# PacificBiosciences/pb-StarPhase

Measured on AMD Instinct MI355X. Metric: HiFi reads/sec diplotyped (HLA+CYP2D6), higher is better.
Workload: dtype int32; 1 GPU; BASELINE configs[1] + configs[2] as ONE sample per step: HLA-A/-B 10000 HiFi reads vs IMGT/HLA v0.14.1 (11,199 DNA alleles) + CYP2D6 2000 targeted reads (39 templates), the six configs[2] scenarios in turn; a new sample uploaded every step; reads -> diplotypes; hla_reads=10000, cyp2d6_reads=2000, cyp2d6_lanes=6, hla_lanes=2, cyp2d6_consensus=launch pairs

## Files before the change

pb-starphase_amd/csrc/sp_affine.hip:

```cpp
#include "sp_internal.h"
#include "sp_wfa.hip.h"
#include <mutex>
#include <set>
#include <string>

namespace {

constexpr int AF_NEG = -(1 << 28);
constexpr uint32_t AF_BIAS = 1u << 22;

struct AfState { int s; uint32_t m0, m1; };
struct AfKey { uint32_t k, m0, m1; };

__device__ __forceinline__ AfState af_none() { AfState x; x.s = AF_NEG; x.m0 = 0; x.m1 = 0; return x; }
template <int CTRL, int ROW_MASK>
__device__ __forceinline__ AfKey af_dpp(const AfKey& v) {
    AfKey r;
    r.k = (uint32_t)__builtin_amdgcn_update_dpp(0, (int)v.k, CTRL, ROW_MASK, 0xf, false);
    r.m0 = (uint32_t)__builtin_amdgcn_update_dpp(0, (int)v.m0, CTRL, ROW_MASK, 0xf, false);
    r.m1 = (uint32_t)__builtin_amdgcn_update_dpp(0, (int)v.m1, CTRL, ROW_MASK, 0xf, false);
    return r;
}
__device__ __forceinline__ AfKey af_max(const AfKey& a, const AfKey& b) { return b.k > a.k ? b : a; }
__device__ __forceinline__ AfKey af_scan(AfKey v) {
// ... 307 lines not shown
        }
        spw::wave_lds_sync();
        if (lane == 0) {
            while (true) {
                const int r = ci - i_lo - r0;
                if (r < 0) break;
                if ((unsigned)cidx >= (unsigned)BAND) { done = 2; break; }
                const uint32_t d = tile[r * BAND + cidx];
                if (st == 0) {
                    const uint32_t h = d & 7u;
                    if (h == AF_D_DIAG || h == AF_D_START) { emit((d & AF_D_X) ? 8u : 7u); --ci; if (h == AF_D_START) { done = 1; break; } continue; }
                    if (h >= AF_D_NONE) { done = 2; break; }
                    st = (int)h;
                }
                if (st == (int)AF_D_E1 || st == (int)AF_D_E2) {
                    emit(2u); const bool cont = d & (st == (int)AF_D_E1 ? AF_D_E1C : AF_D_E2C); --ci; ++cidx; if (!cont) st = 0;
                } else {
                    emit(1u); const bool cont = d & (st == (int)AF_D_F1 ? AF_D_F1C : AF_D_F2C); --cidx; if (!cont) st = 0;
                }
            }
        }
        ci = __shfl(ci, 0); done = __shfl(done, 0);
        if (ci < i_lo && !done) done = 2;
    }
    if (lane == 0) {
        emit(0xE);
        res.score = bs; res.nm = (int32_t)bm1; res.b_start = (int32_t)(bm0 >> 16); res.b_end = bi + 1; res.a_start = (int32_t)(bm0 & 0xFFFFu); res.a_end = bj + 1;
        const bool lost = done != 1 || n_ops > ops_cap;
        out[p] = res; n_cigar[p] = lost ? AF_TB_LOST : n_ops;
        const uint32_t n_out = lost ? 0u : (n_ops < stride ? n_ops : stride);
        for (uint32_t k = 0; k < n_out; ++k) cigar[(size_t)p * stride + k] = ops[n_ops - 1 - k];
    }
}

inline int64_t af_tb_rows(int tlen, int qlen, int diag, int band) {
    const int64_t klo = -(int64_t)diag - band / 2;
    int64_t i_lo = -(klo + band - 1); if (i_lo < 0) i_lo = 0;
    int64_t i_hi = (int64_t)qlen - 1 - klo; if (i_hi > (int64_t)tlen - 1) i_hi = (int64_t)tlen - 1;
    if (tlen <= 0 || qlen <= 0 || i_lo > i_hi) return 0;
    return i_hi - i_lo + 1;
}

}

int sp_launch_affine(sp_ctx* ctx, const sp_seqset* A, const sp_seqset* B, const void* d_pairs, uint64_t n_pairs, const sp_affine_opts& o, int band, sp_affine_aln* d_out,
                     const char* prof_name, const uint32_t* d_n_live, const void* d_wins, const void* d_mids) {
    if (n_pairs == 0) return SP_OK;
    if (band != 64 && band != 256) return sp_fail(ctx, SP_ERR_INVALID_ARG, "affine: band must be 64 or 256");
    if (B->max_len > 65535 || A->max_len > 65535) return sp_fail(ctx, SP_ERR_TOO_LONG, "affine: sequences of up to 65,535 bases");
    const int t_words_max = (B->max_len >> 4) + 4;
    const size_t lds_bytes = sizeof(uint32_t) * (size_t)(4 * t_words_max + 2 * (2 * band / 16 + 8));
    ProfScope ps(ctx, prof_name, n_pairs);
    const bool hasn = A->has_n || B->has_n;
#define SP_AF_LAUNCH(D, N) do { \
        (void)hipFuncSetAttribute((const void*)affine_kernel<D, N>, hipFuncAttributeMaxDynamicSharedMemorySize, (int)lds_bytes); \
        hipLaunchKernelGGL((affine_kernel<D, N>), dim3((uint32_t)n_pairs), dim3(64), lds_bytes, ctx->stream, A->view(), B->view(), (const AfPair*)d_pairs, (uint32_t)n_pairs, d_n_live, o, d_out, t_words_max, (const AfWin*)d_wins, (const AfMid*)d_mids); } while (0)
    if (band == 64) { if (hasn) SP_AF_LAUNCH(1, true); else SP_AF_LAUNCH(1, false); }
    else { if (hasn) SP_AF_LAUNCH(4, true); else SP_AF_LAUNCH(4, false); }
#undef SP_AF_LAUNCH
    if (hipGetLastError() != hipSuccess) return sp_fail(ctx, SP_ERR_HIP, "affine launch failed");
    return SP_OK;
}

constexpr int AF_ISOLATED = 16;
constexpr int AF_MARGIN = 24;
struct AfAudit { int32_t route, diag; };
__device__ __forceinline__ int af_gap_cost(const sp_affine_opts& o, int l) { const int c1 = o.q + l * o.e, c2 = o.q2 + l * o.e2; return c1 < c2 ? c1 : c2; }
struct AfPathCost {
    int pen = 0, type = -1, pos = 0, run = 0;
    __device__ __forceinline__ void step(const sp_affine_opts& o, int t, int p) {
        if (t == (int)SP_EV_X) { pen += o.b; run = 0; }
        else {
            const bool more = run > 0 && t == type && p == (t == (int)SP_EV_D ? pos + 1 : pos);
            run = more ? run + 1 : 1;
            pen += af_gap_cost(o, run) - (run > 1 ? af_gap_cost(o, run - 1) : 0);
        }
        type = t; pos = p;
    }
};

template <bool ENDS>
__global__ void af_classify_kernel(const CellDesc* __restrict__ cells, const sp_aln* __restrict__ ref, const sp_aln* __restrict__ tr, const uint32_t* __restrict__ ev,
                                   uint32_t stride, uint32_t n, int target_is_a, int has_n, sp_affine_opts o, sp_affine_aln* __restrict__ out,
                                   AfPair* __restrict__ todo, uint32_t* __restrict__ todo_at, uint32_t* __restrict__ n_todo, AfWin* __restrict__ wins, AfMid* __restrict__ mids, int band, int windows, int ends_only, AfAudit* __restrict__ audit) {
    const uint32_t x = blockIdx.x * blockDim.x + threadIdx.x;
    if (x >= n) return;
    sp_affine_aln res; res.score = 0; res.nm = 0; res.a_start = res.a_end = res.b_start = res.b_end = 0;
    const CellDesc c = cells[x];
    if (c.max_ed < 0) { out[x] = res; if (audit) { audit[x].route = 3; audit[x].diag = target_is_a ? -c.diag : c.diag; } return; }
    const sp_aln r = ref[x], t = tr[x];
    const int d_mid = ((r.b_start - r.a_start) + (r.b_end - r.a_end)) / 2;
    const int d_dp = r.ok ? (target_is_a ? -d_mid : d_mid) : (target_is_a ? -c.diag : c.diag);
    bool simple = !has_n && r.ok && t.ok && t.nm == r.nm && t.a_start == r.a_start && t.a_end == r.a_end && t.b_start == r.b_start && t.b_end == r.b_end && (uint32_t)r.nm <= stride;
    const bool traced = simple;
    int nx = 0, ngap = 0, gap_cost = -1;
    if (simple) {
        const uint32_t* e = ev + (size_t)x * stride;
        int prev = -(1 << 29);
        for (int k = 0; k < r.nm && simple; ++k) {
            const uint32_t w = e[k]; const int pos = (int)(w & 0x3FFFFFFFu), type = (int)(w >> 30);
            const int gap = pos > prev ? pos - prev : prev - pos;
            if (k > 0 && gap < AF_ISOLATED) simple = false;
            if (pos - r.b_start < AF_ISOLATED || r.b_end - pos < AF_ISOLATED) simple = false;
            if (type == (int)SP_EV_X) ++nx; else ++ngap;
            prev = pos;
        }
    }
    int kh = -1, kt = r.nm;
    if (ENDS && ends_only > 0 && traced && !simple && r.nm > 0) {
        const uint32_t* e = ev + (size_t)x * stride;
        const int clear = o.a * AF_ISOLATED - af_gap_cost(o, 1);
        AfPathCost pc; int nxd = 0, total = 0, drift = 0;
        bool in_band = true;
        nx = 0; ngap = 0;
        for (int pass = 0; pass < 2; ++pass) {
            pc = AfPathCost(); nxd = 0;
            for (int k = 0; k < r.nm; ++k) {
                const uint32_t w = e[k]; const int pos = (int)(w & 0x3FFFFFFFu), type = (int)(w >> 30);
                const int before = o.a * (pos - r.b_start - nxd) - pc.pen;
                pc.step(o, type, pos);
                if (type != (int)SP_EV_I) ++nxd;
                if (pass == 0) {
                    if (type == (int)SP_EV_X) ++nx; else ++ngap;
                    drift += type == (int)SP_EV_D ? 1 : type == (int)SP_EV_I ? -1 : 0;
                    const int off = (r.b_start - r.a_start) + drift - d_mid;
                    if (off <= -(band / 2 - 2) || off >= band / 2 - 2) in_band = false;
                    const int prev = k > 0 ? (int)(e[k - 1] & 0x3FFFFFFFu) : -(1 << 29), next = k + 1 < r.nm ? (int)(e[k + 1] & 0x3FFFFFFFu) : (1 << 29);
                    const bool lone = pos - prev >= AF_ISOLATED && next - pos >= AF_ISOLATED && pos - r.b_start >= AF_ISOLATED && r.b_end - pos >= AF_ISOLATED;
                    if (o.a * (pos - r.b_start - (nxd - (type != (int)SP_EV_I ? 1 : 0))) - pc.pen < clear || (!lone && pos - r.b_start < ends_only)) kh = k;
                    if (!lone && r.b_end - pos < ends_only && k < kt) kt = k;
                } else if (total - before < clear && k < kt) kt = k;
            }
            if (pass == 0) total = o.a * (r.b_end - r.b_start - nxd) - pc.pen;
        }
        if (!in_band) { kh = r.nm - 1; kt = 0; }
        if (kh < 0 && kt == r.nm) { simple = true; gap_cost = pc.pen - o.b * nx; }
    }
    if (simple) {
        const int a_span = r.a_end - r.a_start, b_span = r.b_end - r.b_start;
        const int m2 = a_span + b_span - 2 * nx - ngap;
        const int M = m2 / 2;
        res.score = o.a * M - o.b * nx - (gap_cost >= 0 ? gap_cost : (o.q + o.e) * ngap); res.nm = r.nm;
        if (target_is_a) { res.b_start = r.a_start; res.b_end = r.a_end; res.a_start = r.b_start; res.a_end = r.b_end; }
        else { res.a_start = r.a_start; res.a_end = r.a_end; res.b_start = r.b_start; res.b_end = r.b_end; }
        out[x] = res;
        if (audit) { audit[x].route = 0; audit[x].diag = d_dp; }
        return;
    }
    const uint32_t at = atomicAdd(n_todo, 1u);
    AfPair p;
    if (target_is_a) { p.a = c.b; p.b = c.a; } else { p.a = c.a; p.b = c.b; }
    p.diag = d_dp; p.pad = 0;
    todo[at] = p; todo_at[at] = x;
    AfWin w; w.r0 = -1; w.r1 = -1; w.idx_in = w.idx_out = 0; w.s_in = w.nm_in = w.d_score = w.d_nm = w.end_t = w.end_q = w.n_mid = 0; w.start_cell = 0;
    if (traced && windows && r.nm > 0) {
        const uint32_t* e = ev + (size_t)x * stride;
        auto pos_of = [&](int k) { return (int)(e[k] & 0x3FFFFFFFu); };
        int wF[AF_MAXMID + 1], wL[AF_MAXMID + 1], wIn[AF_MAXMID + 1], wOut[AF_MAXMID + 1], nw = 0;
        const bool ends_head = ENDS && kh >= 0, ends_tail = ENDS && kt < r.nm;
        if (ends_head || ends_tail) {
            if (ends_head) { while (kh + 1 < r.nm && pos_of(kh + 1) - pos_of(kh) < AF_MARGIN + AF_ISOLATED) ++kh; }
            if (ends_tail) { while (kt > 0 && pos_of(kt) - pos_of(kt - 1) < AF_MARGIN + AF_ISOLATED) --kt; }
            if (kh < kt) {
                if (ends_head) { wF[nw] = 0; wL[nw] = kh; wIn[nw] = pos_of(0) - AF_MARGIN; wOut[nw] = pos_of(kh) + AF_MARGIN; ++nw; }
                if (ends_tail) { wF[nw] = kt; wL[nw] = r.nm - 1; wIn[nw] = pos_of(kt) - AF_MARGIN; wOut[nw] = pos_of(r.nm - 1) + AF_MARGIN; ++nw; }
            }
        } else
        for (int k = 0; k < r.nm; ++k) {
            const int pos = pos_of(k);
            const bool lone = !(pos - r.b_start < AF_ISOLATED || r.b_end - pos < AF_ISOLATED) && !(k > 0 && pos - pos_of(k - 1) < AF_ISOLATED) && !(k + 1 < r.nm && pos_of(k + 1) - pos < AF_ISOLATED);
            if (lone) continue;
            int kF = k, kL = k;
            const int floor_k = nw ? wL[nw - 1] + 1 : 0;
            int entry = pos_of(kF) - AF_MARGIN;
            while (kF > floor_k && pos_of(kF - 1) > entry - AF_ISOLATED) { --kF; entry = pos_of(kF) - AF_MARGIN; }
            int leave = pos_of(kL) + AF_MARGIN;
            while (kL + 1 < r.nm && pos_of(kL + 1) < leave + AF_ISOLATED) { ++kL; leave = pos_of(kL) + AF_MARGIN; }
            if (nw && (entry - wOut[nw - 1] < AF_ISOLATED || nw == AF_MAXMID + 1)) { wL[nw - 1] = kL; wOut[nw - 1] = leave; }
            else { wF[nw] = kF; wL[nw] = kL; wIn[nw] = entry; wOut[nw] = leave; ++nw; }
            k = kL;
        }
        if (nw > 0) {
            const int klo = -p.diag - band / 2;
            int i = r.a_start, j = r.b_start, cx = 0, cd = 0, ci = 0, k = 0; AfPathCost pc;
            auto piece_cost = [&]() { return ENDS ? pc.pen : o.b * cx + (o.q + o.e) * (cd + ci); };
            auto step_to = [&](int k2) { const int pos = pos_of(k2), type = (int)(e[k2] >> 30); if (ENDS) pc.step(o, type, pos); i += pos - j; j = pos; if (type == (int)SP_EV_X) { ++i; ++j; ++cx; } else if (type == (int)SP_EV_D) { ++j; ++cd; } else { ++i; ++ci; } };
            AfMid* mid = mids + (size_t)at * AF_MAXMID;
            int out_t = 0, out_idx = 0, out_b = 0; bool have_out = false;
            for (int v = 0; v < nw; ++v) {
                for (; k < wF[v]; ++k) step_to(k);
                {
                    const int ia = i + (wIn[v] - j), jb = wIn[v];
                    const int t_in = target_is_a ? ia : jb, q_in = target_is_a ? jb : ia;
                    const int idx = (q_in - t_in) - klo;
                    const bool fits = idx >= 0 && idx < band && t_in >= 1 && q_in >= 1;
                    if (v == 0) {
                        if (wIn[0] - r.b_start >= AF_ISOLATED && fits) {
                            w.r0 = t_in; w.idx_in = idx;
                            w.s_in = o.a * ((wIn[0] - r.b_start) - cx - cd) - piece_cost(); w.nm_in = cx + cd + ci;
                            const int ts = target_is_a ? r.a_start : r.b_start, qs = target_is_a ? r.b_start : r.a_start;
                            w.start_cell = ((uint32_t)ts << 16) | (uint32_t)(qs & 0xFFFF);
                        }
                    } else if (have_out && fits && t_in > out_t + 1) {
                        AfMid m; m.r_exit = out_t; m.idx_out = out_idx; m.r_entry = t_in; m.idx_in = idx;
                        m.d_score = o.a * ((wIn[v] - out_b - 1) - cx - cd) - piece_cost(); m.d_nm = cx + cd + ci;
                        mid[w.n_mid++] = m;
                    }
                }
                for (; k <= wL[v]; ++k) step_to(k);
                cx = cd = ci = 0; pc.pen = 0;
                {
                    const int ia = i + (wOut[v] - j), jb = wOut[v];
                    const int t_out = target_is_a ? ia : jb, q_out = target_is_a ? jb : ia;
                    const int idx = (q_out - t_out) - klo;
                    have_out = idx >= 0 && idx < band && wOut[v] >= j;
                    out_t = t_out; out_idx = idx; out_b = wOut[v];
                }
            }
            if (have_out && r.b_end - out_b >= AF_ISOLATED) {
                for (; k < r.nm; ++k) step_to(k);
                w.r1 = out_t; w.idx_out = out_idx;
                w.d_score = o.a * ((r.b_end - out_b - 1) - cx - cd) - piece_cost(); w.d_nm = cx + cd + ci;
                w.end_t = target_is_a ? r.a_end : r.b_end; w.end_q = target_is_a ? r.b_end : r.a_end;
            }
        }
    }
    wins[at] = w;
    if (audit) { audit[x].route = (w.r0 >= 0 || w.r1 >= 0 || w.n_mid > 0) ? 1 : 2; audit[x].diag = d_dp; }
}
__global__ void af_scatter_kernel(const sp_affine_aln* __restrict__ part, const uint32_t* __restrict__ todo_at, const uint32_t* __restrict__ n_todo, sp_affine_aln* __restrict__ out) {
    const uint32_t k = blockIdx.x * blockDim.x + threadIdx.x;
    if (k < *n_todo) out[todo_at[k]] = part[k];
}

int sp_rescore_mappings(sp_ctx* ctx, const sp_seqset* Aw, const sp_seqset* Bw, const CellDesc* d_cells, const sp_aln* d_ref, uint64_t n, bool target_is_a,
                        const sp_affine_opts& o, int band, sp_affine_aln* d_out, const char* prefix, uint32_t stride, int trace_retry_wide, const sp_aln* d_tr_in, const uint32_t* d_ev_in, int ends_only, int windows, void* d_audit) {
    if (n == 0) return SP_OK;
    const std::string pre(prefix);
    static std::mutex names_lock; static std::set<std::string> names;
    auto stable = [&](const std::string& n2) { std::lock_guard<std::mutex> g(names_lock); return names.insert(n2).first->c_str(); };
    const sp_aln* d_tr = d_tr_in ? d_tr_in : (const sp_aln*)sp_pool(ctx, (pre + "_tr").c_str(), n * sizeof(sp_aln));
    const uint32_t* d_ev = d_ev_in ? d_ev_in : (const uint32_t*)sp_pool(ctx, (pre + "_ev").c_str(), n * (size_t)stride * 4);
    AfPair* d_todo = (AfPair*)sp_pool(ctx, (pre + "_todo").c_str(), n * sizeof(AfPair));
    uint32_t* d_at = (uint32_t*)sp_pool(ctx, (pre + "_at").c_str(), n * 4 + 64);
    sp_affine_aln* d_part = (sp_affine_aln*)sp_pool(ctx, (pre + "_part").c_str(), n * sizeof(sp_affine_aln));
    AfWin* d_win = (AfWin*)sp_pool(ctx, (pre + "_win").c_str(), n * sizeof(AfWin));
    AfMid* d_mid = (AfMid*)sp_pool(ctx, (pre + "_mid").c_str(), n * sizeof(AfMid) * AF_MAXMID);
    if (!d_tr || !d_ev || !d_todo || !d_at || !d_part || !d_win || !d_mid) return sp_fail(ctx, SP_ERR_OUT_OF_MEMORY, "rescore buffers");
    uint32_t* d_n = d_at + n;
    (void)hipMemsetAsync(d_n, 0, 4, ctx->stream);
    int rc = SP_OK;
    if (!d_tr_in) rc = sp_launch_cells(ctx, Aw, Bw, d_cells, n, const_cast<sp_aln*>(d_tr), const_cast<uint32_t*>(d_ev), stride, stable(pre + "_trace"), trace_retry_wide);
    if (rc != SP_OK) return rc;
    auto* classify = ends_only > 0 ? af_classify_kernel<true> : af_classify_kernel<false>;
    hipLaunchKernelGGL(classify, dim3((unsigned)((n + 255) / 256)), dim3(256), 0, ctx->stream, d_cells, d_ref, d_tr, d_ev, stride, (uint32_t)n, target_is_a ? 1 : 0,
                       (Aw->has_n || Bw->has_n) ? 1 : 0, o, d_out, d_todo, d_at, d_n, d_win, d_mid, band, windows < 0 ? (ctx->mm2_rescore == 2 ? 0 : 1) : windows, ends_only, (AfAudit*)d_audit);
    rc = sp_launch_affine(ctx, target_is_a ? Bw : Aw, target_is_a ? Aw : Bw, d_todo, n, o, band, d_part, stable(pre + "_dp"), d_n, d_win, d_mid);
    if (rc != SP_OK) return rc;
    hipLaunchKernelGGL(af_scatter_kernel, dim3((unsigned)((n + 255) / 256)), dim3(256), 0, ctx->stream, d_part, d_at, d_n, d_out);
    if (ctx->profile_rescore_counts && ctx->profiling) {
        uint32_t n_dp = 0;
        SP_HIP_CHECK(ctx, hipMemcpyAsync(&n_dp, d_n, 4, hipMemcpyDeviceToHost, ctx->stream));
        SP_HIP_CHECK(ctx, hipStreamSynchronize(ctx->stream));
        auto& e = ctx->prof[pre + "_dp_pairs"]; e.cells += n_dp; e.launches += 1;
    }
    return SP_OK;
}

extern "C" int32_t sp_affine_rescore_batch(sp_ctx* ctx, const sp_seqset* A, const sp_seqset* B, const sp_pair* pairs, uint64_t n_pairs, const sp_affine_opts* opts,
                                           int32_t band, sp_affine_aln* out) {
    if (!ctx || !A || !B || !opts || (n_pairs && (!pairs || !out))) return SP_ERR_INVALID_ARG;
    if (n_pairs == 0) return SP_OK;
    if (n_pairs > 0xFFFFFFFFull) return sp_fail(ctx, SP_ERR_INVALID_ARG, "affine: too many pairs");
    (void)hipSetDevice(ctx->device);
    for (uint64_t i = 0; i < n_pairs; ++i) if (pairs[i].a >= A->n || pairs[i].b >= B->n) return sp_fail(ctx, SP_ERR_INVALID_ARG, "affine: index out of range");
    static_assert(sizeof(sp_pair) == sizeof(AfPair), "pair layout");
    void* d_pairs = sp_pool(ctx, "affine_pairs", n_pairs * sizeof(sp_pair));
    sp_affine_aln* d_out = (sp_affine_aln*)sp_pool(ctx, "affine_out", n_pairs * sizeof(sp_affine_aln));
    if (!d_pairs || !d_out) return sp_fail(ctx, SP_ERR_OUT_OF_MEMORY, "affine buffers");
    SP_HIP_CHECK(ctx, hipMemcpyAsync(d_pairs, pairs, n_pairs * sizeof(sp_pair), hipMemcpyHostToDevice, ctx->stream));
    const int rc = sp_launch_affine(ctx, A, B, d_pairs, n_pairs, *opts, band, d_out, "affine_rescore", nullptr, nullptr, nullptr);
    if (rc != SP_OK) return rc;
    SP_HIP_CHECK(ctx, hipMemcpyAsync(out, d_out, n_pairs * sizeof(sp_affine_aln), hipMemcpyDeviceToHost, ctx->stream));
    SP_HIP_CHECK(ctx, hipStreamSynchronize(ctx->stream));
    return SP_OK;
}

extern "C" int32_t sp_affine_rescore_mappings_audit(sp_ctx* ctx, const sp_seqset* A, const sp_seqset* B, const sp_pair* pairs, uint64_t n_pairs, const sp_affine_opts* opts,
                                                    int32_t band, int32_t target_is_a, uint32_t events_stride, int32_t windows, int32_t ends_only, sp_affine_aln* out,
                                                    int32_t* route, int32_t* diag) {
    if (!ctx || !A || !B || !opts || (n_pairs && (!pairs || !out || !route || !diag))) return SP_ERR_INVALID_ARG;
    if (n_pairs == 0) return SP_OK;
    if (n_pairs > 0xFFFFFFFFull) return sp_fail(ctx, SP_ERR_INVALID_ARG, "rescore audit: too many pairs");
    if (events_stride == 0 || events_stride > SP_MAX_ED + 1) return sp_fail(ctx, SP_ERR_INVALID_ARG, "rescore audit: events_stride must be 1..SP_MAX_ED + 1");
    if (ends_only < 0) return sp_fail(ctx, SP_ERR_INVALID_ARG, "rescore audit: ends_only must be >= 0");
    (void)hipSetDevice(ctx->device);
    std::vector<CellDesc> cells(n_pairs);
    for (uint64_t i = 0; i < n_pairs; ++i) {
        if (pairs[i].a >= A->n || pairs[i].b >= B->n) return sp_fail(ctx, SP_ERR_INVALID_ARG, "rescore audit: index out of range");
        if (pairs[i].max_ed > SP_MAX_ED) return sp_fail(ctx, SP_ERR_INVALID_ARG, "rescore audit: max_ed must be <= SP_MAX_ED (< 0: no mapping)");
        cells[i] = CellDesc{pairs[i].a, pairs[i].b, pairs[i].diag, pairs[i].max_ed, 0, -1};
    }
    CellDesc* d_cells = (CellDesc*)sp_pool(ctx, "af_audit_cells", n_pairs * sizeof(CellDesc));
    sp_aln* d_ref = (sp_aln*)sp_pool(ctx, "af_audit_ref", n_pairs * sizeof(sp_aln));
    sp_affine_aln* d_out = (sp_affine_aln*)sp_pool(ctx, "af_audit_out", n_pairs * sizeof(sp_affine_aln));
    AfAudit* d_audit = (AfAudit*)sp_pool(ctx, "af_audit_route", n_pairs * sizeof(AfAudit));
    if (!d_cells || !d_ref || !d_out || !d_audit) return sp_fail(ctx, SP_ERR_OUT_OF_MEMORY, "rescore audit buffers");
    SP_HIP_CHECK(ctx, hipMemcpyAsync(d_cells, cells.data(), n_pairs * sizeof(CellDesc), hipMemcpyHostToDevice, ctx->stream));
    SP_HIP_CHECK(ctx, hipMemsetAsync(d_ref, 0, n_pairs * sizeof(sp_aln), ctx->stream));
    int rc = sp_launch_cells(ctx, A, B, d_cells, n_pairs, d_ref, nullptr, 0, "af_audit_cells", 2);
    if (rc != SP_OK) return rc;
    rc = sp_rescore_mappings(ctx, A, B, d_cells, d_ref, n_pairs, target_is_a != 0, *opts, band, d_out, "af_audit", events_stride, 2, nullptr, nullptr, ends_only, windows ? 1 : 0, d_audit);
    if (rc != SP_OK) return rc;
    std::vector<AfAudit> au(n_pairs);
    SP_HIP_CHECK(ctx, hipMemcpyAsync(out, d_out, n_pairs * sizeof(sp_affine_aln), hipMemcpyDeviceToHost, ctx->stream));
    SP_HIP_CHECK(ctx, hipMemcpyAsync(au.data(), d_audit, n_pairs * sizeof(AfAudit), hipMemcpyDeviceToHost, ctx->stream));
    SP_HIP_CHECK(ctx, hipStreamSynchronize(ctx->stream));
    for (uint64_t i = 0; i < n_pairs; ++i) { route[i] = au[i].route; diag[i] = au[i].diag; }
    return SP_OK;
}

constexpr size_t AF_TB_BUDGET = 512ull << 20;

extern "C" int32_t sp_affine_align_batch(sp_ctx* ctx, const sp_seqset* A, const sp_seqset* B, const sp_pair* pairs, uint64_t n_pairs, const sp_affine_opts* opts,
                                         int32_t band, sp_affine_aln* out, uint32_t* cigar, uint32_t cigar_stride, uint32_t* n_cigar) {
    if (!ctx || !A || !B || !opts || (n_pairs && (!pairs || !out || !n_cigar || (cigar_stride && !cigar)))) return SP_ERR_INVALID_ARG;
    if (n_pairs == 0) return SP_OK;
    if (n_pairs > 0xFFFFFFFFull) return sp_fail(ctx, SP_ERR_INVALID_ARG, "affine: too many pairs");
    if (band != 64 && band != 256) return sp_fail(ctx, SP_ERR_INVALID_ARG, "affine: band must be 64 or 256");
    if (B->max_len > 65535 || A->max_len > 65535) return sp_fail(ctx, SP_ERR_TOO_LONG, "affine: sequences of up to 65,535 bases");
    (void)hipSetDevice(ctx->device);
    for (uint64_t i = 0; i < n_pairs; ++i) if (pairs[i].a >= A->n || pairs[i].b >= B->n) return sp_fail(ctx, SP_ERR_INVALID_ARG, "affine: index out of range");
    std::vector<uint64_t> off(n_pairs); std::vector<uint64_t> chunk_end;
    size_t used = 0, largest = 0;
    for (uint64_t i = 0; i < n_pairs; ++i) {
        const int64_t rows = pairs[i].max_ed < 0 ? 0 : af_tb_rows(B->h_len[pairs[i].b], A->h_len[pairs[i].a], pairs[i].diag, band);
        const size_t bytes = rows ? (((size_t)rows * band + ((size_t)2 * rows + 2) * 4 + 15) & ~(size_t)15) : 0;
        if (used && used + bytes > AF_TB_BUDGET) { chunk_end.push_back(i); used = 0; }
        off[i] = used; used += bytes; largest = std::max(largest, used);
// ... 273 lines not shown
```

pb-starphase_amd/csrc/sp_api.hip:

```cpp
#include "sp_internal.h"
#include <algorithm>
#include <thread>
#include <atomic>
#include <cstring>
#include <new>
#include <unistd.h>

extern "C" {

int32_t sp_abi_version(void) { return SP_ABI_VERSION; }

int32_t sp_device_count(int32_t* count) {
    int n = 0;
    hipError_t e = hipGetDeviceCount(&n);
    if (count) *count = (e == hipSuccess) ? n : 0;
    return e == hipSuccess ? SP_OK : SP_ERR_NO_DEVICE;
}

int32_t sp_ctx_create(int32_t device, void* stream, sp_ctx** out) {
    if (!out) return SP_ERR_INVALID_ARG;
    *out = nullptr;
    static std::atomic<int> effective{-1};
    bool by_library = false;
    if (effective.load() < 0) {
// ... 2 lines not shown
        for (int fd = 0; fd < 1024 && !hip_up; ++fd) {
            char path[64]; std::snprintf(path, sizeof path, "/proc/self/fd/%d", fd);
            const ssize_t k = readlink(path, link, sizeof link - 1);
            if (k > 0) { link[k] = 0; hip_up = std::strcmp(link, "/dev/kfd") == 0; }
        }
        const char* had = std::getenv("GPU_MAX_HW_QUEUES");
        if (!had && !hip_up) { (void)setenv("GPU_MAX_HW_QUEUES", "16", 0); by_library = true; }
        const char* now = std::getenv("GPU_MAX_HW_QUEUES");
        effective.store(now ? std::atoi(now) : (hip_up ? 0 : 4));
    }
    const int hw_queues = effective.load() > 0 ? effective.load() : 4;
    int n = 0;
    if (hipGetDeviceCount(&n) != hipSuccess || n <= 0 || device < 0 || device >= n) return SP_ERR_NO_DEVICE;
    if (hipSetDevice(device) != hipSuccess) return SP_ERR_NO_DEVICE;
    hipDeviceProp_t prop;
    if (hipGetDeviceProperties(&prop, device) != hipSuccess) return SP_ERR_NO_DEVICE;
    if (std::strncmp(prop.gcnArchName, "gfx950", 6) != 0) return SP_ERR_NO_DEVICE;
    sp_ctx* ctx = new (std::nothrow) sp_ctx();
    if (!ctx) return SP_ERR_OUT_OF_MEMORY;
    ctx->device = device;
    ctx->num_cus = prop.multiProcessorCount > 0 ? prop.multiProcessorCount : 256;
    static bool set_here = false;
    if (by_library) set_here = true;
    ctx->hw_queues = hw_queues; ctx->hw_queues_by_library = set_here;
    ctx->hw_queues_effective = effective.load();
    { const char* kc = std::getenv("SP_K8_COMPOUND"); if (kc && *kc) ctx->k8_compound = std::atoi(kc); }
    { const char* ks = std::getenv("SP_K8_SIDE_ORDERS"); if (ks && *ks) ctx->k8_side_orders = std::max(0, std::min(3, std::atoi(ks))); }
    { const char* kp = std::getenv("SP_K8_PERSISTENT"); if (kp && *kp) ctx->k8_persistent = std::atoi(kp); }
    if (effective.load() == 0)
        ctx->warning = "the HIP runtime was initialised before the library's first context and GPU_MAX_HW_QUEUES was not set: the process's streams share the runtime's 4 hardware queues; "
                       "export GPU_MAX_HW_QUEUES=16 (or more) before the process initialises HIP";
    else if (hw_queues < 16)
        ctx->warning = "GPU_MAX_HW_QUEUES=" + std::to_string(hw_queues) + ": the library's streams share " + std::to_string(hw_queues) +
                       " hardware queues; export GPU_MAX_HW_QUEUES=16 (or more) before the process initialises HIP";
    if (stream) { ctx->stream = (hipStream_t)stream; ctx->own_stream = false; }
    else {
        if (hipStreamCreateWithFlags(&ctx->stream, hipStreamNonBlocking) != hipSuccess) { delete ctx; return SP_ERR_HIP; }
        ctx->own_stream = true;
    }
    if (hipEventCreate(&ctx->ev0) != hipSuccess || hipEventCreate(&ctx->ev1) != hipSuccess) { delete ctx; return SP_ERR_HIP; }
    *out = ctx;
    return SP_OK;
}

int32_t sp_ctx_get_info(const sp_ctx* ctx, sp_ctx_info* out) {
    if (!ctx || !out) return SP_ERR_INVALID_ARG;
    std::memset(out, 0, sizeof *out);
    out->device = ctx->device; out->num_cus = ctx->num_cus; out->hw_queues = ctx->hw_queues; out->hw_queues_set_by_library = ctx->hw_queues_by_library ? 1 : 0;
    std::snprintf(out->warning, sizeof out->warning, "%s", ctx->warning.c_str());
    return SP_OK;
}

static int32_t upload_finish(sp_seqset* s);
void sp_ctx_destroy(sp_ctx* ctx) {
    if (!ctx) return;
    for (sp_ctx*& h : ctx->helper) if (h) { sp_ctx_destroy(h); h = nullptr; }
    hipSetDevice(ctx->device);
    if (ctx->uploading) (void)upload_finish(ctx->uploading);
    if (ctx->copy_stream) { hipStreamSynchronize(ctx->copy_stream); hipStreamDestroy(ctx->copy_stream); ctx->copy_stream = nullptr; }
    if (ctx->ctl_stream) { hipStreamSynchronize(ctx->ctl_stream); hipStreamDestroy(ctx->ctl_stream); ctx->ctl_stream = nullptr; }
    if (ctx->ev_fork) hipEventDestroy(ctx->ev_fork);
    if (ctx->ev_join) hipEventDestroy(ctx->ev_join);
    hipStreamSynchronize(ctx->stream);
    for (sp_seqset* s : ctx->live_sets) {
        for (void* p : { (void*)s->d_words, (void*)s->d_nplane, (void*)s->d_word_off, (void*)s->d_len, (void*)s->d_kcode, (void*)s->d_kpos, (void*)s->d_koff }) if (p) ctx->dev_cap.erase(p);
        s->ctx = nullptr;
    }
    for (auto& kv : ctx->dev_cap) (void)hipFree(kv.first);
    if (ctx->scratch) hipFree(ctx->scratch);
    for (auto& kv : ctx->pool) if (kv.second.first) hipFree(kv.second.first);
    for (auto& kv : ctx->host_pool) if (kv.second.first) hipHostFree(kv.second.first);
    sp_profile_flush(ctx);
    for (hipEvent_t e : ctx->prof_free) hipEventDestroy(e);
    if (ctx->ev0) hipEventDestroy(ctx->ev0);
    if (ctx->ev1) hipEventDestroy(ctx->ev1);
    if (ctx->own_stream && ctx->stream) hipStreamDestroy(ctx->stream);
    delete ctx;
}

}
sp_ctx* sp_ctx_helper(sp_ctx* ctx, int i) {
    if (i < 0 || i > 6) return nullptr;
    if (!ctx->helper[i] && sp_ctx_create(ctx->device, nullptr, &ctx->helper[i]) != SP_OK) ctx->helper[i] = nullptr;
    if (ctx->helper[i]) { ctx->helper[i]->profiling = ctx->profiling; ctx->helper[i]->k5_block_pairs = ctx->k5_block_pairs; ctx->helper[i]->k8_persistent = ctx->k8_persistent; ctx->helper[i]->k8_side_orders = ctx->k8_side_orders; ctx->helper[i]->k8_compound = ctx->k8_compound; ctx->helper[i]->k8_side_max_blocks = ctx->k8_side_max_blocks; ctx->helper[i]->mm2_rescore = ctx->mm2_rescore; ctx->helper[i]->profile_rescore_counts = ctx->profile_rescore_counts; ctx->helper[i]->k1_best_n = ctx->k1_best_n; }
    return ctx->helper[i];
}
void sp_profile_merge(sp_ctx* into, sp_ctx* from) {
    sp_profile_flush(from);
    for (auto& kv : from->prof) { ProfileEntry& e = into->prof[kv.first]; e.ms += kv.second.ms; e.launches += kv.second.launches; e.cells += kv.second.cells; }
    from->prof.clear();
}
extern "C" {

int32_t sp_struct_size(const char* name) {
    if (!name) return -1;
#define SP_SZ(T) if (std::strcmp(name, #T) == 0) return (int32_t)sizeof(T);
    SP_SZ(sp_ctx_info)
    SP_SZ(sp_pair)
    SP_SZ(sp_aln)
    SP_SZ(sp_hla_db_desc)
    SP_SZ(sp_hla_realign)
    SP_SZ(sp_k1_seed_hit)
    SP_SZ(sp_hla_best)
    SP_SZ(sp_chain_problem)
    SP_SZ(sp_chain_result)
    SP_SZ(sp_region_hit)
    SP_SZ(sp_cyp_problem)
    SP_SZ(sp_cyp_call)
    SP_SZ(sp_cyp_locus)
    SP_SZ(sp_cyp_gene_def)
    SP_SZ(sp_cyp_config)
    SP_SZ(sp_cyp_db_stats)
    SP_SZ(sp_variant_problem)
    SP_SZ(sp_variant_result)
    SP_SZ(sp_sv_definitions)
    SP_SZ(sp_cons_config)
    SP_SZ(sp_cons_result)
    SP_SZ(sp_cons_problem)
    SP_SZ(sp_cons_output)
    SP_SZ(sp_priority_problem)
    SP_SZ(sp_priority_job)
    SP_SZ(sp_hla_call_config)
    SP_SZ(sp_hla_call)
    SP_SZ(sp_diplotype_settings)
    SP_SZ(sp_sample_inputs)
    SP_SZ(sp_starphase_timing)
    SP_SZ(sp_cyp_read_mapping)
    SP_SZ(sp_database_metadata)
    SP_SZ(sp_database_stats)
    SP_SZ(sp_gene_region)
    SP_SZ(sp_variant_detail)
    SP_SZ(sp_bam_read)
    SP_SZ(sp_affine_opts)
    SP_SZ(sp_affine_aln)
    SP_SZ(sp_k1_seed_info)
    SP_SZ(sp_cyp_region_variants)
    SP_SZ(sp_chain_build_info)
    SP_SZ(sp_variant_gene_stats)
    SP_SZ(sp_vcf_allele)
    SP_SZ(sp_vcf_deletion)
    SP_SZ(sp_mapping_stats)
    SP_SZ(sp_hla_rev_hit)
    SP_SZ(sp_batch_options)
    SP_SZ(sp_starphase_batch_timing)
    SP_SZ(sp_hla_alleles_stats)
    SP_SZ(sp_hla_cfg_mapping)
    SP_SZ(sp_hla_cfg_gene)
    SP_SZ(sp_pileup_col)
    SP_SZ(sp_support_summary)
    SP_SZ(sp_support_entry)
#undef SP_SZ
    return -1;
}

const char* sp_last_error(const sp_ctx* ctx) { return ctx ? ctx->err.c_str() : "null context"; }

int32_t sp_ctx_synchronize(sp_ctx* ctx) {
    if (!ctx) return SP_ERR_INVALID_ARG;
    SP_HIP_CHECK(ctx, hipStreamSynchronize(ctx->stream));
    return SP_OK;
}

int32_t sp_ctx_set_option(sp_ctx* ctx, const char* name, int64_t value) {
    if (!ctx || !name) return SP_ERR_INVALID_ARG;
    if (std::strcmp(name, "hla_split_genes") == 0) { ctx->split_genes = value != 0; return SP_OK; }
    if (std::strcmp(name, "k1_best_n") == 0) { if (value < 0 || value > 8) return sp_fail(ctx, SP_ERR_INVALID_ARG, "sp_ctx_set_option: k1_best_n is 0..8"); ctx->k1_best_n = (int)value; for (sp_ctx* h : ctx->helper) if (h) h->k1_best_n = ctx->k1_best_n; return SP_OK; }
    if (std::strcmp(name, "profile_rescore_counts") == 0) { ctx->profile_rescore_counts = value != 0; for (sp_ctx* h : ctx->helper) if (h) h->profile_rescore_counts = ctx->profile_rescore_counts; return SP_OK; }
    if (std::strcmp(name, "mm2_rescore") == 0) { ctx->mm2_rescore = (int)value; for (sp_ctx* h : ctx->helper) if (h) h->mm2_rescore = ctx->mm2_rescore; return SP_OK; }
    if (std::strcmp(name, "k8_side_orders") == 0) { if (value < 0 || value > 3) return sp_fail(ctx, SP_ERR_INVALID_ARG, "sp_ctx_set_option: k8_side_orders is 0 .. 3"); ctx->k8_side_orders = (int)value; for (sp_ctx* h : ctx->helper) if (h) h->k8_side_orders = ctx->k8_side_orders; return SP_OK; }
    if (std::strcmp(name, "k8_compound") == 0) { ctx->k8_compound = (int)value; for (sp_ctx* h : ctx->helper) if (h) h->k8_compound = ctx->k8_compound; return SP_OK; }
    if (std::strcmp(name, "k8_side_max_blocks") == 0) { if (value < 0) return sp_fail(ctx, SP_ERR_INVALID_ARG, "sp_ctx_set_option: k8_side_max_blocks >= 0"); ctx->k8_side_max_blocks = (int)value; for (sp_ctx* h : ctx->helper) if (h) h->k8_side_max_blocks = ctx->k8_side_max_blocks; return SP_OK; }
    if (std::strcmp(name, "k8_persistent") == 0) { if (value < 0 || value > 2) return sp_fail(ctx, SP_ERR_INVALID_ARG, "sp_ctx_set_option: k8_persistent is 0 (never), 1 (whenever a batch fits) or 2 (the library decides)"); ctx->k8_persistent = (int)value; ctx->k8_persist_backoff = 0; ctx->k8_persist_failures = 0; for (sp_ctx* h : ctx->helper) if (h) h->k8_persistent = ctx->k8_persistent; return SP_OK; }
    if (std::strcmp(name, "cons_retry_ladder") == 0) { ctx->cons_retry_ladder = value != 0; for (sp_ctx* h : ctx->helper) if (h) h->cons_retry_ladder = ctx->cons_retry_ladder; return SP_OK; }
    if (std::strcmp(name, "k5_block_pairs") == 0) { if (value < 0 || value > (1 << 20)) return sp_fail(ctx, SP_ERR_INVALID_ARG, "sp_ctx_set_option: k5_block_pairs is 0..1048576"); ctx->k5_block_pairs = (int)value; for (sp_ctx* h : ctx->helper) if (h) h->k5_block_pairs = ctx->k5_block_pairs; return SP_OK; }
    if (std::strcmp(name, "cyp_cohort_min_group") == 0) { if (value < 1 || value > 64) return sp_fail(ctx, SP_ERR_INVALID_ARG, "sp_ctx_set_option: cyp_cohort_min_group is 1..64"); ctx->cyp_cohort_min_group = (int)value; return SP_OK; }
    if (std::strcmp(name, "cyp_cohort_streams") == 0) { if (value < 1 || value > 8) return sp_fail(ctx, SP_ERR_INVALID_ARG, "sp_ctx_set_option: cyp_cohort_streams is 1..8"); ctx->cyp_cohort_streams = (int)value; return SP_OK; }
    if (std::strcmp(name, "hla_split_streams") == 0) { if (value < 1 || value > 4) return sp_fail(ctx, SP_ERR_INVALID_ARG, "sp_ctx_set_option: hla_split_streams is 1..4"); ctx->split_streams = (int)value; return SP_OK; }
    return sp_fail(ctx, SP_ERR_INVALID_ARG, std::string("sp_ctx_set_option: unknown option ") + name);
}

int32_t sp_profile_reset(sp_ctx* ctx) {
    if (!ctx) return SP_ERR_INVALID_ARG;
    for (sp_ctx* h : ctx->helper) if (h) sp_profile_reset(h);
    sp_profile_flush(ctx); ctx->prof.clear();
    unsigned long long* c = sp_counters(ctx);
    if (c) { hipSetDevice(ctx->device); hipMemsetAsync(c, 0, SPC_N * sizeof(unsigned long long), ctx->stream); }
    return SP_OK;
}

int32_t sp_profile_get(sp_ctx* ctx, const char* kernel, double* total_ms, uint64_t* launches, uint64_t* cells) {
    if (!ctx || !kernel) return SP_ERR_INVALID_ARG;
    sp_profile_flush(ctx);
    for (sp_ctx* h : ctx->helper) if (h) sp_profile_merge(ctx, h);
    static const struct { const char* name; int idx; } counters[] = {
        {"count:k1_cells_active", SPC_K1_ACTIVE}, {"count:k1_cells_executed", SPC_K1_EXECUTED}, {"count:k1_cells_resumed", SPC_K1_RESUMED},
        {"count:k1_cells_bytes", SPC_K1_BYTES}, {"count:cons_launches", SPC_CONS_LAUNCHES}, {"count:cons_columns", SPC_CONS_COLUMNS},
        {"count:dbg0", 6}, {"count:dbg1", 7}, {"count:dbg2", 8}, {"count:dbg3", 9}, {"count:dbg4", 10}, {"count:dbg5", 11}, {"count:dbg6", 12}, {"count:dbg7", 13} };
    for (const auto& c : counters) if (std::strcmp(kernel, c.name) == 0) {
        unsigned long long v = 0; unsigned long long* d = sp_counters(ctx);
        if (d) { hipSetDevice(ctx->device); if (hipMemcpyAsync(&v, d + c.idx, 8, hipMemcpyDeviceToHost, ctx->stream) != hipSuccess || hipStreamSynchronize(ctx->stream) != hipSuccess) return sp_fail(ctx, SP_ERR_HIP, "sp_profile_get: counter read failed"); }
        for (sp_ctx* h : ctx->helper) if (h) {
            unsigned long long hv = 0; unsigned long long* hd = sp_counters(h);
            if (hd && hipMemcpyAsync(&hv, hd + c.idx, 8, hipMemcpyDeviceToHost, h->stream) == hipSuccess && hipStreamSynchronize(h->stream) == hipSuccess) v += hv;
        }
        if (total_ms) *total_ms = 0.0;
        if (launches) *launches = 0;
        if (cells) *cells = v;
        return SP_OK;
    }
    if (std::strcmp(kernel, "pool:device") == 0) {
        uint64_t allocs = ctx->pool_allocs, bytes = ctx->scratch_bytes;
        for (const auto& b : ctx->pool) bytes += b.second.second;
        for (sp_ctx* h : ctx->helper) if (h) { allocs += h->pool_allocs; bytes += h->scratch_bytes; for (const auto& b : h->pool) bytes += b.second.second; }
        if (total_ms) *total_ms = 0.0;
        if (launches) *launches = allocs;
        if (cells) *cells = bytes;
        return SP_OK;
    }
    auto it = ctx->prof.find(kernel);
    ProfileEntry e; if (it != ctx->prof.end()) e = it->second;
    if (total_ms) *total_ms = e.ms;
    if (launches) *launches = e.launches;
    if (cells) *cells = e.cells;
    return SP_OK;
}


struct sp_upload {
    std::thread th;
    int32_t rc = SP_OK; std::string err;
    int format = SP_SEQ_ASCII;
    const uint8_t* src = nullptr; uint64_t src_bytes = 0;
    std::vector<uint64_t> rel;
    uint8_t* d_stage = nullptr; uint64_t* d_off = nullptr; uint32_t* d_flag = nullptr;
    uint8_t* ring = nullptr; size_t chunk = 0; int slots = 0;
    hipEvent_t slot_ev[4] = { nullptr, nullptr, nullptr, nullptr };
    size_t wbytes = 0;
};

static constexpr size_t UPLOAD_CHUNK = (size_t)8 << 20;
static constexpr int UPLOAD_SLOTS = 4;

static void upload_run(sp_seqset* s) {
    sp_upload* u = s->up; sp_ctx* ctx = s->ctx;
    hipStream_t st = ctx->copy_stream;
    auto bad = [&](hipError_t e, const char* what) { if (e != hipSuccess && u->rc == SP_OK) { u->rc = SP_ERR_HIP; u->err = std::string(what) + ": " + hipGetErrorString(e); } return e != hipSuccess; };
    if (bad(hipSetDevice(ctx->device), "hipSetDevice")) return;
    const uint32_t n = s->n;
    bad(hipMemcpyAsync(s->d_word_off, s->h_word_off.data(), ((size_t)n + 1) * sizeof(uint64_t), hipMemcpyHostToDevice, st), "offsets");
    if (n) bad(hipMemcpyAsync(s->d_len, s->h_len.data(), (size_t)n * sizeof(int32_t), hipMemcpyHostToDevice, st), "lengths");
    bad(hipMemsetAsync(s->d_words, 0, u->wbytes, st), "clear");
// ... 426 lines not shown
```

pb-starphase_amd/csrc/sp_cyp.hip:

```cpp
#include "sp_internal.h"
#include <system_error>
#include <thread>
#include <atomic>
#include <memory>
#include <map>
#include "sp_json.h"
#include "sp_wfa.hip.h"
#include <algorithm>
#include <cmath>
#include <cstring>
#include <numeric>
#include <string>
#include <vector>

namespace {

inline bool t_is_cyp2d(int t) { return t == SP_CYP_CYP2D6 || t == SP_CYP_CYP2D7 || t == SP_CYP_DELETION || t == SP_CYP_HYBRID; }
inline bool t_is_rep(int t) { return t == SP_CYP_REP6 || t == SP_CYP_REP7; }
inline bool t_is_reported(int t) { return t == SP_CYP_CYP2D6 || t == SP_CYP_DELETION || t == SP_CYP_HYBRID; }
inline bool t_allowed(int t) { return t != SP_CYP_UNKNOWN && t != SP_CYP_FALSE_ALLELE; }
inline bool t_normalizing(int t, bool all) { return all ? t_is_cyp2d(t) : t == SP_CYP_CYP2D6; }
inline bool t_head(int t, bool all) {
    if (t == SP_CYP_REP6 || t == SP_CYP_DELETION) return true;
    if (t == SP_CYP_CYP2D6 || t == SP_CYP_HYBRID) return t_normalizing(t, all);
// ... 466 lines not shown
    const bool block_per_pair = n_pairs <= (uint64_t)ctx->k5_block_pairs;
    const uint64_t blocks = block_per_pair ? n_pairs : (n_pairs + 255) / 256;
    if (blocks > 0x7FFFFFFFull) return sp_fail(ctx, SP_ERR_TOO_LONG, "chain pair: too many chain pairs for one launch");
    PairConsts pc{H, P, maxlen, R, ignore ? 1 : 0, norm_all ? 1 : 0, infer ? 1 : 0, p->lasso_penalty, p->ln_ed_penalty, p->unexpected_chain_penalty,
                  p->inferred_edge_penalty, n_pairs};
    std::vector<double> ovv(p->w_ov, p->w_ov + (size_t)n_rows * H);
    size_t in_bytes = 0;
    auto place = [&](size_t bytes) { const size_t at = (in_bytes + 15) & ~(size_t)15; in_bytes = at + std::max<size_t>(bytes, 16); return at; };
    auto bytes_of = [](const auto& v) { return v.size() * sizeof(v[0]); };
    const size_t at_chains = place(bytes_of(chains)), at_clen = place(bytes_of(clen)), at_unexp = place(bytes_of(unexp)), at_ninf = place(bytes_of(ninf)), at_del = place(bytes_of(has_del)),
                 at_lasso = place(bytes_of(hap_lasso)), at_norm = place(bytes_of(hap_norm)), at_rwo = place(bytes_of(rwo)), at_ed = place(bytes_of(ed32)), at_ov = place(bytes_of(ovv)),
                 at_opt = place(bytes_of(optimum)), at_worst = place(bytes_of(worst)), at_lf = place(bytes_of(ln_fact)), at_lp = place(bytes_of(ln_p));
    uint8_t* d_in = (uint8_t*)sp_pool(ctx, "k5_in", in_bytes + 16); uint8_t* h_in = (uint8_t*)sp_host_pool(ctx, "k5_in", in_bytes + 16);
    if (!d_in || !h_in) return sp_fail(ctx, SP_ERR_OUT_OF_MEMORY, "chain pair buffers");
    auto put = [&](size_t at, const auto& v) { if (!v.empty()) std::memcpy(h_in + at, v.data(), v.size() * sizeof(v[0])); };
    put(at_chains, chains); put(at_clen, clen); put(at_unexp, unexp); put(at_ninf, ninf); put(at_del, has_del); put(at_lasso, hap_lasso); put(at_norm, hap_norm); put(at_rwo, rwo);
    put(at_ed, ed32); put(at_ov, ovv); put(at_opt, optimum); put(at_worst, worst); put(at_lf, ln_fact); put(at_lp, ln_p);
    (void)hipMemcpyAsync(d_in, h_in, in_bytes, hipMemcpyHostToDevice, ctx->stream);
    uint8_t* d_chains = d_in + at_chains; int32_t* d_clen = (int32_t*)(d_in + at_clen);
    uint32_t* d_unexp = (uint32_t*)(d_in + at_unexp); uint32_t* d_ninf = (uint32_t*)(d_in + at_ninf);
    uint8_t* d_del = d_in + at_del; uint8_t* d_lasso = d_in + at_lasso; uint8_t* d_norm = d_in + at_norm;
    int32_t* d_rwo = (int32_t*)(d_in + at_rwo); uint32_t* d_ed = (uint32_t*)(d_in + at_ed); double* d_ov = (double*)(d_in + at_ov);
    uint64_t* d_opt = (uint64_t*)(d_in + at_opt); uint64_t* d_worst = (uint64_t*)(d_in + at_worst);
    double* d_lf = (double*)(d_in + at_lf); double* d_lp = (double*)(d_in + at_lp);
    const size_t out_bytes = 16 + (size_t)blocks * (8 + 8 + 8 + 40);
    uint8_t* d_out = (uint8_t*)sp_pool(ctx, "k5_out", out_bytes); uint8_t* h_out = (uint8_t*)sp_host_pool(ctx, "k5_out", out_bytes);
    unsigned long long* d_gb = (unsigned long long*)d_out;
    double* d_bs = (double*)(d_out + 16); unsigned long long* d_bp = (unsigned long long*)(d_out + 16 + (size_t)blocks * 8);
    unsigned long long* d_be = (unsigned long long*)(d_out + 16 + (size_t)blocks * 16); double* d_bc = (double*)(d_out + 16 + (size_t)blocks * 24);
    if (!d_out || !h_out) return sp_fail(ctx, SP_ERR_OUT_OF_MEMORY, "chain pair buffers");
    if (!d_chains || !d_clen || !d_unexp || !d_ninf || !d_del || !d_lasso || !d_norm || !d_rwo || !d_ed || !d_ov || !d_opt || !d_worst || !d_lf || !d_lp ||
        !d_gb || !d_bs || !d_bp || !d_bc || !d_be) return sp_fail(ctx, SP_ERR_OUT_OF_MEMORY, "chain pair buffers");
    unsigned long long* d_tb = (unsigned long long*)sp_pool(ctx, "k5_tab_best", std::max<size_t>(1, (size_t)P * R) * 8);
    unsigned long long* d_tm = (unsigned long long*)sp_pool(ctx, "k5_tab_mask", std::max<size_t>(1, (size_t)P * R) * 8);
    if (!d_tb || !d_tm) return sp_fail(ctx, SP_ERR_OUT_OF_MEMORY, "chain pair tables");
    if ((size_t)P * R) {
        ProfScope ps(ctx, "k5_chain_reads", (uint64_t)P * R);
        hipLaunchKernelGGL(k5_chain_read_kernel, dim3((unsigned)(((size_t)P * R + 255) / 256)), dim3(256), 0, ctx->stream, P, R, H, maxlen, d_chains, d_clen, d_rwo, d_ed, d_tb, d_tm);
    }
    const unsigned long long init[2] = {0x7FF0000000000000ull , 0ull};
    (void)hipMemcpyAsync(d_gb, init, 16, hipMemcpyHostToDevice, ctx->stream);
    (void)hipMemsetAsync(d_bp, 0xFF, blocks * 8, ctx->stream);
    {
        ProfScope ps(ctx, "k5_pairs", n_pairs);
        if (block_per_pair)
            hipLaunchKernelGGL(k5_pair_block_kernel, dim3((unsigned)blocks), dim3(K5_TILE), 0, ctx->stream, pc, d_chains, d_clen, d_unexp, d_ninf, d_del, d_lasso, d_norm,
                               d_rwo, d_ov, d_tb, d_tm, d_opt, d_worst, d_lf, lf_n, d_lp, max_total + 1, d_gb, d_bs, d_bp, d_bc, d_be, d_gb + 1);
        else {
        (void)hipFuncSetAttribute((const void*)k5_pair_kernel, hipFuncAttributeMaxDynamicSharedMemorySize, (int)((size_t)256 * H * sizeof(double)));
        hipLaunchKernelGGL(k5_pair_kernel, dim3((unsigned)blocks), dim3(256), (size_t)256 * H * sizeof(double), ctx->stream, pc, d_chains, d_clen, d_unexp, d_ninf, d_del, d_lasso, d_norm,
                           d_rwo, d_ed, d_ov, d_tb, d_tm, d_opt, d_worst, d_lf, lf_n, d_lp, max_total + 1, d_gb, d_bs, d_bp, d_bc, d_be, d_gb + 1);
        }
        if (hipGetLastError() != hipSuccess) return sp_fail(ctx, SP_ERR_HIP, "k5 launch failed");
    }
    (void)hipMemcpyAsync(h_out, d_out, out_bytes, hipMemcpyDeviceToHost, ctx->stream);
    const unsigned long long* gb = (const unsigned long long*)h_out;
    const double* bs = (const double*)(h_out + 16); const unsigned long long* bp = (const unsigned long long*)(h_out + 16 + (size_t)blocks * 8);
    const unsigned long long* be = (const unsigned long long*)(h_out + 16 + (size_t)blocks * 16); const double* bc = (const double*)(h_out + 16 + (size_t)blocks * 24);
    hipError_t e = hipStreamSynchronize(ctx->stream);
    if (e != hipSuccess) return sp_fail(ctx, SP_ERR_HIP, std::string("chain pair: ") + hipGetErrorString(e));
    res->n_pairs_scored = gb[1];
    int64_t wb = -1;
    for (uint64_t b = 0; b < blocks; ++b) {
        if (bp[b] == 0xFFFFFFFFFFFFFFFFull) continue;
        if (wb < 0 || bs[b] < bs[wb] || (bs[b] == bs[wb] && bp[b] < bp[wb])) wb = (int64_t)b;
    }
    if (wb < 0) return SP_ERR_NO_SCORE_PAIRS;
    uint64_t pid = bp[wb]; int wi = 0;
    while (wi + 1 < P && (uint64_t)(wi + 1) * P - (uint64_t)(wi + 1) * wi / 2 <= pid) ++wi;
    const int wj = (int)(pid - ((uint64_t)wi * P - (uint64_t)wi * (wi - 1) / 2)) + wi;
    res->index1 = wi; res->index2 = wj;
    res->score = bs[wb]; res->ln_ed_penalty = bc[wb * 5]; res->mn_llh_penalty = bc[wb * 5 + 1]; res->allele_expected_penalty = bc[wb * 5 + 2];
    res->unexpected_chain_penalty = bc[wb * 5 + 3]; res->inferred_chain_penalty = bc[wb * 5 + 4]; res->edit_distance = be[wb];
    const std::vector<int>* a = &possible[wi]; const std::vector<int>* b = &possible[wj];
    if (*b < *a) std::swap(a, b);
    res->n1 = (int32_t)a->size(); res->n2 = (int32_t)b->size();
    for (size_t x = 0; x < a->size(); ++x) res->chain1[x] = (*a)[x];
    for (size_t x = 0; x < b->size(); ++x) res->chain2[x] = (*b)[x];
    return SP_OK;
}

#define CYP_TOPK      4
#define CYP_MIN_VOTES 4

int sp_seqset_build_index(sp_ctx* ctx, sp_seqset* s);

__global__ void cyp_build_cells_kernel(const uint32_t* __restrict__ a_idx, const uint32_t* __restrict__ b_idx,
                                       const int32_t* __restrict__ diag, const int32_t* __restrict__ votes, uint64_t n_pairs, int topk,
                                       int min_votes, const int32_t* __restrict__ a_len, double frac_cap, CellDesc* __restrict__ cells) {
    uint64_t i = (uint64_t)blockIdx.x * blockDim.x + threadIdx.x;
    if (i >= n_pairs * (uint64_t)topk) return;
    const uint64_t p = i / (uint64_t)topk;
    CellDesc c; c.a = a_idx[p]; c.b = b_idx[p]; c.max_ed = SP_MAX_ED; c.b_lo = 0; c.b_hi = -1;
    if (frac_cap > 0.0) { const int cap = (int)(frac_cap * (double)a_len[c.a]) + 1; c.max_ed = cap < SP_MAX_ED ? cap : SP_MAX_ED; }
    c.diag = votes[i] >= min_votes ? diag[i] : SP_NO_DIAG;
    cells[i] = c;
}

static int cyp_align_pairs(sp_ctx* ctx, const sp_seqset* A, const sp_seqset* B, const std::vector<uint32_t>& ai, const std::vector<uint32_t>& bi, uint32_t a_period,
                           int topk, double frac_cap, int retry_wide, const char* prof, std::vector<sp_aln>& out, std::vector<int32_t>* diag_out = nullptr, std::vector<int32_t>* votes_out = nullptr) {
    const uint64_t n_pairs = ai.size(), n_cells = n_pairs * (uint64_t)topk;
    out.assign(n_cells, sp_aln{});
    if (n_pairs == 0) return SP_OK;
    int rc = sp_seqset_build_index(ctx, const_cast<sp_seqset*>(A));
    if (rc) return rc;
    uint32_t* d_a = (uint32_t*)sp_pool(ctx, "cyp_a", n_pairs * 4); uint32_t* d_b = (uint32_t*)sp_pool(ctx, "cyp_b", n_pairs * 4);
    int32_t* d_d = (int32_t*)sp_pool(ctx, "cyp_d", n_cells * 4); int32_t* d_v = (int32_t*)sp_pool(ctx, "cyp_v", n_cells * 4);
    CellDesc* d_cells = (CellDesc*)sp_pool(ctx, "cyp_cells", n_cells * sizeof(CellDesc));
    sp_aln* d_alns = (sp_aln*)sp_pool(ctx, "cyp_alns", n_cells * sizeof(sp_aln));
    if (!d_a || !d_b || !d_d || !d_v || !d_cells || !d_alns) return sp_fail(ctx, SP_ERR_OUT_OF_MEMORY, "cyp placement buffers");
    (void)hipMemcpyAsync(d_a, ai.data(), n_pairs * 4, hipMemcpyHostToDevice, ctx->stream);
    (void)hipMemcpyAsync(d_b, bi.data(), n_pairs * 4, hipMemcpyHostToDevice, ctx->stream);
    (void)hipStreamSynchronize(ctx->stream);
    rc = sp_launch_anchor(ctx, A, B, d_a, d_b, n_pairs, d_d, d_v, topk, "anchor", a_period);
    if (rc) return rc;
    hipLaunchKernelGGL(cyp_build_cells_kernel, dim3((unsigned)((n_cells + 255) / 256)), dim3(256), 0, ctx->stream, d_a, d_b, d_d, d_v, n_pairs, topk, CYP_MIN_VOTES, A->d_len, frac_cap, d_cells);
    rc = sp_launch_cells(ctx, A, B, d_cells, n_cells, d_alns, nullptr, 0, prof, retry_wide);
    if (rc) return rc;
    (void)hipMemcpyAsync(out.data(), d_alns, n_cells * sizeof(sp_aln), hipMemcpyDeviceToHost, ctx->stream);
    if (diag_out && votes_out) {
        diag_out->resize(n_cells); votes_out->resize(n_cells);
        (void)hipMemcpyAsync(diag_out->data(), d_d, n_cells * 4, hipMemcpyDeviceToHost, ctx->stream);
        (void)hipMemcpyAsync(votes_out->data(), d_v, n_cells * 4, hipMemcpyDeviceToHost, ctx->stream);
    }
    hipError_t e = hipStreamSynchronize(ctx->stream);
    if (e != hipSuccess) return sp_fail(ctx, SP_ERR_HIP, std::string("cyp placements: ") + hipGetErrorString(e));
    return SP_OK;
}

__global__ void cyp_all_pairs_kernel(uint32_t nA, uint64_t n_pairs, uint32_t* __restrict__ a_idx, uint32_t* __restrict__ b_idx) {
    const uint64_t i = (uint64_t)blockIdx.x * blockDim.x + threadIdx.x;
    if (i >= n_pairs) return;
    a_idx[i] = (uint32_t)(i % nA); b_idx[i] = (uint32_t)(i / nA);
}
static int cyp_align_all_pinned(sp_ctx* ctx, const sp_seqset* A, const sp_seqset* B, int topk, double frac_cap, const char* prof, sp_aln** out, int32_t** diag_out, int32_t** votes_out) {
    const uint64_t nA = A->n, n_pairs = nA * (uint64_t)B->n, n_cells = n_pairs * (uint64_t)topk;
    *out = nullptr; *diag_out = nullptr; *votes_out = nullptr;
    if (n_pairs == 0) return SP_OK;
    int rc = sp_seqset_build_index(ctx, const_cast<sp_seqset*>(A));
    if (rc) return rc;
    uint32_t* d_a = (uint32_t*)sp_pool(ctx, "cyp_a", n_pairs * 4); uint32_t* d_b = (uint32_t*)sp_pool(ctx, "cyp_b", n_pairs * 4);
    int32_t* d_d = (int32_t*)sp_pool(ctx, "cyp_d", n_cells * 4); int32_t* d_v = (int32_t*)sp_pool(ctx, "cyp_v", n_cells * 4);
    CellDesc* d_cells = (CellDesc*)sp_pool(ctx, "cyp_cells", n_cells * sizeof(CellDesc));
    sp_aln* d_alns = (sp_aln*)sp_pool(ctx, "cyp_alns", n_cells * sizeof(sp_aln));
    sp_aln* h_alns = (sp_aln*)sp_host_pool(ctx, "k3_alns_host", n_cells * sizeof(sp_aln));
    int32_t* h_d = (int32_t*)sp_host_pool(ctx, "k3_diag_host", n_cells * 4); int32_t* h_v = (int32_t*)sp_host_pool(ctx, "k3_votes_host", n_cells * 4);
    if (!d_a || !d_b || !d_d || !d_v || !d_cells || !d_alns || !h_alns || !h_d || !h_v) return sp_fail(ctx, SP_ERR_OUT_OF_MEMORY, "cyp placement buffers");
    hipLaunchKernelGGL(cyp_all_pairs_kernel, dim3((unsigned)((n_pairs + 255) / 256)), dim3(256), 0, ctx->stream, (uint32_t)nA, n_pairs, d_a, d_b);
    rc = sp_launch_anchor(ctx, A, B, d_a, d_b, n_pairs, d_d, d_v, topk, "anchor", (uint32_t)nA);
    if (rc) return rc;
    hipLaunchKernelGGL(cyp_build_cells_kernel, dim3((unsigned)((n_cells + 255) / 256)), dim3(256), 0, ctx->stream, d_a, d_b, d_d, d_v, n_pairs, topk, CYP_MIN_VOTES, A->d_len, frac_cap, d_cells);
    rc = sp_launch_cells(ctx, A, B, d_cells, n_cells, d_alns, nullptr, 0, prof, 0);
    if (rc) return rc;
    (void)hipMemcpyAsync(h_alns, d_alns, n_cells * sizeof(sp_aln), hipMemcpyDeviceToHost, ctx->stream);
    (void)hipMemcpyAsync(h_d, d_d, n_cells * 4, hipMemcpyDeviceToHost, ctx->stream);
    (void)hipMemcpyAsync(h_v, d_v, n_cells * 4, hipMemcpyDeviceToHost, ctx->stream);
    hipError_t e = hipStreamSynchronize(ctx->stream);
    if (e != hipSuccess) return sp_fail(ctx, SP_ERR_HIP, std::string("cyp placements: ") + hipGetErrorString(e));
    *out = h_alns; *diag_out = h_d; *votes_out = h_v;
    return SP_OK;
}

static int cyp_align_all(sp_ctx* ctx, const sp_seqset* A, const sp_seqset* B, int topk, double frac_cap, int retry_wide, const char* prof, std::vector<sp_aln>& out,
                         std::vector<int32_t>* diag_out = nullptr, std::vector<int32_t>* votes_out = nullptr) {
    const uint64_t nA = A->n, nB = B->n, n_pairs = nA * nB;
    std::vector<uint32_t> ai(n_pairs), bi(n_pairs);
    for (uint64_t b = 0; b < nB; ++b) for (uint64_t a = 0; a < nA; ++a) { ai[b * nA + a] = (uint32_t)a; bi[b * nA + a] = (uint32_t)b; }
    return cyp_align_pairs(ctx, A, B, ai, bi, (uint32_t)nA, topk, frac_cap, retry_wide, prof, out, diag_out, votes_out);
}

static inline double cyp_score(int seq_len, int nm, int unmapped, bool penalize) {
    const int len = penalize ? seq_len : seq_len - unmapped;
    double num = (double)(nm + (penalize ? unmapped : 0)); if (num < 0.1) num = 0.1;
    return num / (double)len;
}

static void cyp_weights_from_alns(uint32_t C, const int32_t* cons_len, const uint8_t* allowed, uint32_t n_segments, const int32_t* seg_len, const std::vector<sp_aln>& alns,
                                  uint64_t* ed, double* ov, uint8_t* kept, const sp_affine_aln* af = nullptr);

constexpr int CYP_K4_NEAR = 16;
struct K4Pick { uint32_t a, b; const sp_aln* al; sp_affine_aln* out; };
static void cyp_pick_near_min(uint32_t C, const uint8_t* allowed, uint32_t n_segments, const int32_t* seg_len, const std::vector<sp_aln>& alns, std::vector<sp_affine_aln>& af,
                              uint32_t a0, const int32_t* a_of_c, uint32_t b0, std::vector<K4Pick>& picks) {
    af.assign((size_t)n_segments * C, sp_affine_aln{});
    for (uint32_t s = 0; s < n_segments; ++s) {
        int64_t best = INT64_MAX;
        for (uint32_t c = 0; c < C; ++c) {
            const sp_aln& al = alns[(size_t)s * C + c];
            if (!allowed[c] || !al.ok) continue;
            best = std::min<int64_t>(best, (int64_t)al.nm + (seg_len[s] - (al.b_end - al.b_start)));
        }
        if (best == INT64_MAX) continue;
        for (uint32_t c = 0; c < C; ++c) {
            const sp_aln& al = alns[(size_t)s * C + c];
            if (!allowed[c] || !al.ok || (int64_t)al.nm + (seg_len[s] - (al.b_end - al.b_start)) > best + CYP_K4_NEAR) continue;
            picks.push_back(K4Pick{ a_of_c ? (uint32_t)a_of_c[c] : a0 + c, b0 + s, &al, &af[(size_t)s * C + c] });
        }
    }
}
static int cyp_rescore_picks(sp_ctx* ctx, const sp_seqset* A, const sp_seqset* B, const std::vector<K4Pick>& picks) {
    const uint64_t n = picks.size();
    if (n == 0 || !ctx->mm2_rescore) return SP_OK;
    std::vector<CellDesc> cells(n); std::vector<sp_aln> ref(n); std::vector<sp_affine_aln> out(n);
    for (uint64_t x = 0; x < n; ++x) {
        const sp_aln& al = *picks[x].al;
        cells[x] = CellDesc{ picks[x].a, picks[x].b, ((al.b_start - al.a_start) + (al.b_end - al.a_end)) / 2, 320, 0, -1 };
        ref[x] = al;
    }
    CellDesc* d_cells = (CellDesc*)sp_pool(ctx, "k4_af_cells", n * sizeof(CellDesc));
    sp_aln* d_ref = (sp_aln*)sp_pool(ctx, "k4_af_ref", n * sizeof(sp_aln));
    sp_affine_aln* d_af = (sp_affine_aln*)sp_pool(ctx, "k4_af_out", n * sizeof(sp_affine_aln));
    if (!d_cells || !d_ref || !d_af) return sp_fail(ctx, SP_ERR_OUT_OF_MEMORY, "weights: re-score buffers");
    SP_HIP_CHECK(ctx, hipMemcpyAsync(d_cells, cells.data(), n * sizeof(CellDesc), hipMemcpyHostToDevice, ctx->stream));
    SP_HIP_CHECK(ctx, hipMemcpyAsync(d_ref, ref.data(), n * sizeof(sp_aln), hipMemcpyHostToDevice, ctx->stream));
    const sp_affine_opts ao = { 1, 4, 6, 2, 26, 1, 1 };
    const int rc = sp_rescore_mappings(ctx, A, B, d_cells, d_ref, n, false, ao, 256, d_af, "k4_af", 320);
    if (rc != SP_OK) return rc;
    SP_HIP_CHECK(ctx, hipMemcpyAsync(out.data(), d_af, n * sizeof(sp_affine_aln), hipMemcpyDeviceToHost, ctx->stream));
    SP_HIP_CHECK(ctx, hipStreamSynchronize(ctx->stream));
    for (uint64_t x = 0; x < n; ++x) *picks[x].out = out[x];
    return SP_OK;
}

extern "C" int32_t sp_cyp_weight_segments(sp_ctx* ctx, const sp_seqset* consensus, const uint8_t* allowed, const sp_seqset* segments,
                                          uint64_t* ed, double* ov, uint8_t* kept) {
    if (!ctx || !consensus || !segments || (consensus->n && !allowed) || (segments->n && (!ed || !ov || !kept))) return SP_ERR_INVALID_ARG;
    (void)hipSetDevice(ctx->device);
    std::vector<sp_aln> alns;
    int rc = cyp_align_all(ctx, consensus, segments, 1, 0.0, 1, "k4_weight_cells", alns);
    if (rc) return rc;
    std::vector<sp_affine_aln> af; std::vector<K4Pick> picks;
    if (ctx->mm2_rescore) {
        cyp_pick_near_min(consensus->n, allowed, segments->n, segments->h_len.data(), alns, af, 0, nullptr, 0, picks);
        rc = cyp_rescore_picks(ctx, consensus, segments, picks);
        if (rc) return rc;
    }
    cyp_weights_from_alns(consensus->n, consensus->h_len.data(), allowed, segments->n, segments->h_len.data(), alns, ed, ov, kept, af.empty() ? nullptr : af.data());
    return SP_OK;
}

static void cyp_weights_from_alns(uint32_t C, const int32_t* cons_len, const uint8_t* allowed, uint32_t n_segments, const int32_t* seg_len, const std::vector<sp_aln>& alns,
                                  uint64_t* ed, double* ov, uint8_t* kept, const sp_affine_aln* af) {
    for (uint32_t s = 0; s < n_segments; ++s) {
        const int seq_len = seg_len[s];
        double min_ed_frac = 1.0;
        for (uint32_t c = 0; c < C; ++c) {
            uint64_t& e = ed[(size_t)s * C + c]; double& o = ov[(size_t)s * C + c];
            e = (uint64_t)seq_len; o = 0.0;
            sp_aln al = alns[(size_t)s * C + c];
            if (!allowed[c] || !al.ok) continue;
            if (af && af[(size_t)s * C + c].score > 0) {
                const sp_affine_aln& r = af[(size_t)s * C + c];
                al.nm = r.nm; al.a_start = r.a_start; al.a_end = r.a_end; al.b_start = r.b_start; al.b_end = r.b_end;
            }
            const int con_len = cons_len[c];
            const uint64_t nm = (uint64_t)al.nm, unmapped = (uint64_t)(seq_len - (al.b_end - al.b_start));
            const uint64_t match_score = nm + unmapped;
            const double overlap_score = 1.0 - (double)(al.a_start + (con_len - al.a_end)) / (double)con_len;
            if (match_score < e || (match_score == e && overlap_score > o)) {
                e = match_score; o = overlap_score;
                const double sc = cyp_score(seq_len, (int)nm, (int)unmapped, true);
                if (sc < min_ed_frac) min_ed_frac = sc;
            }
        }
        kept[s] = min_ed_frac <= 0.05 ? 1 : 0;
    }
}

constexpr uint32_t K3_HOST_THREADS = 4, K3_HOST_MIN_READS = 256;
template <class F> static void k3_read_ranges(uint32_t n_reads, F&& fn) {
    const uint32_t nt = n_reads >= K3_HOST_MIN_READS ? K3_HOST_THREADS : 1, per = (n_reads + nt - 1) / nt;
    std::thread th[K3_HOST_THREADS]; bool started[K3_HOST_THREADS] = {};
    for (uint32_t t = 1; t < nt; ++t) {
        const uint32_t lo = std::min(n_reads, t * per), hi = std::min(n_reads, lo + per);
        try { th[t] = std::thread([&fn, t, lo, hi]() { fn(t, lo, hi); }); started[t] = true; } catch (...) { fn(t, lo, hi); }
    }
    fn(0u, 0u, std::min(n_reads, per));
    for (uint32_t t = 1; t < nt; ++t) if (started[t]) th[t].join();
}
static int32_t cyp_find_regions(sp_ctx* ctx, const sp_seqset* templates, const int32_t* template_type, const sp_seqset* reads,
                                double max_missing_frac, sp_region_hit* hits, uint64_t hits_cap, uint64_t* n_hits, bool rescore);
extern "C" int32_t sp_cyp_find_regions(sp_ctx* ctx, const sp_seqset* templates, const int32_t* template_type, const sp_seqset* reads,
                                       double max_missing_frac, sp_region_hit* hits, uint64_t hits_cap, uint64_t* n_hits) {
    if (!ctx) return SP_ERR_INVALID_ARG;
    return cyp_find_regions(ctx, templates, template_type, reads, max_missing_frac, hits, hits_cap, n_hits, ctx->mm2_rescore);
}
constexpr double K3_CAP_HI = 0.056, K3_OVL = 0.85;
constexpr int K3_RETRY_VOTES = 128, K3_RETRY_HOLE = 500;
static int32_t cyp_find_regions(sp_ctx* ctx, const sp_seqset* templates, const int32_t* template_type, const sp_seqset* reads,
                                double max_missing_frac, sp_region_hit* hits, uint64_t hits_cap, uint64_t* n_hits, bool rescore) {
    if (!ctx || !templates || !reads || !n_hits || (templates->n && !template_type) || (hits_cap && !hits)) return SP_ERR_INVALID_ARG;
    (void)hipSetDevice(ctx->device);
    *n_hits = 0;
    HostMarks hm(ctx);
    sp_aln* alns = nullptr; int32_t* adiag = nullptr; int32_t* avotes = nullptr;
    int rc = cyp_align_all_pinned(ctx, templates, reads, CYP_TOPK, 0.05, "k3_region_cells", &alns, &adiag, &avotes);
    if (rc) return rc;
    hm.mark("host:k3_cells");
    if (!alns) return SP_OK;
    const uint32_t T = templates->n;
    auto penalized_type = [](int t) { return t == SP_CYP_DELETION || t == SP_CYP_REP6 || t == SP_CYP_REP7; };
    if (rescore) {
        std::vector<CellDesc> retry; std::vector<uint32_t> retry_at;
        std::vector<CellDesc> retry_of[K3_HOST_THREADS]; std::vector<uint32_t> retry_at_of[K3_HOST_THREADS];
        k3_read_ranges(reads->n, [&](uint32_t part, uint32_t r_lo, uint32_t r_hi) {
        std::vector<CellDesc>& retry = retry_of[part]; std::vector<uint32_t>& retry_at = retry_at_of[part];
        std::vector<std::pair<int, int>> iv;
        for (uint32_t r = r_lo; r < r_hi; ++r) {
            const int rlen = reads->h_len[r];
            if (rlen == 0) continue;
            iv.clear();
            bool any_lost = false;
            for (uint32_t t = 0; t < T; ++t) {
                bool placed = false;
                for (int k = 0; k < CYP_TOPK; ++k) { const sp_aln& al = alns[((size_t)r * T + t) * CYP_TOPK + k]; if (al.ok) { placed = true; iv.push_back({ al.b_start, al.b_end }); } }
                if (!placed && avotes[((size_t)r * T + t) * CYP_TOPK] >= K3_RETRY_VOTES) any_lost = true;
            }
            if (!any_lost) continue;
            std::sort(iv.begin(), iv.end());
            for (uint32_t t = 0; t < T; ++t) {
                const size_t c0 = ((size_t)r * T + t) * CYP_TOPK;
                bool placed = false;
                for (int k = 0; k < CYP_TOPK; ++k) placed = placed || alns[c0 + k].ok;
                if (placed || avotes[c0] < K3_RETRY_VOTES) continue;
                const int tlen = templates->h_len[t], d0 = adiag[c0];
                const int s0 = std::max(0, d0), e0 = std::min(rlen, d0 + tlen);
                int uncovered = 0, at = s0;
                for (const auto& x : iv) { if (x.second <= at) continue; if (x.first >= e0) break; if (x.first > at) uncovered += x.first - at; at = std::max(at, x.second); if (at >= e0) break; }
                if (at < e0) uncovered += e0 - at;
                if (uncovered < K3_RETRY_HOLE) continue;
                int cap = (int)(0.05 * (double)tlen) + 1; if (cap > SP_MAX_ED) cap = SP_MAX_ED;
                retry.push_back(CellDesc{ t, r, d0, cap, 0, -1 }); retry_at.push_back((uint32_t)c0);
            }
        }
        });
        for (uint32_t part = 0; part < K3_HOST_THREADS; ++part) { retry.insert(retry.end(), retry_of[part].begin(), retry_of[part].end()); retry_at.insert(retry_at.end(), retry_at_of[part].begin(), retry_at_of[part].end()); }
        if (!retry.empty()) {
            const size_t nr = retry.size();
            CellDesc* d_rc = (CellDesc*)sp_pool(ctx, "k3_retry_cells", nr * sizeof(CellDesc)); sp_aln* d_ro = (sp_aln*)sp_pool(ctx, "k3_retry_alns", nr * sizeof(sp_aln));
            if (!d_rc || !d_ro) return sp_fail(ctx, SP_ERR_OUT_OF_MEMORY, "find_regions: retry buffers");
            std::vector<sp_aln> got(nr);
            SP_HIP_CHECK(ctx, hipMemcpyAsync(d_rc, retry.data(), nr * sizeof(CellDesc), hipMemcpyHostToDevice, ctx->stream));
            SP_HIP_CHECK(ctx, hipMemsetAsync(d_ro, 0, nr * sizeof(sp_aln), ctx->stream));
            { ProfScope ps(ctx, "k3_retry_wide", nr); rc = sp_launch_cells_wide(ctx, templates, reads, d_rc, nr, d_ro); }
            if (rc != SP_OK) return rc;
            SP_HIP_CHECK(ctx, hipMemcpyAsync(got.data(), d_ro, nr * sizeof(sp_aln), hipMemcpyDeviceToHost, ctx->stream));
            SP_HIP_CHECK(ctx, hipStreamSynchronize(ctx->stream));
            for (size_t x = 0; x < nr; ++x) if (got[x].ok) alns[retry_at[x]] = got[x];
            if (ctx->profiling) ctx->prof["k3_retried_pairs"].cells += nr;
        }
    }
    auto own_score = [&](const sp_region_hit& h) { return cyp_score(h.seq_len, h.nm, h.unmapped, penalized_type(template_type[h.template_idx])); };
    auto overlap = [](const sp_region_hit& u, const sp_region_hit& v) {
        const int min_end = std::min(u.end, v.end), max_start = std::max(u.start, v.start);
        return max_start < min_end ? (double)(min_end - max_start) / std::min((double)(u.end - u.start), (double)(v.end - v.start)) : 0.0;
    };
    struct Pl { sp_region_hit h; uint32_t which; uint8_t done; };
    auto rescore_list = [&](std::vector<Pl*>& list, const char* prof) -> int {
        const uint64_t nc = list.size();
        if (!nc) return SP_OK;
        CellDesc* cells = (CellDesc*)sp_host_pool(ctx, "k3_af_cells_host", nc * sizeof(CellDesc));
        sp_aln* ref = (sp_aln*)sp_host_pool(ctx, "k3_af_ref_host", nc * sizeof(sp_aln));
        sp_affine_aln* af = (sp_affine_aln*)sp_host_pool(ctx, "k3_af_out_host", nc * sizeof(sp_affine_aln));
        CellDesc* d_cells = (CellDesc*)sp_pool(ctx, "k3_af_cells", nc * sizeof(CellDesc));
        sp_aln* d_ref = (sp_aln*)sp_pool(ctx, "k3_af_ref", nc * sizeof(sp_aln));
        sp_affine_aln* d_af = (sp_affine_aln*)sp_pool(ctx, "k3_af_out", nc * sizeof(sp_affine_aln));
        if (!cells || !ref || !af || !d_cells || !d_ref || !d_af) return sp_fail(ctx, SP_ERR_OUT_OF_MEMORY, "find_regions: re-score buffers");
        k3_read_ranges((uint32_t)nc, [&](uint32_t, uint32_t lo, uint32_t hi) {
            for (uint64_t x = lo; x < hi; ++x) {
                const sp_region_hit& h = list[x]->h; const sp_aln& al = alns[list[x]->which];
                cells[x] = CellDesc{ (uint32_t)h.template_idx, (uint32_t)h.read, ((al.b_start - al.a_start) + (al.b_end - al.a_end)) / 2, 320, 0, -1 };
                ref[x] = al;
            }
        });
        SP_HIP_CHECK(ctx, hipMemcpyAsync(d_cells, cells, nc * sizeof(CellDesc), hipMemcpyHostToDevice, ctx->stream));
        SP_HIP_CHECK(ctx, hipMemcpyAsync(d_ref, ref, nc * sizeof(sp_aln), hipMemcpyHostToDevice, ctx->stream));
        const sp_affine_opts ao = { 1, 4, 6, 2, 26, 1, 1 };
        const int rc2 = sp_rescore_mappings(ctx, templates, reads, d_cells, d_ref, nc, false, ao, 256, d_af, prof, 320);
        if (rc2 != SP_OK) return rc2;
        SP_HIP_CHECK(ctx, hipMemcpyAsync(af, d_af, nc * sizeof(sp_affine_aln), hipMemcpyDeviceToHost, ctx->stream));
        SP_HIP_CHECK(ctx, hipStreamSynchronize(ctx->stream));
        k3_read_ranges((uint32_t)nc, [&](uint32_t, uint32_t lo, uint32_t hi) {
            for (uint64_t x = lo; x < hi; ++x) {
                sp_region_hit& h = list[x]->h;
                list[x]->done = 1;
                if (af[x].score <= 0) continue;
                h.mm2_score = af[x].score; h.mm2_nm = af[x].nm; h.mm2_start = af[x].b_start; h.mm2_end = af[x].b_end; h.mm2_q_start = af[x].a_start; h.mm2_q_end = af[x].a_end;
                h.start = af[x].b_start; h.end = af[x].b_end; h.nm = af[x].nm;
                h.unmapped = h.seq_len - (af[x].a_end - af[x].a_start); h.clip_start = af[x].a_start; h.clip_end = h.seq_len - af[x].a_end;
            }
        });
        return SP_OK;
    };
    hm.mark("host:k3_retry");
    std::vector<Pl> un; std::vector<uint32_t> first(reads->n + 1, 0);
    {
        std::vector<Pl> un_of[K3_HOST_THREADS]; uint32_t lo_of[K3_HOST_THREADS] = {}, hi_of[K3_HOST_THREADS] = {};
        k3_read_ranges(reads->n, [&](uint32_t part, uint32_t r_lo, uint32_t r_hi) {
            std::vector<Pl>& mine = un_of[part]; lo_of[part] = r_lo; hi_of[part] = r_hi;
            for (uint32_t r = r_lo; r < r_hi; ++r) {
                first[r] = (uint32_t)mine.size();
                if (reads->h_len[r] == 0) continue;
                for (uint32_t t = 0; t < T; ++t) for (int k = 0; k < CYP_TOPK; ++k) {
                    const uint32_t which = (uint32_t)(((size_t)r * T + t) * CYP_TOPK + k);
                    const sp_aln& al = alns[which];
                    if (!al.ok) continue;
                    const int tlen = templates->h_len[t];
                    sp_region_hit h{(int32_t)r, (int32_t)t, al.b_start, al.b_end, tlen, al.nm, tlen - (al.a_end - al.a_start), al.a_start, tlen - al.a_end, 0, 0, 0, 0, 0, 0};
                    if (own_score(h) > (rescore ? K3_CAP_HI : 0.05)) continue;
                    mine.push_back(Pl{ h, which, 0 });
                }
            }
        });
        size_t total = 0; for (uint32_t part = 0; part < K3_HOST_THREADS; ++part) total += un_of[part].size();
        un.reserve(total);
        for (uint32_t part = 0; part < K3_HOST_THREADS; ++part) {
            const uint32_t base = (uint32_t)un.size();
            for (uint32_t r = lo_of[part]; r < hi_of[part]; ++r) first[r] += base;
            un.insert(un.end(), un_of[part].begin(), un_of[part].end());
        }
    }
    first[reads->n] = (uint32_t)un.size();
    hm.mark("host:k3_list");
    if (rescore) {
        std::vector<Pl*> crit;
        std::vector<uint8_t> mark(un.size(), 1);
        std::vector<double> s_own(un.size()), s_pen(un.size()); std::vector<uint8_t> is_pen(un.size());
        std::vector<int> p_s(un.size()), p_e(un.size());
        k3_read_ranges(reads->n, [&](uint32_t, uint32_t r_lo, uint32_t r_hi) {
        for (size_t i = first[r_lo]; i < first[r_hi]; ++i) {
            const sp_region_hit& h = un[i].h;
            s_own[i] = cyp_score(h.seq_len, h.nm, h.unmapped, false); s_pen[i] = cyp_score(h.seq_len, h.nm, h.unmapped, true); is_pen[i] = penalized_type(template_type[h.template_idx]);
            p_s[i] = h.start; p_e[i] = h.end;
        }
        for (uint32_t r = r_lo; r < r_hi; ++r) for (uint32_t i = first[r]; i < first[r + 1]; ++i) {
            const int us = p_s[i], ue = p_e[i], ul = ue - us;
            for (uint32_t j = i + 1; j < first[r + 1]; ++j) {
                const int shared = std::min(ue, p_e[j]) - std::max(us, p_s[j]);
                if (shared <= 0) continue;
                const int vl = p_e[j] - p_s[j], ml = std::min(ul, vl);
                if ((int64_t)shared * 100 < (int64_t)84 * ml) continue;
                if (!((double)shared / (double)ml > K3_OVL)) continue;
                const bool pen = is_pen[i] || is_pen[j];
                const double a = pen ? s_pen[i] : s_own[i], b = pen ? s_pen[j] : s_own[j];
                if (a > 1.25 * b + 0.001) mark[i] = 0;
                if (b > 1.25 * a + 0.001) mark[j] = 0;
            }
        }
        });
        for (size_t i = 0; i < un.size(); ++i) if (mark[i]) crit.push_back(&un[i]);
        hm.mark("host:k3_mark");
        rc = rescore_list(crit, "k3_af_crit");
        if (rc != SP_OK) return rc;
        if (ctx->profiling) ctx->prof["k3_critical_placements"].cells += crit.size();
        hm.mark("host:k3_crit_rescore");
    }
    std::vector<Pl> coll;
    std::vector<Pl> coll_of[K3_HOST_THREADS];
    k3_read_ranges(reads->n, [&](uint32_t part, uint32_t r_lo, uint32_t r_hi) {
    std::vector<Pl>& coll = coll_of[part];
    std::vector<Pl> cur_read;
    for (uint32_t r = r_lo; r < r_hi; ++r) {
        cur_read.clear();
        for (uint32_t i = first[r]; i < first[r + 1]; ++i) if (!(own_score(un[i].h) > 0.05)) cur_read.push_back(un[i]);
        std::stable_sort(cur_read.begin(), cur_read.end(), [](const Pl& x, const Pl& y) { return x.h.start != y.h.start ? x.h.start < y.h.start : x.h.end < y.h.end; });
        bool have = false; Pl cur{};
        for (const Pl& u : cur_read) {
            if (!have) { cur = u; have = true; continue; }
            if (overlap(u.h, cur.h) > 0.9) {
                const bool pen = penalized_type(template_type[u.h.template_idx]) || penalized_type(template_type[cur.h.template_idx]);
                const int up = template_type[u.h.template_idx] == SP_CYP_DELETION, cp = template_type[cur.h.template_idx] == SP_CYP_DELETION;
                if ((cyp_score(u.h.seq_len, u.h.nm, u.h.unmapped, pen) < cyp_score(cur.h.seq_len, cur.h.nm, cur.h.unmapped, pen) && up >= cp) || up > cp) cur = u;
            } else { coll.push_back(cur); cur = u; }
        }
        if (have) coll.push_back(cur);
    }
    });
    for (uint32_t part = 0; part < K3_HOST_THREADS; ++part) coll.insert(coll.end(), coll_of[part].begin(), coll_of[part].end());
    hm.mark("host:k3_collapse");
    if (rescore) {
        std::vector<Pl*> rest;
        for (Pl& c : coll) if (!c.done) rest.push_back(&c);
        rc = rescore_list(rest, "k3_af");
        if (rc != SP_OK) return rc;
        hm.mark("host:k3_rest_rescore");
    }
    for (const Pl& c : coll) {
        const sp_region_hit& h = c.h;
        if (rescore && own_score(h) > 0.05) continue;
        if (cyp_score(h.seq_len, h.nm, h.unmapped, true) > max_missing_frac) continue;
        if (*n_hits < hits_cap) hits[*n_hits] = h;
        ++*n_hits;
    }
    return SP_OK;
}

__global__ __launch_bounds__(256) void k7_score_kernel(const uint8_t* __restrict__ hap, const uint8_t* __restrict__ is_vi, const uint8_t* __restrict__ states,
                                                       uint32_t n_variants, uint32_t n_alleles, uint32_t n_seqs, uint32_t* __restrict__ scores ) {
    const uint64_t w = ((uint64_t)blockIdx.x * blockDim.x + threadIdx.x) >> 6;
    const int lane = threadIdx.x & 63;
    if (w >= (uint64_t)n_seqs * n_alleles) return;
    const uint32_t s = (uint32_t)(w / n_alleles), a = (uint32_t)(w % n_alleles);
    const uint8_t* hv = hap + (size_t)a * n_variants; const uint8_t* sv = states + (size_t)s * n_variants;
    uint32_t vi = 0, all = 0;
    for (uint32_t v = lane; v < n_variants; v += 64) {
        const uint8_t seq_value = sv[v], hap_value = hv[v];
        const bool is_match = seq_value <= 1 ? hap_value == seq_value : seq_value == 2;
        all += is_match; vi += is_match && is_vi[v];
    }
    for (int o = 32; o > 0; o >>= 1) { vi += __shfl_xor(vi, o); all += __shfl_xor(all, o); }
    if (lane == 0) { scores[w * 2] = vi; scores[w * 2 + 1] = all; }
}

extern "C" int32_t sp_cyp_score_alleles(sp_ctx* ctx, uint32_t n_variants, uint32_t n_alleles, const uint8_t* hap_matrix, const uint8_t* is_vi,
                                        uint32_t n_seqs, const uint8_t* states, uint32_t* best_vi, uint32_t* best_all, uint8_t* tie_mask) {
    if (!ctx || (n_alleles && n_variants && (!hap_matrix || !is_vi)) || (n_seqs && (!states || !best_vi || !best_all || !tie_mask))) return SP_ERR_INVALID_ARG;
    (void)hipSetDevice(ctx->device);
    for (uint32_t s = 0; s < n_seqs; ++s) { best_vi[s] = 0; best_all[s] = 0; }
    if (n_seqs) std::memset(tie_mask, 0, (size_t)n_seqs * n_alleles);
    if (!n_seqs || !n_alleles) return SP_OK;
    const size_t hb = (size_t)n_alleles * n_variants, sb = (size_t)n_seqs * n_variants, nw = (size_t)n_seqs * n_alleles;
    uint8_t* d_hap = (uint8_t*)sp_pool(ctx, "k7_hap", hb + 1); uint8_t* d_vi = (uint8_t*)sp_pool(ctx, "k7_vi", n_variants + 1);
    uint8_t* d_st = (uint8_t*)sp_pool(ctx, "k7_states", sb + 1); uint32_t* d_sc = (uint32_t*)sp_pool(ctx, "k7_scores", nw * 8);
    if (!d_hap || !d_vi || !d_st || !d_sc) return sp_fail(ctx, SP_ERR_OUT_OF_MEMORY, "score_alleles buffers");
    (void)hipMemcpyAsync(d_hap, hap_matrix, hb, hipMemcpyHostToDevice, ctx->stream);
    (void)hipMemcpyAsync(d_vi, is_vi, n_variants, hipMemcpyHostToDevice, ctx->stream);
    (void)hipMemcpyAsync(d_st, states, sb, hipMemcpyHostToDevice, ctx->stream);
    std::vector<uint32_t> sc(nw * 2);
    {
        ProfScope ps(ctx, "k7_score", nw);
        hipLaunchKernelGGL(k7_score_kernel, dim3((unsigned)((nw * 64 + 255) / 256)), dim3(256), 0, ctx->stream, d_hap, d_vi, d_st, n_variants, n_alleles, n_seqs, d_sc);
    }
    (void)hipMemcpyAsync(sc.data(), d_sc, nw * 8, hipMemcpyDeviceToHost, ctx->stream);
    hipError_t e = hipStreamSynchronize(ctx->stream);
    if (e != hipSuccess) return sp_fail(ctx, SP_ERR_HIP, std::string("score_alleles: ") + hipGetErrorString(e));
    for (uint32_t s = 0; s < n_seqs; ++s) {
        uint32_t bv = 0, ba = 0;
        for (uint32_t a = 0; a < n_alleles; ++a) {
            const uint32_t v = sc[((size_t)s * n_alleles + a) * 2], al = sc[((size_t)s * n_alleles + a) * 2 + 1];
            if (v > bv || (v == bv && al > ba)) { bv = v; ba = al; }
        }
        best_vi[s] = bv; best_all[s] = ba;
        for (uint32_t a = 0; a < n_alleles; ++a) {
            const uint32_t v = sc[((size_t)s * n_alleles + a) * 2], al = sc[((size_t)s * n_alleles + a) * 2 + 1];
            tie_mask[(size_t)s * n_alleles + a] = (v == bv && al == ba) ? 1 : 0;
        }
    }
    return SP_OK;
}


#define K9_DIAGS 256
#define K9_INF 30000
#define K9_SITE_MAX 8

__host__ __device__ inline int k9_lds_bytes(int L, int G, int alt_bytes, int n_sites, int n_alts) { return ((L + G + alt_bytes + 3) & ~3) + 4 * (3 * n_sites + 1 + 2 * n_alts); }

struct K9Job {
    uint32_t seq_off; int32_t L;
    uint32_t bb_off; int32_t G;
    int32_t k0;
    uint32_t site_first, n_sites;
    uint32_t alt_base, n_alts;
    uint32_t alt_bytes_off, alt_bytes;
    uint32_t exit_off, entry_off;
    int32_t opt;
};

__device__ __forceinline__ void k9_step(int (&c)[4], int x, const int (&r)[4], int L, int off, int k0, int lane) {
    const int next0 = spw::from_upper(c[0], K9_INF);
    int nw[4];
    bool need = false;
    int below0;
    if (off + k0 >= 0 && off + k0 + K9_DIAGS + 1 <= L) {
        const int xm = x < 4 ? x : 99;
#pragma unroll
        for (int j = 0; j < 4; ++j) {
// ... 1199 lines not shown
```

pb-starphase_amd/csrc/sp_device.hip:

```cpp
#include "sp_internal.h"
#include "sp_wfa.hip.h"
#include "sp_anchor.hip.h"
#include <algorithm>

#ifndef SP_ANCHOR_BUCKET_BITS
#ifndef SP_ANCHOR_BUCKET_BITS
#define SP_ANCHOR_BUCKET_BITS 10
#endif
#endif
#ifndef SP_ANCHOR_ILP
#define SP_ANCHOR_ILP 2
#endif
#ifndef SP_ANCHOR_THREADS
#define SP_ANCHOR_THREADS 512
#endif
__global__ __launch_bounds__(SP_ANCHOR_THREADS) void sp_anchor_kernel(SeqSetView A, KmerIndexView KA, SeqSetView B,
                                                        const uint32_t* __restrict__ a_idx, const uint32_t* __restrict__ b_idx,
                                                        uint64_t n_pairs, int32_t* __restrict__ diag_out, int32_t* __restrict__ votes_out,
                                                        int bins_cap, int topk, int tab_cap, unsigned long long* dbg) {
    extern __shared__ uint32_t lds[];
    __shared__ unsigned long long red[SP_ANCHOR_THREADS / 64];
    __shared__ int spread[2];
    __shared__ uint16_t bucket[(1 << SP_ANCHOR_BUCKET_BITS) + 1];
    __shared__ int bucket_steps;
// ... 26 lines not shown
        long long tq[5]; tq[0] = clock64();
#define SP_AT(k) tq[k] = clock64()
#else
#define SP_AT(k)
#endif
        sp_anchor_clear<SP_ANCHOR_THREADS>(lds, nb32);
        const uint32_t* bw = B.words + cur.woff;
        const uint32_t* bn = B.nplane ? B.nplane + cur.woff : nullptr;
        const uint64_t k0 = cur.k0, k1 = cur.k1;
        const int nk = (int)(k1 - k0);
        const bool in_lds = nk <= tab_cap && nk < 65536;
        if (in_lds && (int)a != tab_a) {
            constexpr int NB = 1 << SP_ANCHOR_BUCKET_BITS, SH = 32 - SP_ANCHOR_BUCKET_BITS;
            for (int i = tid; i < nk; i += SP_ANCHOR_THREADS) {
                const uint32_t c = KA.code[k0 + i];
                tab_code[i] = c; tab_pos[i] = KA.pos[k0 + i];
                const int from = i > 0 ? (int)(KA.code[k0 + i - 1] >> SH) + 1 : 0, to = (int)(c >> SH);
                for (int q = from; q <= to; ++q) bucket[q] = (uint16_t)i;
            }
            if (tid == 0) { bucket_steps = 0; for (int q = nk > 0 ? (int)(KA.code[k1 - 1] >> SH) + 1 : 0; q <= NB; ++q) bucket[q] = (uint16_t)nk; }
            __syncthreads();
            int widest = 0;
            for (int q = tid; q < NB; q += SP_ANCHOR_THREADS) { const int w = (int)bucket[q + 1] - (int)bucket[q]; widest = w > widest ? w : widest; }
            if (widest > 0) atomicMax(&bucket_steps, 32 - __builtin_clz((unsigned)widest));
        }
        tab_a = in_lds ? (int)a : -1;
        const uint32_t* kc = in_lds ? tab_code : KA.code + k0; const int32_t* kp = in_lds ? tab_pos : KA.pos + k0;
        __syncthreads();
        SP_AT(1);
        const int steps = in_lds ? bucket_steps : nk > 0 ? 32 - __builtin_clz((unsigned)nk) : 0;
        for (int j0 = tid; j0 + SP_KMER <= n; j0 += SP_ANCHOR_THREADS * SP_ANCHOR_ILP) {
            uint32_t code[SP_ANCHOR_ILP]; int lo[SP_ANCHOR_ILP], hi[SP_ANCHOR_ILP], jj[SP_ANCHOR_ILP]; bool live[SP_ANCHOR_ILP];
#pragma unroll
            for (int u = 0; u < SP_ANCHOR_ILP; ++u) {
                const int j = j0 + u * SP_ANCHOR_THREADS;
                jj[u] = j;
                bool ok = j + SP_KMER <= n;
                const int w = ok ? j >> 4 : 0; const uint32_t sh = (uint32_t)((j & 15) << 1);
                if (ok && bn && __builtin_amdgcn_alignbit(bn[w + 1], bn[w], sh)) ok = false;
                code[u] = __builtin_amdgcn_alignbit(bw[w + 1], bw[w], sh);
                const int q = (int)(code[u] >> (32 - SP_ANCHOR_BUCKET_BITS));
                lo[u] = in_lds ? (int)bucket[q] : 0; hi[u] = !ok ? lo[u] : in_lds ? (int)bucket[q + 1] : nk; live[u] = ok;
            }
            for (int st = 0; st < steps; ++st) {
#pragma unroll
                for (int u = 0; u < SP_ANCHOR_ILP; ++u) {
                    const bool open = lo[u] < hi[u];
                    int mid = (lo[u] + hi[u]) >> 1; mid = mid < nk ? mid : nk - 1;
                    const bool less = kc[mid] < code[u];
                    lo[u] = open && less ? mid + 1 : lo[u];
                    hi[u] = open && !less ? mid : hi[u];
                }
            }
#pragma unroll
            for (int u = 0; u < SP_ANCHOR_ILP; ++u) {
                const int l = lo[u];
                int e = l;
                if (live[u]) while (e < nk && e - l <= SP_MAXOCC && kc[e] == code[u]) ++e;
                int occ = e - l;
                if (occ > SP_MAXOCC) occ = 0;
                sp_anchor_vote_run(lds, occ == 1 ? jj[u] - kp[l] + m : -1);
                if (occ > 1)
                    for (int y = l; y < e; ++y) {
                        const int bin = jj[u] - kp[y] + m;
                        atomicAdd(&lds[bin >> 1], (bin & 1) ? 0x10000u : 1u);
                    }
            }
        }
        SP_AT(2);
        __syncthreads();
        SP_AT(3);
        sp_anchor_peaks<SP_ANCHOR_THREADS>(lds, nbins, m, topk, p, diag_out, votes_out, red, spread);
        __syncthreads();
#ifdef SP_ANCHOR_TIMING
        SP_AT(4);
        if (tid == 0) { for (int k2 = 0; k2 < 4; ++k2) atomicAdd(&dbg[6 + k2], (unsigned long long)(tq[k2 + 1] - tq[k2])); atomicAdd(&dbg[10], 1ull); atomicAdd(&dbg[11], (unsigned long long)n); atomicAdd(&dbg[12], (unsigned long long)m); }
#endif
    }
}

template <bool TRACE, bool HASN>
__global__ __launch_bounds__(256) void sp_cells_kernel(SeqSetView A, SeqSetView B, const CellDesc* __restrict__ cells, uint64_t n_cells,
                                                       sp_aln* __restrict__ out, uint32_t* __restrict__ events, uint32_t ev_stride,
                                                       uint16_t* __restrict__ hist_pool, int hist_rows, int slot_words) {
    extern __shared__ uint32_t lds[];
    const int wave = threadIdx.x >> 6, lane = threadIdx.x & 63;
    uint32_t* slot = lds + wave * slot_words;
    const uint64_t gw = (uint64_t)blockIdx.x * 4 + wave, nw = (uint64_t)gridDim.x * 4;
    uint16_t* hist = TRACE ? hist_pool + gw * (uint64_t)hist_rows * SP_WAVE : nullptr;
    for (uint64_t c = gw; c < n_cells; c += nw) {
        const CellDesc cd = cells[c];
        spw::CellIn in;
        in.a_words = A.words + A.word_off[cd.a]; in.a_nplane = A.nplane ? A.nplane + A.word_off[cd.a] : nullptr;
        in.a0 = 0; in.a1 = A.len[cd.a];
        in.b_words = B.words + B.word_off[cd.b]; in.b_nplane = B.nplane ? B.nplane + B.word_off[cd.b] : nullptr;
        const int blen = B.len[cd.b];
        in.b0 = cd.b_hi >= 0 ? cd.b_lo : 0; in.b1 = cd.b_hi >= 0 ? cd.b_hi : blen;
        in.diag = cd.diag;
        in.max_ed = cd.max_ed < hist_rows - 1 ? cd.max_ed : hist_rows - 1;
        spw::CellOut o;
        uint32_t* ev = (TRACE && events) ? events + c * (uint64_t)ev_stride : nullptr;
        if (TRACE && ev && (uint32_t)in.max_ed > ev_stride) in.max_ed = (int)ev_stride;
        if (cd.diag == SP_NO_DIAG) { o.ok = 0; o.nm = 0; o.a_start = o.a_end = o.b_start = o.b_end = 0; }
        else spw::wfa_cell<TRACE, HASN>(in, slot, slot_words, lane, hist, ev, o);
        if (lane == 0) {
            sp_aln r; r.ok = o.ok; r.nm = o.nm; r.a_start = o.a_start; r.a_end = o.a_end;
            r.b_start = o.b_start; r.b_end = o.b_end; r.a_len = in.a1 - in.a0; r.b_len = in.b1 - in.b0;
            out[c] = r;
        }
    }
}


constexpr int SP_WIDE = 256;
constexpr int SP_WPL = 4;

__device__ __forceinline__ uint32_t wide_get16(const uint32_t* w, int p) { return __builtin_amdgcn_alignbit(w[(p >> 4) + 1], w[p >> 4], (uint32_t)(p & 15) << 1); }

__device__ __forceinline__ int wide_extend(const uint32_t* aw, const uint32_t* an, int m, const uint32_t* bw, const uint32_t* bn, int b0, int n, int i, int k) {
    while (i < m && i + k < n) {
        const int pa = i, pb = b0 + i + k;
        const uint32_t x = wide_get16(aw, pa) ^ wide_get16(bw, pb);
        uint32_t mm = (x | (x >> 1)) & 0x55555555u;
        if (an) mm |= wide_get16(an, pa) & 0x55555555u;
        if (bn) mm |= wide_get16(bn, pb) & 0x55555555u;
        int run = mm ? (__builtin_ctz(mm) >> 1) : 16;
        const int l1 = m - i, l2 = n - i - k, lim = l1 < l2 ? l1 : l2;
        run = run < lim ? run : lim;
        i += run;
        if (run < 16) break;
    }
    return i;
}

template <bool TRACE>
__global__ __launch_bounds__(256) void sp_cells_wide_kernel(SeqSetView A, SeqSetView B, const CellDesc* __restrict__ cells, uint64_t n_cells,
                                                            sp_aln* __restrict__ out, uint32_t* __restrict__ events, uint32_t ev_stride,
                                                            uint16_t* __restrict__ hist_pool, int hist_rows, int mode) {
    const int wave = threadIdx.x >> 6, lane = threadIdx.x & 63;
    const uint64_t gw = (uint64_t)blockIdx.x * 4 + wave, nw = (uint64_t)gridDim.x * 4;
    uint16_t* hist = TRACE ? hist_pool + gw * (uint64_t)hist_rows * SP_WIDE : nullptr;
    for (uint64_t c = gw; c < n_cells; c += nw) {
        const CellDesc cd = cells[c];
        if (cd.diag == SP_NO_DIAG) continue;
        const sp_aln narrow = out[c];
        if (narrow.ok && (mode < 2 || narrow.nm <= SP_BAND / 2)) continue;
        const uint32_t* aw = A.words + A.word_off[cd.a]; const uint32_t* an = A.nplane ? A.nplane + A.word_off[cd.a] : nullptr;
        const uint32_t* bw = B.words + B.word_off[cd.b]; const uint32_t* bn = B.nplane ? B.nplane + B.word_off[cd.b] : nullptr;
        const int m = A.len[cd.a], blen = B.len[cd.b];
        const int b0 = cd.b_hi >= 0 ? cd.b_lo : 0, n = (cd.b_hi >= 0 ? cd.b_hi : blen) - b0;
        int max_ed = cd.max_ed < hist_rows - 1 ? cd.max_ed : hist_rows - 1;
        uint32_t* ev = (TRACE && events) ? events + c * (uint64_t)ev_stride : nullptr;
        if (TRACE && ev && (uint32_t)max_ed > ev_stride) max_ed = (int)ev_stride;
        if (m <= 0 || n <= 0 || max_ed < 0) continue;
        const int kb = cd.diag - SP_WIDE / 2;
        int H[SP_WPL], O[SP_WPL];
#pragma unroll
        for (int j = 0; j < SP_WPL; ++j) {
            const int D = lane * SP_WPL + j, k = kb + D, i0 = k < 0 ? -k : 0;
            H[j] = (i0 < m && i0 + k < n) ? wide_extend(aw, an, m, bw, bn, b0, n, i0, k) : SP_NEG;
            O[j] = D;
            if (TRACE) hist[D] = (uint16_t)(H[j] >= 0 ? H[j] : 0xFFFF);
        }
        int s = 0, end_D = -1;
        for (;;) {
            long long key = -1;
#pragma unroll
            for (int j = 0; j < SP_WPL; ++j) {
                const int D = lane * SP_WPL + j, k = kb + D, i = H[j];
                if (i >= 0 && (i == m || i + k == n)) {
                    int cdist = D - SP_WIDE / 2; cdist = cdist < 0 ? -cdist : cdist;
                    const long long kk = (long long)(i + i + k) * (2ll * SP_WIDE * SP_WIDE) + (long long)(SP_WIDE - cdist) * SP_WIDE + (SP_WIDE - 1 - D);
                    key = kk > key ? kk : key;
                }
            }
#pragma unroll
            for (int o = 32; o > 0; o >>= 1) { const long long other = __shfl_xor(key, o); key = other > key ? other : key; }
            if (key >= 0) { end_D = SP_WIDE - 1 - (int)(key % SP_WIDE); break; }
            if (s == max_ed) break;
            const int from_below = spw::from_lower(H[SP_WPL - 1], SP_NEG), ofb = spw::from_lower(O[SP_WPL - 1], 0);
            const int from_above = spw::from_upper(H[0], SP_NEG), ofa = spw::from_upper(O[0], 0);
            int NH[SP_WPL], NO[SP_WPL];
#pragma unroll
            for (int j = 0; j < SP_WPL; ++j) {
                const int up = j > 0 ? H[j - 1] : from_below, oup = j > 0 ? O[j - 1] : ofb;
                const int dn = j < SP_WPL - 1 ? H[j + 1] : from_above, odn = j < SP_WPL - 1 ? O[j + 1] : ofa;
                int best = H[j] >= 0 ? H[j] + 1 : SP_NEG, o = O[j];
                if (up >= 0 && up > best) { best = up; o = oup; }
                if (dn >= 0 && dn + 1 > best) { best = dn + 1; o = odn; }
                NH[j] = best; NO[j] = o;
            }
            ++s;
#pragma unroll
            for (int j = 0; j < SP_WPL; ++j) {
                const int D = lane * SP_WPL + j;
                H[j] = NH[j] >= 0 ? wide_extend(aw, an, m, bw, bn, b0, n, NH[j], kb + D) : SP_NEG;
                O[j] = NO[j];
                if (TRACE) hist[(size_t)s * SP_WIDE + D] = (uint16_t)(H[j] >= 0 ? H[j] : 0xFFFF);
            }
        }
        if (end_D < 0) continue;
        if (narrow.ok && s >= narrow.nm) continue;
        const int el = end_D / SP_WPL, ej = end_D % SP_WPL;
        int he = 0, oe = 0;
#pragma unroll
        for (int j = 0; j < SP_WPL; ++j) if (j == ej) { he = __builtin_amdgcn_readlane(H[j], el); oe = __builtin_amdgcn_readlane(O[j], el); }
        const int ko = kb + oe, i0 = ko < 0 ? -ko : 0;
        if (lane == 0) {
            sp_aln r; r.ok = 1; r.nm = s; r.a_start = i0; r.a_end = he; r.b_start = i0 + ko; r.b_end = he + kb + end_D; r.a_len = m; r.b_len = n;
            out[c] = r;
            if (TRACE && ev) {
                __threadfence();
                int l = end_D;
                for (int t = s; t > 0; --t) {
                    const uint16_t* Hp = hist + (size_t)(t - 1) * SP_WIDE;
                    auto hv = [&](int d) { return (d < 0 || d >= SP_WIDE || Hp[d] == 0xFFFF) ? SP_NEG : (int)Hp[d]; };
                    const int cc = hv(l), uu = hv(l - 1), dd = hv(l + 1);
                    int best = cc >= 0 ? cc + 1 : SP_NEG, src = l; uint32_t type = SP_EV_X;
                    if (uu >= 0 && uu > best) { best = uu; src = l - 1; type = SP_EV_D; }
                    if (dd >= 0 && dd + 1 > best) { best = dd + 1; src = l + 1; type = SP_EV_I; }
                    const int kk = kb + l;
// ... 73 lines not shown
    for (uint32_t s = blockIdx.x; s < n; s += gridDim.x) {
        const int L = len[s]; const uint8_t* src = seq2 + off[s];
        const int nw = (L + 15) >> 4, nbytes = (L + 3) >> 2;
        for (int w = threadIdx.x; w < nw; w += blockDim.x) {
            uint32_t word = 0;
            for (int k = 0; k < 4; ++k) { const int y = 4 * w + k; if (y < nbytes) word |= (uint32_t)src[y] << (8 * k); }
            const int left = L - (w << 4);
            if (left < 16) word &= (1u << (2 * left)) - 1u;
            words[word_off[s] + w] = word;
        }
    }
}

int sp_launch_pack_on(hipStream_t stream, int num_cus, int format, const void* d_src, const uint64_t* d_off, const uint64_t* d_word_off, const int32_t* d_len, uint32_t n,
                      uint32_t* d_words, uint32_t* d_nplane, uint32_t* d_flag) {
    if (n == 0) return SP_OK;
    const unsigned grid = std::min<unsigned>(n, (unsigned)num_cus * 16);
    if (format == SP_SEQ_ASCII) hipLaunchKernelGGL(sp_pack_kernel, dim3(grid), dim3(256), 0, stream, (const char*)d_src, d_off, d_word_off, d_len, n, d_words, d_nplane, d_flag);
    else if (format == SP_SEQ_BAM4) hipLaunchKernelGGL(sp_pack4_kernel, dim3(grid), dim3(256), 0, stream, (const uint8_t*)d_src, d_off, d_word_off, d_len, n, d_words, d_nplane, d_flag);
    else if (d_words) hipLaunchKernelGGL(sp_pack2_kernel, dim3(grid), dim3(256), 0, stream, (const uint8_t*)d_src, d_off, d_word_off, d_len, n, d_words);
    return hipGetLastError() == hipSuccess ? SP_OK : SP_ERR_HIP;
}

int sp_launch_pack(sp_ctx* ctx, const char* d_ascii, const uint64_t* d_off, const uint64_t* d_word_off, const int32_t* d_len, uint32_t n,
                   uint32_t* d_words, uint32_t* d_nplane, uint32_t* d_flag) {
    if (sp_launch_pack_on(ctx->stream, ctx->num_cus, SP_SEQ_ASCII, d_ascii, d_off, d_word_off, d_len, n, d_words, d_nplane, d_flag) != SP_OK)
        return sp_fail(ctx, SP_ERR_HIP, "pack kernel launch");
    return SP_OK;
}

int sp_fail(sp_ctx* ctx, int code, const std::string& msg) { if (ctx) ctx->err = msg; return code; }

void* sp_scratch(sp_ctx* ctx, size_t bytes) {
    if (bytes <= ctx->scratch_bytes) return ctx->scratch;
    (void)hipSetDevice(ctx->device);
    if (ctx->scratch) { hipFree(ctx->scratch); ctx->scratch = nullptr; ctx->scratch_bytes = 0; }
    size_t want = bytes + bytes / 4;
    ++ctx->pool_allocs;
    if (hipMalloc(&ctx->scratch, want) != hipSuccess) { ctx->scratch = nullptr; return nullptr; }
    ctx->scratch_bytes = want;
    return ctx->scratch;
}

void* sp_pool(sp_ctx* ctx, const char* name, size_t bytes) {
    auto& e = ctx->pool[name];
    if (bytes <= e.second && e.first) return e.first;
    (void)hipSetDevice(ctx->device);
    if (e.first) { (void)hipFree(e.first); e.first = nullptr; e.second = 0; }
    size_t want = bytes + bytes / 8 + 256;
    ++ctx->pool_allocs;
    if (hipMalloc(&e.first, want) != hipSuccess) { e.first = nullptr; return nullptr; }
    e.second = want;
    return e.first;
}

size_t sp_pool_bytes(const sp_ctx* ctx, const char* name) {
    const auto it = ctx->pool.find(name);
    return it != ctx->pool.end() && it->second.first ? it->second.second : 0;
}

unsigned long long* sp_counters(sp_ctx* ctx) {
    auto it = ctx->pool.find("prof_counters");
    if (it != ctx->pool.end() && it->second.first) return (unsigned long long*)it->second.first;
    unsigned long long* c = (unsigned long long*)sp_pool(ctx, "prof_counters", SPC_N * sizeof(unsigned long long));
    if (c) (void)hipMemsetAsync(c, 0, SPC_N * sizeof(unsigned long long), ctx->stream);
    return c;
}

void* sp_host_pool(sp_ctx* ctx, const char* name, size_t bytes) {
    auto& e = ctx->host_pool[name];
    if (bytes <= e.second && e.first) return e.first;
    (void)hipSetDevice(ctx->device);
    if (e.first) { (void)hipHostFree(e.first); e.first = nullptr; e.second = 0; }
    size_t want = bytes + bytes / 8 + 256;
    if (hipHostMalloc(&e.first, want, hipHostMallocDefault) != hipSuccess) { e.first = nullptr; return nullptr; }
    e.second = want;
    return e.first;
}

int sp_launch_cells_wide(sp_ctx* ctx, const sp_seqset* A, const sp_seqset* B, const CellDesc* d_cells, uint64_t n_cells, sp_aln* d_out) {
    if (n_cells == 0) return SP_OK;
    const uint64_t wblocks = std::min<uint64_t>((n_cells + 3) / 4, (uint64_t)ctx->num_cus * 8);
    hipLaunchKernelGGL((sp_cells_wide_kernel<false>), dim3((unsigned)wblocks), dim3(256), 0, ctx->stream, A->view(), B->view(), d_cells, n_cells, d_out, (uint32_t*)nullptr, 0u,
                       (uint16_t*)nullptr, SP_MAX_ED + 1, 1);
    SP_HIP_CHECK(ctx, hipGetLastError());
    return SP_OK;
}

int sp_slot_words(const sp_seqset* A, const sp_seqset* B, bool hasn) {
    int mn = std::min(A->max_len, B->max_len);
    int w = (mn + SP_BAND + 30) / 16 + 3;
    return (hasn ? 4 : 2) * w;
}

int sp_launch_anchor(sp_ctx* ctx, const sp_seqset* A, const sp_seqset* B,
                     const uint32_t* d_a_idx, const uint32_t* d_b_idx, uint64_t n_pairs,
                     int32_t* d_diag, int32_t* d_votes, int topk, const char* prof_name, uint32_t a_period) {
    if (topk < 1 || topk > 8) return sp_fail(ctx, SP_ERR_INVALID_ARG, "anchor: topk must be 1..8");
    if (n_pairs == 0) return SP_OK;
    if (!A->has_index) return sp_fail(ctx, SP_ERR_INVALID_ARG, "anchor: set A has no k-mer index");
    int bins_cap = A->max_len + B->max_len + 1;
    size_t lds_bytes = (size_t)((bins_cap + 1) / 2) * 4;
    if (lds_bytes > 160 * 1024 - 64) return sp_fail(ctx, SP_ERR_TOO_LONG, "anchor: sequences too long for the LDS vote histogram");
    int tab_cap = A->max_len;
    if (lds_bytes + (size_t)tab_cap * 8 > 160 * 1024 - 64) tab_cap = 0;
    lds_bytes += (size_t)tab_cap * 8;
    SP_HIP_CHECK(ctx, hipFuncSetAttribute((const void*)sp_anchor_kernel, hipFuncAttributeMaxDynamicSharedMemorySize, (int)lds_bytes));
    uint64_t grid = std::min<uint64_t>(n_pairs, (uint64_t)ctx->num_cus * 8);
    if (a_period > 1 && grid > a_period) grid -= grid % a_period;
    ProfScope ps(ctx, prof_name, n_pairs);
    hipLaunchKernelGGL(sp_anchor_kernel, dim3((unsigned)grid), dim3(SP_ANCHOR_THREADS), lds_bytes, ctx->stream,
                       A->view(), A->kview(), B->view(), d_a_idx, d_b_idx, n_pairs, d_diag, d_votes, bins_cap, topk, tab_cap, sp_counters(ctx));
    SP_HIP_CHECK(ctx, hipGetLastError());
    return SP_OK;
}

#ifndef SP_TRACE_BLOCKS_PER_CU
#define SP_TRACE_BLOCKS_PER_CU 16
#endif
int sp_launch_cells(sp_ctx* ctx, const sp_seqset* A, const sp_seqset* B,
                    const CellDesc* d_cells, uint64_t n_cells,
                    sp_aln* d_out, uint32_t* d_events, uint32_t events_stride, const char* prof_name, int retry_wide) {
    if (n_cells == 0) return SP_OK;
    const bool trace = d_events != nullptr;
    const bool hasn = A->has_n || B->has_n;
    const int slot_words = sp_slot_words(A, B, hasn);
    const size_t lds_bytes = (size_t)slot_words * 4 * 4 + SP_LDS_TAIL;
    if (lds_bytes > 160 * 1024 - 64) return sp_fail(ctx, SP_ERR_TOO_LONG, "align: sequences too long for the LDS window");
    uint64_t blocks = (n_cells + 3) / 4;
    const uint64_t max_blocks = trace ? (uint64_t)ctx->num_cus * SP_TRACE_BLOCKS_PER_CU : (uint64_t)ctx->num_cus * 16;
    if (blocks > max_blocks) blocks = max_blocks;
    const int hist_rows = SP_MAX_ED + 1;
    uint16_t* hist = nullptr;
    if (trace) {
        hist = (uint16_t*)sp_scratch(ctx, blocks * 4 * (size_t)hist_rows * SP_WAVE * sizeof(uint16_t));
        if (!hist) return sp_fail(ctx, SP_ERR_OUT_OF_MEMORY, "align: traceback scratch");
    }
    SeqSetView av = A->view(), bv = B->view();
    ProfScope ps(ctx, prof_name, n_cells);
#define SP_LAUNCH(T, N) do { \
        SP_HIP_CHECK(ctx, hipFuncSetAttribute((const void*)sp_cells_kernel<T, N>, hipFuncAttributeMaxDynamicSharedMemorySize, (int)lds_bytes)); \
        hipLaunchKernelGGL((sp_cells_kernel<T, N>), dim3((unsigned)blocks), dim3(256), lds_bytes, ctx->stream, \
                           av, bv, d_cells, n_cells, d_out, d_events, events_stride, hist, hist_rows, slot_words); } while (0)
    if (trace) { if (hasn) SP_LAUNCH(true, true); else SP_LAUNCH(true, false); }
    else       { if (hasn) SP_LAUNCH(false, true); else SP_LAUNCH(false, false); }
#undef SP_LAUNCH
    SP_HIP_CHECK(ctx, hipGetLastError());
    if (retry_wide) {
        uint64_t wblocks = std::min<uint64_t>((n_cells + 3) / 4, (uint64_t)ctx->num_cus * (trace ? 2 : 8));
        uint16_t* whist = nullptr;
        if (trace) {
            whist = (uint16_t*)sp_pool(ctx, "wide_hist", wblocks * 4 * (size_t)hist_rows * SP_WIDE * sizeof(uint16_t));
            if (!whist) return sp_fail(ctx, SP_ERR_OUT_OF_MEMORY, "align: wide traceback scratch");
        }
        if (trace) hipLaunchKernelGGL((sp_cells_wide_kernel<true>), dim3((unsigned)wblocks), dim3(256), 0, ctx->stream, av, bv, d_cells, n_cells, d_out, d_events, events_stride, whist, hist_rows, retry_wide);
        else hipLaunchKernelGGL((sp_cells_wide_kernel<false>), dim3((unsigned)wblocks), dim3(256), 0, ctx->stream, av, bv, d_cells, n_cells, d_out, d_events, events_stride, whist, hist_rows, retry_wide);
        SP_HIP_CHECK(ctx, hipGetLastError());
    }
    return SP_OK;
}
```

pb-starphase_amd/csrc/sp_internal.h:

```cpp
#pragma once
#include <hip/hip_runtime.h>
#include <stdint.h>
#include <string>
#include <vector>
#include <chrono>
#include <set>
#include <mutex>
#include <map>
#include "../../include/starphase_hip.h"

#define SP_NEG        (-(1 << 28))
#define SP_SEQ_PAD_WORDS 512
#define SP_LDS_TAIL    288
#define SP_WAVE       64
#define SP_MAXOCC     4
#define SP_CELL_NONE  0xFFFFFFFFu
#define SP_PEAK_SPREAD   48
#define SP_PEAK_SUPPRESS 128

struct SeqSetView {
    const uint32_t* words;
    const uint32_t* nplane;
    const uint64_t* word_off;
    const int32_t*  len;
    uint32_t n;
};

struct KmerIndexView {
    const uint32_t* code;
    const int32_t*  pos;
    const uint64_t* off;
};

struct sp_seqset {
    sp_ctx* ctx = nullptr;
    uint32_t n = 0;
    bool has_n = false;
    std::vector<int32_t>  h_len;
    std::vector<uint64_t> h_word_off;
    std::vector<uint32_t> h_words;
    uint32_t* d_words = nullptr;
    uint32_t* d_nplane = nullptr;
    uint64_t* d_word_off = nullptr;
    int32_t*  d_len = nullptr;
    int32_t   max_len = 0;
    uint32_t  n_skipped = 0;
    struct sp_upload* up = nullptr;
    int32_t up_rc = 0; std::string up_err;
    bool has_index = false;
    uint32_t* d_kcode = nullptr; int32_t* d_kpos = nullptr; uint64_t* d_koff = nullptr;
    SeqSetView view() const { return SeqSetView{d_words, d_nplane, d_word_off, d_len, n}; }
    KmerIndexView kview() const { return KmerIndexView{d_kcode, d_kpos, d_koff}; }
};

struct ProfileEntry { double ms = 0; uint64_t launches = 0; uint64_t cells = 0; };

struct sp_ctx {
    int device = 0;
    hipStream_t stream = nullptr;
    bool own_stream = false;
    std::string err;
    bool profiling = true;
    hipEvent_t ev0 = nullptr, ev1 = nullptr;
    std::map<std::string, ProfileEntry> prof;
    struct PendingProf { hipEvent_t e0, e1; const char* name; uint64_t cells; };
    std::vector<PendingProf> prof_pending;
    std::vector<hipEvent_t> prof_free;
    void* scratch = nullptr; size_t scratch_bytes = 0;
    std::map<std::string, std::pair<void*, size_t>> pool;
    uint64_t pool_allocs = 0;
    std::map<std::string, std::pair<void*, size_t>> host_pool;
    std::multimap<size_t, void*> dev_cache; std::map<void*, size_t> dev_cap; size_t dev_cache_bytes = 0; std::mutex dev_cache_mu;
    std::set<sp_seqset*> live_sets;
    int num_cus = 256;
    int hw_queues = 4; bool hw_queues_by_library = false; std::string warning;
    bool split_genes = true;
    int split_streams = 3;
    bool cons_retry_ladder = false;
    hipStream_t copy_stream = nullptr;
    hipStream_t ctl_stream = nullptr;
    hipEvent_t ev_fork = nullptr, ev_join = nullptr;
    int k1_best_n = 5;
    int profile_rescore_counts = 0;
    int mm2_rescore = 1;
    int k8_persistent = 2;
    int hw_queues_effective = 0;
    int k8_side_orders = 1;
    int k8_compound = 1;
    int k8_side_max_blocks = 4096;
    int k8_persist_backoff = 0;
    int k8_persist_failures = 0;
    sp_seqset* uploading = nullptr;
    int k5_block_pairs = 4096;
    int cyp_cohort_min_group = 12;
    int cyp_cohort_streams = 8;
    sp_ctx* helper[7] = { nullptr, nullptr, nullptr, nullptr, nullptr, nullptr, nullptr };
};

struct CellDesc {
    uint32_t a, b;
    int32_t  diag;
    int32_t  max_ed;
    int32_t  b_lo, b_hi;
};

struct K2Dict {
    bool built = false, failed = false;
    uint32_t* d_ids = nullptr;
    uint64_t* d_id_off = nullptr;
    uint32_t* d_code = nullptr;
    uint32_t* d_dict_off = nullptr;
    std::vector<uint32_t> dict_off;
    uint32_t n_dict = 0, max_dict = 0;
};
void* sp_dev_alloc(sp_ctx* ctx, size_t bytes);
void sp_dev_release(sp_ctx* ctx, void* p);
int  sp_k2_dict_build(sp_ctx* ctx, const sp_seqset* set, const uint32_t* d_gene_of, uint32_t n_genes, K2Dict* out);
void sp_k2_dict_free(K2Dict* d);

struct K1Seed;
struct K1SeedDebug {
    uint32_t read;
    int32_t* chains; uint32_t chain_cap; uint32_t* n_chains;
    sp_k1_seed_hit* hits; uint32_t* n_hits;
    uint64_t* counters;
};
int  sp_k1_seed_build(sp_ctx* ctx, const sp_seqset* alleles, K1Seed** out);
void sp_k1_seed_free(K1Seed* s);
void sp_k1_seed_stats(const K1Seed* s, int64_t out[4]);
int  sp_k1_seed_sketch(sp_ctx* ctx, const sp_seqset* set, uint32_t idx, uint64_t* hash, int32_t* end_pos, uint8_t* strand, uint32_t cap, uint32_t* n_out);
int  sp_k1_seed_map(sp_ctx* ctx, const K1Seed* idx, const sp_seqset* alleles, const sp_seqset* reads, int best_n, int32_t* d_best, sp_k1_seed_info* d_info,
                    sp_aln* d_win_aln, sp_affine_aln* d_win_af, const K1SeedDebug* dbg, sp_hla_rev_hit* d_rev = nullptr);

sp_ctx* sp_ctx_helper(sp_ctx* ctx, int i = 0);
void sp_profile_merge(sp_ctx* into, sp_ctx* from);
int sp_launch_anchor(sp_ctx* ctx, const sp_seqset* A, const sp_seqset* B,
                     const uint32_t* d_a_idx, const uint32_t* d_b_idx, uint64_t n_pairs,
                     int32_t* d_diag, int32_t* d_votes, int topk = 1, const char* prof_name = "anchor", uint32_t a_period = 1);
int sp_launch_cells(sp_ctx* ctx, const sp_seqset* A, const sp_seqset* B,
                    const CellDesc* d_cells, uint64_t n_cells,
                    sp_aln* d_out, uint32_t* d_events, uint32_t events_stride, const char* prof_name, int retry_wide = 0);

int sp_launch_affine(sp_ctx* ctx, const sp_seqset* A, const sp_seqset* B, const void* d_pairs , uint64_t n_pairs, const sp_affine_opts& o, int band,
                     sp_affine_aln* d_out, const char* prof_name, const uint32_t* d_n_live = nullptr, const void* d_wins = nullptr, const void* d_mids = nullptr);
int sp_rescore_mappings(sp_ctx* ctx, const sp_seqset* Aw, const sp_seqset* Bw, const CellDesc* d_cells, const sp_aln* d_ref, uint64_t n, bool target_is_a,
                        const sp_affine_opts& o, int band, sp_affine_aln* d_out, const char* prefix, uint32_t stride, int trace_retry_wide = 0, const sp_aln* d_tr_in = nullptr, const uint32_t* d_ev_in = nullptr, int ends_only = 0, int windows = -1, void* d_audit = nullptr);
int sp_launch_affine_map(sp_ctx* ctx, const sp_seqset* A, const sp_seqset* B, const void* d_pairs , uint64_t n_pairs, const sp_affine_opts& o, sp_affine_aln* d_out,
                         uint32_t* d_n_cigar, uint64_t* d_op_off, uint32_t* d_ops, uint64_t ops_cap, unsigned long long* d_cursor, const char* prof_name);
constexpr uint32_t SP_ANCHOR_SKIP = 0xFFFFFFFFu;
int sp_launch_cells_wide(sp_ctx* ctx, const sp_seqset* A, const sp_seqset* B, const CellDesc* d_cells, uint64_t n_cells, sp_aln* d_out);
int sp_launch_pack_on(hipStream_t stream, int num_cus, int format, const void* d_src, const uint64_t* d_off, const uint64_t* d_word_off, const int32_t* d_len, uint32_t n,
                      uint32_t* d_words, uint32_t* d_nplane, uint32_t* d_flag);
int sp_launch_pack(sp_ctx* ctx, const char* d_ascii, const uint64_t* d_off, const uint64_t* d_word_off, const int32_t* d_len, uint32_t n,
                   uint32_t* d_words, uint32_t* d_nplane, uint32_t* d_flag);
int sp_make_segments(sp_ctx* ctx, const sp_seqset* reads, const std::vector<uint32_t>& idx, const std::vector<int32_t>& start,
                     const std::vector<int32_t>& len, const char* prefix, sp_seqset* seg, sp_seqset* hpc);
int sp_seqset_make_small(sp_ctx* ctx, const char* prefix, const char* bases, const uint64_t* offsets, uint32_t n, bool with_index, sp_seqset* out);
int sp_seqset_fetch_host(sp_ctx* ctx, sp_seqset* s);
std::string sp_seqset_decode(sp_ctx* ctx, const sp_seqset* s, uint32_t i);
enum { SPC_K1_ACTIVE = 0, SPC_K1_EXECUTED, SPC_K1_RESUMED, SPC_K1_BYTES, SPC_CONS_LAUNCHES, SPC_CONS_COLUMNS, SPC_N = 16 };
unsigned long long* sp_counters(sp_ctx* ctx);
void* sp_scratch(sp_ctx* ctx, size_t bytes);
void* sp_pool(sp_ctx* ctx, const char* name, size_t bytes);
size_t sp_pool_bytes(const sp_ctx* ctx, const char* name);
void* sp_host_pool(sp_ctx* ctx, const char* name, size_t bytes);
int   sp_fail(sp_ctx* ctx, int code, const std::string& msg);
#define SP_HIP_CHECK(ctx, expr) do { hipError_t _e = (expr); if (_e != hipSuccess) \
    return sp_fail((ctx), SP_ERR_HIP, std::string(#expr) + ": " + hipGetErrorString(_e)); } while (0)

void sp_profile_flush(sp_ctx* ctx);
struct HostMarks {
    sp_ctx* ctx; std::chrono::steady_clock::time_point t;
    explicit HostMarks(sp_ctx* c) : ctx(c), t(std::chrono::steady_clock::now()) {}
    void mark(const char* name) { const auto now = std::chrono::steady_clock::now(); if (ctx->profiling) { auto& e = ctx->prof[name]; e.ms += std::chrono::duration<double, std::milli>(now - t).count(); e.launches += 1; } t = now; }
};
struct HostScope {
    sp_ctx* ctx; const char* name; std::chrono::steady_clock::time_point t0;
    HostScope(sp_ctx* c, const char* n) : ctx(c), name(n), t0(std::chrono::steady_clock::now()) {}
    ~HostScope() { if (ctx->profiling) { auto& e = ctx->prof[name]; e.ms += std::chrono::duration<double, std::milli>(std::chrono::steady_clock::now() - t0).count(); e.launches += 1; } }
};
struct ProfScope {
    sp_ctx* ctx; const char* name; uint64_t cells; hipEvent_t e0 = nullptr, e1 = nullptr;
    ProfScope(sp_ctx* c, const char* n, uint64_t cells_) : ctx(c), name(n), cells(cells_) {
        if (!(ctx->profiling && name)) return;
        auto take = [&]() { hipEvent_t e = nullptr; if (!ctx->prof_free.empty()) { e = ctx->prof_free.back(); ctx->prof_free.pop_back(); } else if (hipEventCreate(&e) != hipSuccess) e = nullptr; return e; };
        e0 = take(); e1 = take();
        if (e0 && e1) hipEventRecord(e0, ctx->stream);
    }
    ~ProfScope() {
        if (!(e0 && e1)) { if (e0) ctx->prof_free.push_back(e0); if (e1) ctx->prof_free.push_back(e1); return; }
        hipEventRecord(e1, ctx->stream);
        ctx->prof_pending.push_back({e0, e1, name, cells});
        if (ctx->prof_pending.size() >= 2048) sp_profile_flush(ctx);
    }
};


int32_t spi_gene_entry_extras(const sp_database* db, const sp_variant_gene* g, std::string* reference_allele, bool* has_sv, std::string* sv_chrom);
std::string spi_hla_allele_fwd(sp_ctx* ctx, const sp_hla_db* db, uint32_t a);
int spi_hla_gene_fwd(const sp_hla_db* db, uint32_t gene);
int32_t spi_hla_map_type_batch(sp_ctx* ctx, const sp_hla_db* db, uint32_t n, const uint32_t* genes, const char* const* consensus_fwd, const uint32_t* consensus_len,
                               int32_t require_dna, int32_t disable_cdna, sp_hla_map** out, std::vector<uint32_t>* item_of);
int32_t spi_cyp_diplotype_mappings(sp_ctx* ctx, const sp_cyp_problem* pr, const sp_seqset* reads, sp_cyp_call* call, char* consensus, uint32_t cons_cap,
                                   sp_cyp_region_variants* region_variants, std::vector<sp_cyp_read_mapping>* mappings);
int32_t spi_cyp_diplotype_cohort_mappings(sp_ctx* ctx, const sp_cyp_problem* pr, uint32_t n_samples, const sp_seqset* const* reads, sp_cyp_call* calls,
                                          char* consensus, uint32_t cons_cap, sp_cyp_region_variants* region_variants,
                                          std::vector<sp_cyp_read_mapping>* mappings, int32_t* sample_rc);
```

Before: 357,300 reads/s.

## Move CYP2D6 region finding (k3) onto the device with live-count gated kernels

Adds a device path for CYP2D6 region finding. Hole detection, scan and compaction, and the retry/rest placement lists run in GPU kernels instead of copying all alignments to pinned host memory and processing them in host threads. Kernels for cells and rescoring take a device-side live count, so work lists can be sized on the GPU without host syncs, and an unneeded stream sync is dropped. This removes host round-trips and host CPU work in exchange for considerable new device code that must match the host results exactly.

```diff
diff --git a/pb-starphase_amd/csrc/sp_affine.hip b/pb-starphase_amd/csrc/sp_affine.hip
--- a/pb-starphase_amd/csrc/sp_affine.hip
+++ b/pb-starphase_amd/csrc/sp_affine.hip
@@ -413,9 +413,9 @@
 template <bool ENDS>
 __global__ void af_classify_kernel(const CellDesc* __restrict__ cells, const sp_aln* __restrict__ ref, const sp_aln* __restrict__ tr, const uint32_t* __restrict__ ev,
                                    uint32_t stride, uint32_t n, int target_is_a, int has_n, sp_affine_opts o, sp_affine_aln* __restrict__ out,
-                                   AfPair* __restrict__ todo, uint32_t* __restrict__ todo_at, uint32_t* __restrict__ n_todo, AfWin* __restrict__ wins, AfMid* __restrict__ mids, int band, int windows, int ends_only, AfAudit* __restrict__ audit) {
+                                   AfPair* __restrict__ todo, uint32_t* __restrict__ todo_at, uint32_t* __restrict__ n_todo, AfWin* __restrict__ wins, AfMid* __restrict__ mids, int band, int windows, int ends_only, AfAudit* __restrict__ audit, const uint32_t* __restrict__ n_live) {
     const uint32_t x = blockIdx.x * blockDim.x + threadIdx.x;
-    if (x >= n) return;
+    if (x >= n || (n_live && x >= *n_live)) return;
     sp_affine_aln res; res.score = 0; res.nm = 0; res.a_start = res.a_end = res.b_start = res.b_end = 0;
     const CellDesc c = cells[x];
     if (c.max_ed < 0) { out[x] = res; if (audit) { audit[x].route = 3; audit[x].diag = target_is_a ? -c.diag : c.diag; } return; }
@@ -565,7 +565,7 @@
 }
 
 int sp_rescore_mappings(sp_ctx* ctx, const sp_seqset* Aw, const sp_seqset* Bw, const CellDesc* d_cells, const sp_aln* d_ref, uint64_t n, bool target_is_a,
-                        const sp_affine_opts& o, int band, sp_affine_aln* d_out, const char* prefix, uint32_t stride, int trace_retry_wide, const sp_aln* d_tr_in, const uint32_t* d_ev_in, int ends_only, int windows, void* d_audit) {
+                        const sp_affine_opts& o, int band, sp_affine_aln* d_out, const char* prefix, uint32_t stride, int trace_retry_wide, const sp_aln* d_tr_in, const uint32_t* d_ev_in, int ends_only, int windows, void* d_audit, const uint32_t* d_n_live) {
     if (n == 0) return SP_OK;
     const std::string pre(prefix);
     static std::mutex names_lock; static std::set<std::string> names;
@@ -581,11 +581,11 @@
     uint32_t* d_n = d_at + n;
     (void)hipMemsetAsync(d_n, 0, 4, ctx->stream);
     int rc = SP_OK;
-    if (!d_tr_in) rc = sp_launch_cells(ctx, Aw, Bw, d_cells, n, const_cast<sp_aln*>(d_tr), const_cast<uint32_t*>(d_ev), stride, stable(pre + "_trace"), trace_retry_wide);
+    if (!d_tr_in) rc = sp_launch_cells(ctx, Aw, Bw, d_cells, n, const_cast<sp_aln*>(d_tr), const_cast<uint32_t*>(d_ev), stride, stable(pre + "_trace"), trace_retry_wide, d_n_live);
     if (rc != SP_OK) return rc;
     auto* classify = ends_only > 0 ? af_classify_kernel<true> : af_classify_kernel<false>;
     hipLaunchKernelGGL(classify, dim3((unsigned)((n + 255) / 256)), dim3(256), 0, ctx->stream, d_cells, d_ref, d_tr, d_ev, stride, (uint32_t)n, target_is_a ? 1 : 0,
-                       (Aw->has_n || Bw->has_n) ? 1 : 0, o, d_out, d_todo, d_at, d_n, d_win, d_mid, band, windows < 0 ? (ctx->mm2_rescore == 2 ? 0 : 1) : windows, ends_only, (AfAudit*)d_audit);
+                       (Aw->has_n || Bw->has_n) ? 1 : 0, o, d_out, d_todo, d_at, d_n, d_win, d_mid, band, windows < 0 ? (ctx->mm2_rescore == 2 ? 0 : 1) : windows, ends_only, (AfAudit*)d_audit, d_n_live);
     rc = sp_launch_affine(ctx, target_is_a ? Bw : Aw, target_is_a ? Aw : Bw, d_todo, n, o, band, d_part, stable(pre + "_dp"), d_n, d_win, d_mid);
     if (rc != SP_OK) return rc;
     hipLaunchKernelGGL(af_scatter_kernel, dim3((unsigned)((n + 255) / 256)), dim3(256), 0, ctx->stream, d_part, d_at, d_n, d_out);
diff --git a/pb-starphase_amd/csrc/sp_api.hip b/pb-starphase_amd/csrc/sp_api.hip
--- a/pb-starphase_amd/csrc/sp_api.hip
+++ b/pb-starphase_amd/csrc/sp_api.hip
@@ -108,7 +108,7 @@
 sp_ctx* sp_ctx_helper(sp_ctx* ctx, int i) {
     if (i < 0 || i > 6) return nullptr;
     if (!ctx->helper[i] && sp_ctx_create(ctx->device, nullptr, &ctx->helper[i]) != SP_OK) ctx->helper[i] = nullptr;
-    if (ctx->helper[i]) { ctx->helper[i]->profiling = ctx->profiling; ctx->helper[i]->k5_block_pairs = ctx->k5_block_pairs; ctx->helper[i]->k8_persistent = ctx->k8_persistent; ctx->helper[i]->k8_side_orders = ctx->k8_side_orders; ctx->helper[i]->k8_compound = ctx->k8_compound; ctx->helper[i]->k8_side_max_blocks = ctx->k8_side_max_blocks; ctx->helper[i]->mm2_rescore = ctx->mm2_rescore; ctx->helper[i]->profile_rescore_counts = ctx->profile_rescore_counts; ctx->helper[i]->k1_best_n = ctx->k1_best_n; }
+    if (ctx->helper[i]) { ctx->helper[i]->profiling = ctx->profiling; ctx->helper[i]->k5_block_pairs = ctx->k5_block_pairs; ctx->helper[i]->k8_persistent = ctx->k8_persistent; ctx->helper[i]->k8_side_orders = ctx->k8_side_orders; ctx->helper[i]->k8_compound = ctx->k8_compound; ctx->helper[i]->k8_side_max_blocks = ctx->k8_side_max_blocks; ctx->helper[i]->mm2_rescore = ctx->mm2_rescore; ctx->helper[i]->k3_device = ctx->k3_device; ctx->helper[i]->profile_rescore_counts = ctx->profile_rescore_counts; ctx->helper[i]->k1_best_n = ctx->k1_best_n; }
     return ctx->helper[i];
 }
 void sp_profile_merge(sp_ctx* into, sp_ctx* from) {
@@ -193,6 +193,7 @@
     if (std::strcmp(name, "k1_best_n") == 0) { if (value < 0 || value > 8) return sp_fail(ctx, SP_ERR_INVALID_ARG, "sp_ctx_set_option: k1_best_n is 0..8"); ctx->k1_best_n = (int)value; for (sp_ctx* h : ctx->helper) if (h) h->k1_best_n = ctx->k1_best_n; return SP_OK; }
     if (std::strcmp(name, "profile_rescore_counts") == 0) { ctx->profile_rescore_counts = value != 0; for (sp_ctx* h : ctx->helper) if (h) h->profile_rescore_counts = ctx->profile_rescore_counts; return SP_OK; }
     if (std::strcmp(name, "mm2_rescore") == 0) { ctx->mm2_rescore = (int)value; for (sp_ctx* h : ctx->helper) if (h) h->mm2_rescore = ctx->mm2_rescore; return SP_OK; }
+    if (std::strcmp(name, "k3_device") == 0) { if (value < 0 || value > 1) return sp_fail(ctx, SP_ERR_INVALID_ARG, "sp_ctx_set_option: k3_device is 0 or 1"); ctx->k3_device = (int)value; for (sp_ctx* h : ctx->helper) if (h) h->k3_device = ctx->k3_device; return SP_OK; }
     if (std::strcmp(name, "k8_side_orders") == 0) { if (value < 0 || value > 3) return sp_fail(ctx, SP_ERR_INVALID_ARG, "sp_ctx_set_option: k8_side_orders is 0 .. 3"); ctx->k8_side_orders = (int)value; for (sp_ctx* h : ctx->helper) if (h) h->k8_side_orders = ctx->k8_side_orders; return SP_OK; }
     if (std::strcmp(name, "k8_compound") == 0) { ctx->k8_compound = (int)value; for (sp_ctx* h : ctx->helper) if (h) h->k8_compound = ctx->k8_compound; return SP_OK; }
     if (std::strcmp(name, "k8_side_max_blocks") == 0) { if (value < 0) return sp_fail(ctx, SP_ERR_INVALID_ARG, "sp_ctx_set_option: k8_side_max_blocks >= 0"); ctx->k8_side_max_blocks = (int)value; for (sp_ctx* h : ctx->helper) if (h) h->k8_side_max_blocks = ctx->k8_side_max_blocks; return SP_OK; }
diff --git a/pb-starphase_amd/csrc/sp_cyp.hip b/pb-starphase_amd/csrc/sp_cyp.hip
--- a/pb-starphase_amd/csrc/sp_cyp.hip
+++ b/pb-starphase_amd/csrc/sp_cyp.hip
@@ -572,6 +572,7 @@
 
 #define CYP_TOPK      4
 #define CYP_MIN_VOTES 4
+#define K3_DEV_MAXP   512
 
 int sp_seqset_build_index(sp_ctx* ctx, sp_seqset* s);
 
@@ -601,12 +602,11 @@
     if (!d_a || !d_b || !d_d || !d_v || !d_cells || !d_alns) return sp_fail(ctx, SP_ERR_OUT_OF_MEMORY, "cyp placement buffers");
     (void)hipMemcpyAsync(d_a, ai.data(), n_pairs * 4, hipMemcpyHostToDevice, ctx->stream);
     (void)hipMemcpyAsync(d_b, bi.data(), n_pairs * 4, hipMemcpyHostToDevice, ctx->stream);
-    (void)hipStreamSynchronize(ctx->stream);
     rc = sp_launch_anchor(ctx, A, B, d_a, d_b, n_pairs, d_d, d_v, topk, "anchor", a_period);
-    if (rc) return rc;
+    if (rc) { (void)hipStreamSynchronize(ctx->stream); return rc; }
     hipLaunchKernelGGL(cyp_build_cells_kernel, dim3((unsigned)((n_cells + 255) / 256)), dim3(256), 0, ctx->stream, d_a, d_b, d_d, d_v, n_pairs, topk, CYP_MIN_VOTES, A->d_len, frac_cap, d_cells);
     rc = sp_launch_cells(ctx, A, B, d_cells, n_cells, d_alns, nullptr, 0, prof, retry_wide);
-    if (rc) return rc;
+    if (rc) { (void)hipStreamSynchronize(ctx->stream); return rc; }
     (void)hipMemcpyAsync(out.data(), d_alns, n_cells * sizeof(sp_aln), hipMemcpyDeviceToHost, ctx->stream);
     if (diag_out && votes_out) {
         diag_out->resize(n_cells); votes_out->resize(n_cells);
@@ -623,7 +623,7 @@
     if (i >= n_pairs) return;
     a_idx[i] = (uint32_t)(i % nA); b_idx[i] = (uint32_t)(i / nA);
 }
-static int cyp_align_all_pinned(sp_ctx* ctx, const sp_seqset* A, const sp_seqset* B, int topk, double frac_cap, const char* prof, sp_aln** out, int32_t** diag_out, int32_t** votes_out) {
+static int cyp_align_all_device(sp_ctx* ctx, const sp_seqset* A, const sp_seqset* B, int topk, double frac_cap, const char* prof, sp_aln** out, int32_t** diag_out, int32_t** votes_out) {
     const uint64_t nA = A->n, n_pairs = nA * (uint64_t)B->n, n_cells = n_pairs * (uint64_t)topk;
     *out = nullptr; *diag_out = nullptr; *votes_out = nullptr;
     if (n_pairs == 0) return SP_OK;
@@ -633,15 +633,25 @@
     int32_t* d_d = (int32_t*)sp_pool(ctx, "cyp_d", n_cells * 4); int32_t* d_v = (int32_t*)sp_pool(ctx, "cyp_v", n_cells * 4);
     CellDesc* d_cells = (CellDesc*)sp_pool(ctx, "cyp_cells", n_cells * sizeof(CellDesc));
     sp_aln* d_alns = (sp_aln*)sp_pool(ctx, "cyp_alns", n_cells * sizeof(sp_aln));
-    sp_aln* h_alns = (sp_aln*)sp_host_pool(ctx, "k3_alns_host", n_cells * sizeof(sp_aln));
-    int32_t* h_d = (int32_t*)sp_host_pool(ctx, "k3_diag_host", n_cells * 4); int32_t* h_v = (int32_t*)sp_host_pool(ctx, "k3_votes_host", n_cells * 4);
-    if (!d_a || !d_b || !d_d || !d_v || !d_cells || !d_alns || !h_alns || !h_d || !h_v) return sp_fail(ctx, SP_ERR_OUT_OF_MEMORY, "cyp placement buffers");
+    if (!d_a || !d_b || !d_d || !d_v || !d_cells || !d_alns) return sp_fail(ctx, SP_ERR_OUT_OF_MEMORY, "cyp placement buffers");
     hipLaunchKernelGGL(cyp_all_pairs_kernel, dim3((unsigned)((n_pairs + 255) / 256)), dim3(256), 0, ctx->stream, (uint32_t)nA, n_pairs, d_a, d_b);
     rc = sp_launch_anchor(ctx, A, B, d_a, d_b, n_pairs, d_d, d_v, topk, "anchor", (uint32_t)nA);
     if (rc) return rc;
     hipLaunchKernelGGL(cyp_build_cells_kernel, dim3((unsigned)((n_cells + 255) / 256)), dim3(256), 0, ctx->stream, d_a, d_b, d_d, d_v, n_pairs, topk, CYP_MIN_VOTES, A->d_len, frac_cap, d_cells);
     rc = sp_launch_cells(ctx, A, B, d_cells, n_cells, d_alns, nullptr, 0, prof, 0);
     if (rc) return rc;
+    *out = d_alns; *diag_out = d_d; *votes_out = d_v;
+    return SP_OK;
+}
+static int cyp_align_all_pinned(sp_ctx* ctx, const sp_seqset* A, const sp_seqset* B, int topk, double frac_cap, const char* prof, sp_aln** out, int32_t** diag_out, int32_t** votes_out) {
+    const uint64_t n_cells = (uint64_t)A->n * B->n * (uint64_t)topk;
+    sp_aln* d_alns = nullptr; int32_t* d_d = nullptr; int32_t* d_v = nullptr;
+    *out = nullptr; *diag_out = nullptr; *votes_out = nullptr;
+    const int rc = cyp_align_all_device(ctx, A, B, topk, frac_cap, prof, &d_alns, &d_d, &d_v);
+    if (rc || !d_alns) return rc;
+    sp_aln* h_alns = (sp_aln*)sp_host_pool(ctx, "k3_alns_host", n_cells * sizeof(sp_aln));
+    int32_t* h_d = (int32_t*)sp_host_pool(ctx, "k3_diag_host", n_cells * 4); int32_t* h_v = (int32_t*)sp_host_pool(ctx, "k3_votes_host", n_cells * 4);
+    if (!h_alns || !h_d || !h_v) return sp_fail(ctx, SP_ERR_OUT_OF_MEMORY, "cyp placement buffers");
     (void)hipMemcpyAsync(h_alns, d_alns, n_cells * sizeof(sp_aln), hipMemcpyDeviceToHost, ctx->stream);
     (void)hipMemcpyAsync(h_d, d_d, n_cells * 4, hipMemcpyDeviceToHost, ctx->stream);
     (void)hipMemcpyAsync(h_v, d_v, n_cells * 4, hipMemcpyDeviceToHost, ctx->stream);
@@ -659,7 +669,7 @@
     return cyp_align_pairs(ctx, A, B, ai, bi, (uint32_t)nA, topk, frac_cap, retry_wide, prof, out, diag_out, votes_out);
 }
 
-static inline double cyp_score(int seq_len, int nm, int unmapped, bool penalize) {
+__host__ __device__ static inline double cyp_score(int seq_len, int nm, int unmapped, bool penalize) {
     const int len = penalize ? seq_len : seq_len - unmapped;
     double num = (double)(nm + (penalize ? unmapped : 0)); if (num < 0.1) num = 0.1;
     return num / (double)len;
@@ -758,15 +768,19 @@
 }
 
 constexpr uint32_t K3_HOST_THREADS = 4, K3_HOST_MIN_READS = 256;
-template <class F> static void k3_read_ranges(uint32_t n_reads, F&& fn) {
+template <class F> static bool k3_read_ranges(uint32_t n_reads, F&& fn) {
     const uint32_t nt = n_reads >= K3_HOST_MIN_READS ? K3_HOST_THREADS : 1, per = (n_reads + nt - 1) / nt;
-    std::thread th[K3_HOST_THREADS]; bool started[K3_HOST_THREADS] = {};
+    std::thread th[K3_HOST_THREADS]; bool started[K3_HOST_THREADS] = {}; bool failed[K3_HOST_THREADS] = {};
+    auto guarded = [&fn, &failed](uint32_t t, uint32_t lo, uint32_t hi) { try { fn(t, lo, hi); } catch (...) { failed[t] = true; } };
     for (uint32_t t = 1; t < nt; ++t) {
         const uint32_t lo = std::min(n_reads, t * per), hi = std::min(n_reads, lo + per);
-        try { th[t] = std::thread([&fn, t, lo, hi]() { fn(t, lo, hi); }); started[t] = true; } catch (...) { fn(t, lo, hi); }
-    }
-    fn(0u, 0u, std::min(n_reads, per));
+        try { th[t] = std::thread([&guarded, t, lo, hi]() { guarded(t, lo, hi); }); started[t] = true; } catch (...) { guarded(t, lo, hi); }
+    }
+    guarded(0u, 0u, std::min(n_reads, per));
     for (uint32_t t = 1; t < nt; ++t) if (started[t]) th[t].join();
+    bool ok = true;
+    for (uint32_t t = 0; t < nt; ++t) ok = ok && !failed[t];
+    return ok;
 }
 static int32_t cyp_find_regions(sp_ctx* ctx, const sp_seqset* templates, const int32_t* template_type, const sp_seqset* reads,
                                 double max_missing_frac, sp_region_hit* hits, uint64_t hits_cap, uint64_t* n_hits, bool rescore);
@@ -777,11 +791,391 @@
 }
 constexpr double K3_CAP_HI = 0.056, K3_OVL = 0.85;
 constexpr int K3_RETRY_VOTES = 128, K3_RETRY_HOLE = 500;
-static int32_t cyp_find_regions(sp_ctx* ctx, const sp_seqset* templates, const int32_t* template_type, const sp_seqset* reads,
-                                double max_missing_frac, sp_region_hit* hits, uint64_t hits_cap, uint64_t* n_hits, bool rescore) {
-    if (!ctx || !templates || !reads || !n_hits || (templates->n && !template_type) || (hits_cap && !hits)) return SP_ERR_INVALID_ARG;
-    (void)hipSetDevice(ctx->device);
-    *n_hits = 0;
+struct K3Pl { sp_region_hit h; uint32_t which; uint32_t done; };
+enum { K3C_RETRY = 0, K3C_LIST, K3C_CRIT, K3C_REST, K3C_HITS, K3C_N = 8 };
+__device__ __forceinline__ bool k3_penalized_type(int t) { return t == SP_CYP_DELETION || t == SP_CYP_REP6 || t == SP_CYP_REP7; }
+__device__ __forceinline__ uint32_t k3_rank(bool keep, int lane, uint32_t& total) {
+    const unsigned long long m = __ballot(keep);
+    total = (uint32_t)__popcll(m);
+    return (uint32_t)__popcll(m & ((1ull << lane) - 1ull));
+}
+__global__ __launch_bounds__(1024) void k3_scan_kernel(const uint32_t* __restrict__ cnt, uint32_t n, uint32_t* __restrict__ off, uint32_t* __restrict__ total) {
+    __shared__ uint32_t wsum[16]; __shared__ uint32_t carry;
+    const int lane = threadIdx.x & 63, wave = threadIdx.x >> 6;
+    if (threadIdx.x == 0) carry = 0;
+    __syncthreads();
+    for (uint32_t base = 0; base < n; base += 1024) {
+        const uint32_t i = base + threadIdx.x, v = i < n ? cnt[i] : 0;
+        uint32_t inc = v;
+        for (int o = 1; o < 64; o <<= 1) { const uint32_t u = __shfl_up(inc, o); if (lane >= o) inc += u; }
+        if (lane == 63) wsum[wave] = inc;
+        __syncthreads();
+        uint32_t before = 0, all = 0;
+        for (int w = 0; w < 16; ++w) { if (w < wave) before += wsum[w]; all += wsum[w]; }
+        const uint32_t c = carry;
+        if (i < n) off[i] = c + before + inc - v;
+        __syncthreads();
+        if (threadIdx.x == 0) carry = c + all;
+        __syncthreads();
+    }
+    if (threadIdx.x == 0) { off[n] = carry; if (total) *total = carry; }
+}
+__global__ __launch_bounds__(64) void k3_hole_kernel(const sp_aln* __restrict__ alns, const int32_t* __restrict__ diag, const int32_t* __restrict__ votes, const int32_t* __restrict__ tlen,
+                                                     const int32_t* __restrict__ rlen, uint32_t T, uint8_t* __restrict__ flag, uint32_t* __restrict__ cnt) {
+    __shared__ int iv_s[K3_DEV_MAXP], iv_e[K3_DEV_MAXP], so_s[K3_DEV_MAXP], so_e[K3_DEV_MAXP];
+    const uint32_t r = blockIdx.x, P = T * CYP_TOPK; const int lane = threadIdx.x;
+    const size_t c0r = (size_t)r * P;
+    for (uint32_t t = lane; t < T; t += 64) flag[(size_t)r * T + t] = 0;
+    const int rl = rlen[r];
+    if (rl == 0) { if (lane == 0) cnt[r] = 0; return; }
+    uint32_t n = 0;
+    for (uint32_t base = 0; base < P; base += 64) {
+        const uint32_t p = base + lane;
+        sp_aln al; al.ok = 0;
+        if (p < P) al = alns[c0r + p];
+        uint32_t tot; const uint32_t at = k3_rank(al.ok != 0, lane, tot);
+        if (al.ok) { iv_s[n + at] = al.b_start; iv_e[n + at] = al.b_end; }
+        n += tot;
+    }
+    bool lost_mine = false;
+    for (uint32_t base = 0; base < T; base += 64) {
+        const uint32_t t = base + lane;
+        if (t < T) {
+            bool placed = false;
+            for (int k = 0; k < CYP_TOPK; ++k) placed = placed || alns[c0r + (size_t)t * CYP_TOPK + k].ok;
+            if (!placed && votes[c0r + (size_t)t * CYP_TOPK] >= K3_RETRY_VOTES) lost_mine = true;
+        }
+    }
+    if (__ballot(lost_mine) == 0ull) { if (lane == 0) cnt[r] = 0; return; }
+    __syncthreads();
+    for (uint32_t i = lane; i < n; i += 64) {
+        const int s = iv_s[i], e = iv_e[i];
+        uint32_t rank = 0;
+        for (uint32_t j = 0; j < n; ++j) { const int sj = iv_s[j], ej = iv_e[j]; rank += (sj < s || (sj == s && (ej < e || (ej == e && j < i)))) ? 1u : 0u; }
+        so_s[rank] = s; so_e[rank] = e;
+    }
+    __syncthreads();
+    uint32_t mine = 0;
+    for (uint32_t base = 0; base < T; base += 64) {
+        const uint32_t t = base + lane;
+        if (t >= T) continue;
+        const size_t c0 = c0r + (size_t)t * CYP_TOPK;
+        bool placed = false;
+        for (int k = 0; k < CYP_TOPK; ++k) placed = placed || alns[c0 + k].ok;
+        if (placed || votes[c0] < K3_RETRY_VOTES) continue;
+        const int tl = tlen[t], d0 = diag[c0];
+        const int s0 = d0 > 0 ? d0 : 0, e0 = rl < d0 + tl ? rl : d0 + tl;
+        int uncovered = 0, at = s0;
+        for (uint32_t x = 0; x < n; ++x) {
+            const int xs = so_s[x], xe = so_e[x];
+            if (xe <= at) continue;
+            if (xs >= e0) break;
+            if (xs > at) uncovered += xs - at;
+            at = at > xe ? at : xe;
+            if (at >= e0) break;
+        }
+        if (at < e0) uncovered += e0 - at;
+        if (uncovered < K3_RETRY_HOLE) continue;
+        flag[(size_t)r * T + t] = 1; ++mine;
+    }
+    for (int o = 32; o > 0; o >>= 1) mine += __shfl_xor(mine, o);
+    if (lane == 0) cnt[r] = mine;
+}
+__global__ __launch_bounds__(64) void k3_retry_cells_kernel(const uint8_t* __restrict__ flag, const uint32_t* __restrict__ off, const int32_t* __restrict__ diag, const int32_t* __restrict__ tlen,
+                                                            uint32_t T, CellDesc* __restrict__ cells, uint32_t* __restrict__ slot) {
+    const uint32_t r = blockIdx.x; const int lane = threadIdx.x;
+    if (off[r + 1] == off[r]) return;
+    uint32_t n = off[r];
+    for (uint32_t base = 0; base < T; base += 64) {
+        const uint32_t t = base + lane;
+        const bool keep = t < T && flag[(size_t)r * T + t];
+        uint32_t tot; const uint32_t at = k3_rank(keep, lane, tot);
+        if (keep) {
+            const size_t c0 = ((size_t)r * T + t) * CYP_TOPK;
+            int cap = (int)(0.05 * (double)tlen[t]) + 1; if (cap > SP_MAX_ED) cap = SP_MAX_ED;
+            CellDesc c; c.a = t; c.b = r; c.diag = diag[c0]; c.max_ed = cap; c.b_lo = 0; c.b_hi = -1;
+            cells[n + at] = c; slot[n + at] = (uint32_t)c0;
+        }
+        n += tot;
+    }
+}
+__global__ void k3_retry_patch_kernel(const sp_aln* __restrict__ got, const uint32_t* __restrict__ slot, uint32_t n, sp_aln* __restrict__ alns) {
+    const uint32_t x = blockIdx.x * blockDim.x + threadIdx.x;
+    if (x < n && got[x].ok) alns[slot[x]] = got[x];
+}
+template <bool WRITE>
+__global__ __launch_bounds__(64) void k3_list_kernel(const sp_aln* __restrict__ alns, const int32_t* __restrict__ tlen, const int32_t* __restrict__ rlen, const int32_t* __restrict__ ttype,
+                                                     uint32_t T, double cap, uint32_t* __restrict__ cnt, const uint32_t* __restrict__ first, K3Pl* __restrict__ pl) {
+    const uint32_t r = blockIdx.x, P = T * CYP_TOPK; const int lane = threadIdx.x;
+    uint32_t n = 0;
+    if (rlen[r] != 0)
+        for (uint32_t base = 0; base < P; base += 64) {
+            const uint32_t p = base + lane;
+            bool keep = false; sp_aln al; al.ok = 0; int tl = 0; uint32_t t = 0;
+            if (p < P) {
+                al = alns[(size_t)r * P + p];
+                if (al.ok) {
+                    t = p / CYP_TOPK; tl = tlen[t];
+                    keep = !(cyp_score(tl, al.nm, tl - (al.a_end - al.a_start), k3_penalized_type(ttype[t])) > cap);
+                }
+            }
+            uint32_t tot; const uint32_t at = k3_rank(keep, lane, tot);
+            if (WRITE && keep) {
+                K3Pl o;
+                o.h.read = (int32_t)r; o.h.template_idx = (int32_t)t; o.h.start = al.b_start; o.h.end = al.b_end; o.h.seq_len = tl; o.h.nm = al.nm;
+                o.h.unmapped = tl - (al.a_end - al.a_start); o.h.clip_start = al.a_start; o.h.clip_end = tl - al.a_end;
+                o.h.mm2_score = 0; o.h.mm2_nm = 0; o.h.mm2_start = 0; o.h.mm2_end = 0; o.h.mm2_q_start = 0; o.h.mm2_q_end = 0;
+                o.which = (uint32_t)((size_t)r * P + p); o.done = 0;
+                pl[first[r] + n + at] = o;
+            }
+            n += tot;
+        }
+    if (!WRITE && lane == 0) cnt[r] = n;
+}
+__global__ __launch_bounds__(64) void k3_mark_kernel(const K3Pl* __restrict__ pl, const uint32_t* __restrict__ first, const int32_t* __restrict__ ttype,
+                                                     uint8_t* __restrict__ mark, uint32_t* __restrict__ cnt) {
+    __shared__ int p_s[K3_DEV_MAXP], p_e[K3_DEV_MAXP], is_pen[K3_DEV_MAXP];
+    __shared__ double s_own[K3_DEV_MAXP], s_pen[K3_DEV_MAXP];
+    const uint32_t r = blockIdx.x, f = first[r]; const int lane = threadIdx.x;
+    uint32_t n = first[r + 1] - f; if (n > K3_DEV_MAXP) n = K3_DEV_MAXP;
+    for (uint32_t i = lane; i < n; i += 64) {
+        const sp_region_hit h = pl[f + i].h;
+        s_own[i] = cyp_score(h.seq_len, h.nm, h.unmapped, false); s_pen[i] = cyp_score(h.seq_len, h.nm, h.unmapped, true); is_pen[i] = k3_penalized_type(ttype[h.template_idx]) ? 1 : 0;
+        p_s[i] = h.start; p_e[i] = h.end;
+    }
+    __syncthreads();
+    uint32_t mine = 0;
+    for (uint32_t i = lane; i < n; i += 64) {
+        const int us = p_s[i], ue = p_e[i], ul = ue - us;
+        bool m = true;
+        for (uint32_t j = 0; j < n && m; ++j) {
+            if (j == i) continue;
+            const int shared = (ue < p_e[j] ? ue : p_e[j]) - (us > p_s[j] ? us : p_s[j]);
+            if (shared <= 0) continue;
+            const int vl = p_e[j] - p_s[j], ml = ul < vl ? ul : vl;
+            if ((int64_t)shared * 100 < (int64_t)84 * ml) continue;
+            if (!((double)shared / (double)ml > K3_OVL)) continue;
+            const bool pen = is_pen[i] || is_pen[j];
+            const double a = pen ? s_pen[i] : s_own[i], b = pen ? s_pen[j] : s_own[j];
+            if (a > 1.25 * b + 0.001) m = false;
+        }
+        mark[f + i] = m ? 1 : 0; mine += m ? 1u : 0u;
+    }
+    for (int o = 32; o > 0; o >>= 1) mine += __shfl_xor(mine, o);
+    if (lane == 0) cnt[r] = mine;
+}
+template <bool REST>
+__global__ __launch_bounds__(64) void k3_cells_kernel(const K3Pl* __restrict__ pl, const uint32_t* __restrict__ first, const uint8_t* __restrict__ mark, const uint32_t* __restrict__ coll,
+                                                      const uint32_t* __restrict__ coll_n, const uint32_t* __restrict__ off, const sp_aln* __restrict__ alns,
+                                                      CellDesc* __restrict__ cells, sp_aln* __restrict__ ref, uint32_t* __restrict__ idx) {
+    const uint32_t r = blockIdx.x, f = first[r]; const int lane = threadIdx.x;
+    if (off[r + 1] == off[r]) return;
+    const uint32_t m = REST ? coll_n[r] : first[r + 1] - f;
+    uint32_t n = off[r];
+    for (uint32_t base = 0; base < m; base += 64) {
+        const uint32_t i = base + lane;
+        uint32_t g = 0; bool keep = false;
+        if (i < m) { g = REST ? coll[f + i] : f + i; keep = REST ? pl[g].done == 0 : mark[g] != 0; }
+        uint32_t tot; const uint32_t at = k3_rank(keep, lane, tot);
+        if (keep) {
+            const K3Pl p = pl[g]; const sp_aln al = alns[p.which];
+            CellDesc c; c.a = (uint32_t)p.h.template_idx; c.b = (uint32_t)p.h.read; c.diag = ((al.b_start - al.a_start) + (al.b_end - al.a_end)) / 2; c.max_ed = 320; c.b_lo = 0; c.b_hi = -1;
+            cells[n + at] = c; ref[n + at] = al; idx[n + at] = g;
+        }
+        n += tot;
+    }
+}
+__global__ void k3_apply_kernel(const sp_affine_aln* __restrict__ af, const uint32_t* __restrict__ idx, const uint32_t* __restrict__ n_live, K3Pl* __restrict__ pl) {
+    const uint32_t x = blockIdx.x * blockDim.x + threadIdx.x;
+    if (x >= *n_live) return;
+    K3Pl* p = pl + idx[x]; const sp_affine_aln a = af[x];
+    p->done = 1;
+    if (a.score <= 0) return;
+    sp_region_hit h = p->h;
+    h.mm2_score = a.score; h.mm2_nm = a.nm; h.mm2_start = a.b_start; h.mm2_end = a.b_end; h.mm2_q_start = a.a_start; h.mm2_q_end = a.a_end;
+    h.start = a.b_start; h.end = a.b_end; h.nm = a.nm;
+    h.unmapped = h.seq_len - (a.a_end - a.a_start); h.clip_start = a.a_start; h.clip_end = h.seq_len - a.a_end;
+    p->h = h;
+}
+__global__ __launch_bounds__(64) void k3_collapse_kernel(const K3Pl* __restrict__ pl, const uint32_t* __restrict__ first, const int32_t* __restrict__ ttype,
+                                                         uint32_t* __restrict__ coll, uint32_t* __restrict__ coll_n, uint32_t* __restrict__ rest_n) {
+    __shared__ int k_s[K3_DEV_MAXP], k_e[K3_DEV_MAXP], k_i[K3_DEV_MAXP];
+    __shared__ int o_s[K3_DEV_MAXP], o_e[K3_DEV_MAXP], o_len[K3_DEV_MAXP], o_nm[K3_DEV_MAXP], o_un[K3_DEV_MAXP], o_tt[K3_DEV_MAXP], o_i[K3_DEV_MAXP];
+    __shared__ uint32_t n_out;
+    const uint32_t r = blockIdx.x, f = first[r]; const int lane = threadIdx.x;
+    uint32_t m = first[r + 1] - f; if (m > K3_DEV_MAXP) m = K3_DEV_MAXP;
+    uint32_t n = 0;
+    for (uint32_t base = 0; base < m; base += 64) {
+        const uint32_t i = base + lane;
+        bool keep = false; int s = 0, e = 0;
+        if (i < m) {
+            const sp_region_hit h = pl[f + i].h;
+            keep = !(cyp_score(h.seq_len, h.nm, h.unmapped, k3_penalized_type(ttype[h.template_idx])) > 0.05);
+            s = h.start; e = h.end;
+        }
+        uint32_t tot; const uint32_t at = k3_rank(keep, lane, tot);
+        if (keep) { k_s[n + at] = s; k_e[n + at] = e; k_i[n + at] = (int)i; }
+        n += tot;
+    }
+    __syncthreads();
+    for (uint32_t i = lane; i < n; i += 64) {
+        const int s = k_s[i], e = k_e[i];
+        uint32_t rank = 0;
+        for (uint32_t j = 0; j < n; ++j) { const int sj = k_s[j], ej = k_e[j]; rank += (sj < s || (sj == s && (ej < e || (ej == e && j < i)))) ? 1u : 0u; }
+        const sp_region_hit h = pl[f + k_i[i]].h;
+        o_s[rank] = s; o_e[rank] = e; o_len[rank] = h.seq_len; o_nm[rank] = h.nm; o_un[rank] = h.unmapped; o_tt[rank] = ttype[h.template_idx]; o_i[rank] = k_i[i];
+    }
+    __syncthreads();
+    if (lane == 0) {
+        uint32_t c = 0; int cur = -1;
+        for (uint32_t u = 0; u < n; ++u) {
+            if (cur < 0) { cur = (int)u; continue; }
+            const int min_end = o_e[u] < o_e[cur] ? o_e[u] : o_e[cur], max_start = o_s[u] > o_s[cur] ? o_s[u] : o_s[cur];
+            const double lu = (double)(o_e[u] - o_s[u]), lc = (double)(o_e[cur] - o_s[cur]);
+            const double ov = max_start < min_end ? (double)(min_end - max_start) / (lc < lu ? lc : lu) : 0.0;
+            if (ov > 0.9) {
+                const bool pen = k3_penalized_type(o_tt[u]) || k3_penalized_type(o_tt[cur]);
+                const int up = o_tt[u] == SP_CYP_DELETION, cp = o_tt[cur] == SP_CYP_DELETION;
+                if ((cyp_score(o_len[u], o_nm[u], o_un[u], pen) < cyp_score(o_len[cur], o_nm[cur], o_un[cur], pen) && up >= cp) || up > cp) cur = (int)u;
+            } else { coll[f + c++] = f + (uint32_t)o_i[cur]; cur = (int)u; }
+        }
+        if (cur >= 0) coll[f + c++] = f + (uint32_t)o_i[cur];
+        coll_n[r] = c; n_out = c;
+    }
+    __syncthreads();
+    const uint32_t c = n_out;
+    uint32_t rest = 0;
+    for (uint32_t x = lane; x < c; x += 64) rest += pl[coll[f + x]].done == 0 ? 1u : 0u;
+    for (int o = 32; o > 0; o >>= 1) rest += __shfl_xor(rest, o);
+    if (lane == 0) rest_n[r] = rest;
+}
+template <bool WRITE>
+__global__ __launch_bounds__(64) void k3_hits_kernel(const K3Pl* __restrict__ pl, const uint32_t* __restrict__ first, const uint32_t* __restrict__ coll, const uint32_t* __restrict__ coll_n,
+                                                     const int32_t* __restrict__ ttype, int rescore, double max_missing_frac, uint32_t* __restrict__ cnt,
+                                                     const uint32_t* __restrict__ off, sp_region_hit* __restrict__ hits, uint32_t hits_room) {
+    const uint32_t r = blockIdx.x, f = first[r], m = coll_n[r]; const int lane = threadIdx.x;
+    uint32_t n = WRITE ? off[r] : 0;
+    for (uint32_t base = 0; base < m; base += 64) {
+        const uint32_t i = base + lane;
+        bool keep = false; sp_region_hit h;
+        if (i < m) {
+            h = pl[coll[f + i]].h;
+            keep = !(rescore && cyp_score(h.seq_len, h.nm, h.unmapped, k3_penalized_type(ttype[h.template_idx])) > 0.05)
+                   && !(cyp_score(h.seq_len, h.nm, h.unmapped, true) > max_missing_frac);
+        }
+        uint32_t tot; const uint32_t at = k3_rank(keep, lane, tot);
+        if (WRITE && keep && n + at < hits_room) hits[n + at] = h;
+        n += tot;
+    }
+    if (!WRITE && lane == 0) cnt[r] = n;
+}
+
+static int32_t cyp_find_regions_device(sp_ctx* ctx, const sp_seqset* templates, const int32_t* template_type, const sp_seqset* reads,
+                                       double max_missing_frac, sp_region_hit* hits, uint64_t hits_cap, uint64_t* n_hits, bool rescore) {
+    HostMarks hm(ctx);
+    const uint32_t T = templates->n, R = reads->n;
+    sp_aln* d_alns = nullptr; int32_t* d_diag = nullptr; int32_t* d_votes = nullptr;
+    int rc = cyp_align_all_device(ctx, templates, reads, CYP_TOPK, 0.05, "k3_region_cells", &d_alns, &d_diag, &d_votes);
+    if (rc) return rc;
+    if (!d_alns) return SP_OK;
+    hipStream_t st = ctx->stream;
+    enum { A_RETRY_N = 0, A_RETRY_OFF, A_LIST_N, A_FIRST, A_CRIT_N, A_CRIT_OFF, A_COLL_N, A_REST_N, A_REST_OFF, A_HIT_N, A_HIT_OFF, A_COUNT };
+    const size_t stride = (size_t)R + 1;
+    uint32_t* d_reads = (uint32_t*)sp_pool(ctx, "k3_dev_reads", A_COUNT * stride * 4);
+    uint32_t* d_cnt = (uint32_t*)sp_pool(ctx, "k3_dev_counts", K3C_N * 4);
+    int32_t* d_tt = (int32_t*)sp_pool(ctx, "k3_dev_types", (size_t)T * 4);
+    uint8_t* d_flag = rescore ? (uint8_t*)sp_pool(ctx, "k3_dev_retry_flag", (size_t)R * T) : nullptr;
+    uint32_t* h_cnt = (uint32_t*)sp_host_pool(ctx, "k3_counts_host", K3C_N * 4 + (size_t)T * 4);
+    if (!d_reads || !d_cnt || !d_tt || (rescore && !d_flag) || !h_cnt) return sp_fail(ctx, SP_ERR_OUT_OF_MEMORY, "find_regions: per-read buffers");
+    auto arr = [&](int a) { return d_reads + (size_t)a * stride; };
+    int32_t* h_tt = (int32_t*)(h_cnt + K3C_N);
+    std::memcpy(h_tt, template_type, (size_t)T * 4);
+    SP_HIP_CHECK(ctx, hipMemcpyAsync(d_tt, h_tt, (size_t)T * 4, hipMemcpyHostToDevice, st));
+    SP_HIP_CHECK(ctx, hipMemsetAsync(d_cnt, 0, K3C_N * 4, st));
+    const int32_t* d_tlen = templates->d_len; const int32_t* d_rlen = reads->d_len;
+    const double cap = rescore ? K3_CAP_HI : 0.05;
+    if (rescore) {
+        hipLaunchKernelGGL(k3_hole_kernel, dim3(R), dim3(64), 0, st, d_alns, d_diag, d_votes, d_tlen, d_rlen, T, d_flag, arr(A_RETRY_N));
+        hipLaunchKernelGGL(k3_scan_kernel, dim3(1), dim3(1024), 0, st, arr(A_RETRY_N), R, arr(A_RETRY_OFF), d_cnt + K3C_RETRY);
+    }
+    auto count_list = [&]() -> int {
+        hipLaunchKernelGGL(k3_list_kernel<false>, dim3(R), dim3(64), 0, st, d_alns, d_tlen, d_rlen, d_tt, T, cap, arr(A_LIST_N), (const uint32_t*)nullptr, (K3Pl*)nullptr);
+        hipLaunchKernelGGL(k3_scan_kernel, dim3(1), dim3(1024), 0, st, arr(A_LIST_N), R, arr(A_FIRST), d_cnt + K3C_LIST);
+        SP_HIP_CHECK(ctx, hipMemcpyAsync(h_cnt, d_cnt, K3C_N * 4, hipMemcpyDeviceToHost, st));
+        SP_HIP_CHECK(ctx, hipStreamSynchronize(st));
+        return SP_OK;
+    };
+    rc = count_list();
+    if (rc) return rc;
+    hm.mark("host:k3_cells");
+    const uint32_t n_retry = rescore ? h_cnt[K3C_RETRY] : 0;
+    if (n_retry) {
+        CellDesc* d_rc = (CellDesc*)sp_pool(ctx, "k3_retry_cells", (size_t)n_retry * sizeof(CellDesc)); sp_aln* d_ro = (sp_aln*)sp_pool(ctx, "k3_retry_alns", (size_t)n_retry * sizeof(sp_aln));
+        uint32_t* d_slot = (uint32_t*)sp_pool(ctx, "k3_dev_retry_slot", (size_t)n_retry * 4);
+        if (!d_rc || !d_ro || !d_slot) return sp_fail(ctx, SP_ERR_OUT_OF_MEMORY, "find_regions: retry buffers");
+        hipLaunchKernelGGL(k3_retry_cells_kernel, dim3(R), dim3(64), 0, st, d_flag, arr(A_RETRY_OFF), d_diag, d_tlen, T, d_rc, d_slot);
+        SP_HIP_CHECK(ctx, hipMemsetAsync(d_ro, 0, (size_t)n_retry * sizeof(sp_aln), st));
+        { ProfScope ps(ctx, "k3_retry_wide", n_retry); rc = sp_launch_cells_wide(ctx, templates, reads, d_rc, n_retry, d_ro); }
+        if (rc != SP_OK) return rc;
+        hipLaunchKernelGGL(k3_retry_patch_kernel, dim3((n_retry + 255) / 256), dim3(256), 0, st, d_ro, d_slot, n_retry, d_alns);
+        if (ctx->profiling) ctx->prof["k3_retried_pairs"].cells += n_retry;
+        rc = count_list();
+        if (rc) return rc;
+    }
+    hm.mark("host:k3_retry");
+    const uint32_t n_list = h_cnt[K3C_LIST];
+    if (n_list == 0) return SP_OK;
+    K3Pl* d_pl = (K3Pl*)sp_pool(ctx, "k3_dev_list", (size_t)n_list * sizeof(K3Pl));
+    uint8_t* d_mark = (uint8_t*)sp_pool(ctx, "k3_dev_mark", n_list);
+    uint32_t* d_coll = (uint32_t*)sp_pool(ctx, "k3_dev_coll", (size_t)n_list * 4);
+    uint32_t* d_idx = (uint32_t*)sp_pool(ctx, "k3_dev_af_idx", (size_t)n_list * 4);
+    CellDesc* d_cells = (CellDesc*)sp_pool(ctx, "k3_af_cells", (size_t)n_list * sizeof(CellDesc));
+    sp_aln* d_ref = (sp_aln*)sp_pool(ctx, "k3_af_ref", (size_t)n_list * sizeof(sp_aln));
+    sp_affine_aln* d_af = (sp_affine_aln*)sp_pool(ctx, "k3_af_out", (size_t)n_list * sizeof(sp_affine_aln));
+    const uint64_t hits_room = std::min<uint64_t>(hits_cap, n_list);
+    sp_region_hit* d_hits = (sp_region_hit*)sp_pool(ctx, "k3_dev_hits", (size_t)hits_room * sizeof(sp_region_hit));
+    sp_region_hit* h_hits = (sp_region_hit*)sp_host_pool(ctx, "k3_hits_host", (size_t)hits_room * sizeof(sp_region_hit));
+    if (!d_pl || !d_mark || !d_coll || !d_idx || !d_cells || !d_ref || !d_af || !d_hits || !h_hits) return sp_fail(ctx, SP_ERR_OUT_OF_MEMORY, "find_regions: list buffers");
+    hipLaunchKernelGGL(k3_list_kernel<true>, dim3(R), dim3(64), 0, st, d_alns, d_tlen, d_rlen, d_tt, T, cap, (uint32_t*)nullptr, arr(A_FIRST), d_pl);
+    const sp_affine_opts ao = { 1, 4, 6, 2, 26, 1, 1 };
+    if (rescore) {
+        hipLaunchKernelGGL(k3_mark_kernel, dim3(R), dim3(64), 0, st, d_pl, arr(A_FIRST), d_tt, d_mark, arr(A_CRIT_N));
+        hipLaunchKernelGGL(k3_scan_kernel, dim3(1), dim3(1024), 0, st, arr(A_CRIT_N), R, arr(A_CRIT_OFF), d_cnt + K3C_CRIT);
+        hipLaunchKernelGGL(k3_cells_kernel<false>, dim3(R), dim3(64), 0, st, d_pl, arr(A_FIRST), d_mark, (const uint32_t*)nullptr, (const uint32_t*)nullptr, arr(A_CRIT_OFF), d_alns, d_cells, d_ref, d_idx);
+        rc = sp_rescore_mappings(ctx, templates, reads, d_cells, d_ref, n_list, false, ao, 256, d_af, "k3_af_crit", 320, 0, nullptr, nullptr, 0, -1, nullptr, d_cnt + K3C_CRIT);
+        if (rc != SP_OK) return rc;
+        hipLaunchKernelGGL(k3_apply_kernel, dim3((n_list + 255) / 256), dim3(256), 0, st, d_af, d_idx, d_cnt + K3C_CRIT, d_pl);
+    }
+    hipLaunchKernelGGL(k3_collapse_kernel, dim3(R), dim3(64), 0, st, d_pl, arr(A_FIRST), d_tt, d_coll, arr(A_COLL_N), arr(A_REST_N));
+    if (rescore) {
+        hipLaunchKernelGGL(k3_scan_kernel, dim3(1), dim3(1024), 0, st, arr(A_REST_N), R, arr(A_REST_OFF), d_cnt + K3C_REST);
+        hipLaunchKernelGGL(k3_cells_kernel<true>, dim3(R), dim3(64), 0, st, d_pl, arr(A_FIRST), (const uint8_t*)nullptr, d_coll, arr(A_COLL_N), arr(A_REST_OFF), d_alns, d_cells, d_ref, d_idx);
+        rc = sp_rescore_mappings(ctx, templates, reads, d_cells, d_ref, n_list, false, ao, 256, d_af, "k3_af", 320, 0, nullptr, nullptr, 0, -1, nullptr, d_cnt + K3C_REST);
+        if (rc != SP_OK) return rc;
+        hipLaunchKernelGGL(k3_apply_kernel, dim3((n_list + 255) / 256), dim3(256), 0, st, d_af, d_idx, d_cnt + K3C_REST, d_pl);
+    }
+    hipLaunchKernelGGL(k3_hits_kernel<false>, dim3(R), dim3(64), 0, st, d_pl, arr(A_FIRST), d_coll, arr(A_COLL_N), d_tt, rescore ? 1 : 0, max_missing_frac, arr(A_HIT_N), (const uint32_t*)nullptr, (sp_region_hit*)nullptr, 0u);
+    hipLaunchKernelGGL(k3_scan_kernel, dim3(1), dim3(1024), 0, st, arr(A_HIT_N), R, arr(A_HIT_OFF), d_cnt + K3C_HITS);
+    if (hits_room) hipLaunchKernelGGL(k3_hits_kernel<true>, dim3(R), dim3(64), 0, st, d_pl, arr(A_FIRST), d_coll, arr(A_COLL_N), d_tt, rescore ? 1 : 0, max_missing_frac, (uint32_t*)nullptr, arr(A_HIT_OFF), d_hits, (uint32_t)hits_room);
+    SP_HIP_CHECK(ctx, hipGetLastError());
+    const uint64_t first_part = std::min<uint64_t>(hits_room, 4096);
+    SP_HIP_CHECK(ctx, hipMemcpyAsync(h_cnt, d_cnt, K3C_N * 4, hipMemcpyDeviceToHost, st));
+    if (first_part) SP_HIP_CHECK(ctx, hipMemcpyAsync(h_hits, d_hits, (size_t)first_part * sizeof(sp_region_hit), hipMemcpyDeviceToHost, st));
+    SP_HIP_CHECK(ctx, hipStreamSynchronize(st));
+    const uint64_t total = h_cnt[K3C_HITS], have = std::min<uint64_t>(total, hits_room);
+    if (have > first_part) {
+        SP_HIP_CHECK(ctx, hipMemcpyAsync(h_hits + first_part, d_hits + first_part, (size_t)(have - first_part) * sizeof(sp_region_hit), hipMemcpyDeviceToHost, st));
+        SP_HIP_CHECK(ctx, hipStreamSynchronize(st));
+    }
+    if (have) std::memcpy(hits, h_hits, (size_t)have * sizeof(sp_region_hit));
+    *n_hits = total;
+    if (ctx->profiling && rescore) { ctx->prof["k3_critical_placements"].cells += h_cnt[K3C_CRIT]; ctx->prof["k3_rest_placements"].cells += h_cnt[K3C_REST]; }
+    hm.mark("host:k3_decide");
+    return SP_OK;
+}
+
+static int32_t cyp_find_regions_host(sp_ctx* ctx, const sp_seqset* templates, const int32_t* template_type, const sp_seqset* reads,
+                                     double max_missing_frac, sp_region_hit* hits, uint64_t hits_cap, uint64_t* n_hits, bool rescore) {
     HostMarks hm(ctx);
     sp_aln* alns = nullptr; int32_t* adiag = nullptr; int32_t* avotes = nullptr;
     int rc = cyp_align_all_pinned(ctx, templates, reads, CYP_TOPK, 0.05, "k3_region_cells", &alns, &adiag, &avotes);
@@ -793,7 +1187,7 @@
     if (rescore) {
         std::vector<CellDesc> retry; std::vector<uint32_t> retry_at;
         std::vector<CellDesc> retry_of[K3_HOST_THREADS]; std::vector<uint32_t> retry_at_of[K3_HOST_THREADS];
-        k3_read_ranges(reads->n, [&](uint32_t part, uint32_t r_lo, uint32_t r_hi) {
+        if (!k3_read_ranges(reads->n, [&](uint32_t part, uint32_t r_lo, uint32_t r_hi) {
         std::vector<CellDesc>& retry = retry_of[part]; std::vector<uint32_t>& retry_at = retry_at_of[part];
         std::vector<std::pair<int, int>> iv;
         for (uint32_t r = r_lo; r < r_hi; ++r) {
@@ -823,7 +1217,7 @@
                 retry.push_back(CellDesc{ t, r, d0, cap, 0, -1 }); retry_at.push_back((uint32_t)c0);
             }
         }
-        });
+        })) return sp_fail(ctx, SP_ERR_OUT_OF_MEMORY, "find_regions: host lists");
         for (uint32_t part = 0; part < K3_HOST_THREADS; ++part) { retry.insert(retry.end(), retry_of[part].begin(), retry_of[part].end()); retry_at.insert(retry_at.end(), retry_at_of[part].begin(), retry_at_of[part].end()); }
         if (!retry.empty()) {
             const size_t nr = retry.size();
@@ -856,13 +1250,13 @@
         sp_aln* d_ref = (sp_aln*)sp_pool(ctx, "k3_af_ref", nc * sizeof(sp_aln));
         sp_affine_aln* d_af = (sp_affine_aln*)sp_pool(ctx, "k3_af_out", nc * sizeof(sp_affine_aln));
         if (!cells || !ref || !af || !d_cells || !d_ref || !d_af) return sp_fail(ctx, SP_ERR_OUT_OF_MEMORY, "find_regions: re-score buffers");
-        k3_read_ranges((uint32_t)nc, [&](uint32_t, uint32_t lo, uint32_t hi) {
+        if (!k3_read_ranges((uint32_t)nc, [&](uint32_t, uint32_t lo, uint32_t hi) {
             for (uint64_t x = lo; x < hi; ++x) {
                 const sp_region_hit& h = list[x]->h; const sp_aln& al = alns[list[x]->which];
                 cells[x] = CellDesc{ (uint32_t)h.template_idx, (uint32_t)h.read, ((al.b_start - al.a_start) + (al.b_end - al.a_end)) / 2, 320, 0, -1 };
                 ref[x] = al;
             }
-        });
+        })) return sp_fail(ctx, SP_ERR_OUT_OF_MEMORY, "find_regions: host lists");
         SP_HIP_CHECK(ctx, hipMemcpyAsync(d_cells, cells, nc * sizeof(CellDesc), hipMemcpyHostToDevice, ctx->stream));
         SP_HIP_CHECK(ctx, hipMemcpyAsync(d_ref, ref, nc * sizeof(sp_aln), hipMemcpyHostToDevice, ctx->stream));
         const sp_affine_opts ao = { 1, 4, 6, 2, 26, 1, 1 };
@@ -870,7 +1264,7 @@
         if (rc2 != SP_OK) return rc2;
         SP_HIP_CHECK(ctx, hipMemcpyAsync(af, d_af, nc * sizeof(sp_affine_aln), hipMemcpyDeviceToHost, ctx->stream));
         SP_HIP_CHECK(ctx, hipStreamSynchronize(ctx->stream));
-        k3_read_ranges((uint32_t)nc, [&](uint32_t, uint32_t lo, uint32_t hi) {
+        if (!k3_read_ranges((uint32_t)nc, [&](uint32_t, uint32_t lo, uint32_t hi) {
             for (uint64_t x = lo; x < hi; ++x) {
                 sp_region_hit& h = list[x]->h;
                 list[x]->done = 1;
@@ -879,14 +1273,14 @@
                 h.start = af[x].b_start; h.end = af[x].b_end; h.nm = af[x].nm;
                 h.unmapped = h.seq_len - (af[x].a_end - af[x].a_start); h.clip_start = af[x].a_start; h.clip_end = h.seq_len - af[x].a_end;
             }
-        });
+        })) return sp_fail(ctx, SP_ERR_OUT_OF_MEMORY, "find_regions: host lists");
         return SP_OK;
     };
     hm.mark("host:k3_retry");
     std::vector<Pl> un; std::vector<uint32_t> first(reads->n + 1, 0);
     {
         std::vector<Pl> un_of[K3_HOST_THREADS]; uint32_t lo_of[K3_HOST_THREADS] = {}, hi_of[K3_HOST_THREADS] = {};
-        k3_read_ranges(reads->n, [&](uint32_t part, uint32_t r_lo, uint32_t r_hi) {
+        if (!k3_read_ranges(reads->n, [&](uint32_t part, uint32_t r_lo, uint32_t r_hi) {
             std::vector<Pl>& mine = un_of[part]; lo_of[part] = r_lo; hi_of[part] = r_hi;
             for (uint32_t r = r_lo; r < r_hi; ++r) {
                 first[r] = (uint32_t)mine.size();
@@ -901,7 +1295,7 @@
                     mine.push_back(Pl{ h, which, 0 });
                 }
             }
-        });
+        })) return sp_fail(ctx, SP_ERR_OUT_OF_MEMORY, "find_regions: host lists");
         size_t total = 0; for (uint32_t part = 0; part < K3_HOST_THREADS; ++part) total += un_of[part].size();
         un.reserve(total);
         for (uint32_t part = 0; part < K3_HOST_THREADS; ++part) {
@@ -917,7 +1311,7 @@
         std::vector<uint8_t> mark(un.size(), 1);
         std::vector<double> s_own(un.size()), s_pen(un.size()); std::vector<uint8_t> is_pen(un.size());
         std::vector<int> p_s(un.size()), p_e(un.size());
-        k3_read_ranges(reads->n, [&](uint32_t, uint32_t r_lo, uint32_t r_hi) {
+        if (!k3_read_ranges(reads->n, [&](uint32_t, uint32_t r_lo, uint32_t r_hi) {
         for (size_t i = first[r_lo]; i < first[r_hi]; ++i) {
             const sp_region_hit& h = un[i].h;
             s_own[i] = cyp_score(h.seq_len, h.nm, h.unmapped, false); s_pen[i] = cyp_score(h.seq_len, h.nm, h.unmapped, true); is_pen[i] = penalized_type(template_type[h.template_idx]);
@@ -937,7 +1331,7 @@
                 if (b > 1.25 * a + 0.001) mark[j] = 0;
             }
         }
-        });
+        })) return sp_fail(ctx, SP_ERR_OUT_OF_MEMORY, "find_regions: host lists");
         for (size_t i = 0; i < un.size(); ++i) if (mark[i]) crit.push_back(&un[i]);
         hm.mark("host:k3_mark");
         rc = rescore_list(crit, "k3_af_crit");
@@ -947,7 +1341,7 @@
     }
     std::vector<Pl> coll;
     std::vector<Pl> coll_of[K3_HOST_THREADS];
-    k3_read_ranges(reads->n, [&](uint32_t part, uint32_t r_lo, uint32_t r_hi) {
+    if (!k3_read_ranges(reads->n, [&](uint32_t part, uint32_t r_lo, uint32_t r_hi) {
     std::vector<Pl>& coll = coll_of[part];
     std::vector<Pl> cur_read;
     for (uint32_t r = r_lo; r < r_hi; ++r) {
@@ -965,7 +1359,7 @@
         }
         if (have) coll.push_back(cur);
     }
-    });
+    })) return sp_fail(ctx, SP_ERR_OUT_OF_MEMORY, "find_regions: host lists");
     for (uint32_t part = 0; part < K3_HOST_THREADS; ++part) coll.insert(coll.end(), coll_of[part].begin(), coll_of[part].end());
     hm.mark("host:k3_collapse");
     if (rescore) {
@@ -973,6 +1367,7 @@
         for (Pl& c : coll) if (!c.done) rest.push_back(&c);
         rc = rescore_list(rest, "k3_af");
         if (rc != SP_OK) return rc;
+        if (ctx->profiling) ctx->prof["k3_rest_placements"].cells += rest.size();
         hm.mark("host:k3_rest_rescore");
     }
     for (const Pl& c : coll) {
@@ -983,6 +1378,16 @@
         ++*n_hits;
     }
     return SP_OK;
+}
+static int32_t cyp_find_regions(sp_ctx* ctx, const sp_seqset* templates, const int32_t* template_type, const sp_seqset* reads,
+                                double max_missing_frac, sp_region_hit* hits, uint64_t hits_cap, uint64_t* n_hits, bool rescore) {
+    if (!ctx || !templates || !reads || !n_hits || (templates->n && !template_type) || (hits_cap && !hits)) return SP_ERR_INVALID_ARG;
+    (void)hipSetDevice(ctx->device);
+    *n_hits = 0;
+    if (ctx->k3_device && (uint64_t)templates->n * CYP_TOPK <= K3_DEV_MAXP)
+        return cyp_find_regions_device(ctx, templates, template_type, reads, max_missing_frac, hits, hits_cap, n_hits, rescore);
+    try { return cyp_find_regions_host(ctx, templates, template_type, reads, max_missing_frac, hits, hits_cap, n_hits, rescore); }
+    catch (const std::bad_alloc&) { return sp_fail(ctx, SP_ERR_OUT_OF_MEMORY, "find_regions: host lists"); }
 }
 
 __global__ __launch_bounds__(256) void k7_score_kernel(const uint8_t* __restrict__ hap, const uint8_t* __restrict__ is_vi, const uint8_t* __restrict__ states,
diff --git a/pb-starphase_amd/csrc/sp_device.hip b/pb-starphase_amd/csrc/sp_device.hip
--- a/pb-starphase_amd/csrc/sp_device.hip
+++ b/pb-starphase_amd/csrc/sp_device.hip
@@ -132,7 +132,8 @@
 template <bool TRACE, bool HASN>
 __global__ __launch_bounds__(256) void sp_cells_kernel(SeqSetView A, SeqSetView B, const CellDesc* __restrict__ cells, uint64_t n_cells,
                                                        sp_aln* __restrict__ out, uint32_t* __restrict__ events, uint32_t ev_stride,
-                                                       uint16_t* __restrict__ hist_pool, int hist_rows, int slot_words) {
+                                                       uint16_t* __restrict__ hist_pool, int hist_rows, int slot_words, const uint32_t* __restrict__ n_live) {
+    if (n_live && *n_live < n_cells) n_cells = *n_live;
     extern __shared__ uint32_t lds[];
     const int wave = threadIdx.x >> 6, lane = threadIdx.x & 63;
     uint32_t* slot = lds + wave * slot_words;
@@ -186,7 +187,8 @@
 template <bool TRACE>
 __global__ __launch_bounds__(256) void sp_cells_wide_kernel(SeqSetView A, SeqSetView B, const CellDesc* __restrict__ cells, uint64_t n_cells,
                                                             sp_aln* __restrict__ out, uint32_t* __restrict__ events, uint32_t ev_stride,
-                                                            uint16_t* __restrict__ hist_pool, int hist_rows, int mode) {
+                                                            uint16_t* __restrict__ hist_pool, int hist_rows, int mode, const uint32_t* __restrict__ n_live = nullptr) {
+    if (n_live && *n_live < n_cells) n_cells = *n_live;
     const int wave = threadIdx.x >> 6, lane = threadIdx.x & 63;
     const uint64_t gw = (uint64_t)blockIdx.x * 4 + wave, nw = (uint64_t)gridDim.x * 4;
     uint16_t* hist = TRACE ? hist_pool + gw * (uint64_t)hist_rows * SP_WIDE : nullptr;
@@ -426,7 +428,7 @@
     if (n_cells == 0) return SP_OK;
     const uint64_t wblocks = std::min<uint64_t>((n_cells + 3) / 4, (uint64_t)ctx->num_cus * 8);
     hipLaunchKernelGGL((sp_cells_wide_kernel<false>), dim3((unsigned)wblocks), dim3(256), 0, ctx->stream, A->view(), B->view(), d_cells, n_cells, d_out, (uint32_t*)nullptr, 0u,
-                       (uint16_t*)nullptr, SP_MAX_ED + 1, 1);
+                       (uint16_t*)nullptr, SP_MAX_ED + 1, 1, (const uint32_t*)nullptr);
     SP_HIP_CHECK(ctx, hipGetLastError());
     return SP_OK;
 }
@@ -464,7 +466,7 @@
 #endif
 int sp_launch_cells(sp_ctx* ctx, const sp_seqset* A, const sp_seqset* B,
                     const CellDesc* d_cells, uint64_t n_cells,
-                    sp_aln* d_out, uint32_t* d_events, uint32_t events_stride, const char* prof_name, int retry_wide) {
+                    sp_aln* d_out, uint32_t* d_events, uint32_t events_stride, const char* prof_name, int retry_wide, const uint32_t* d_n_live) {
     if (n_cells == 0) return SP_OK;
     const bool trace = d_events != nullptr;
     const bool hasn = A->has_n || B->has_n;
@@ -485,7 +487,7 @@
 #define SP_LAUNCH(T, N) do { \
         SP_HIP_CHECK(ctx, hipFuncSetAttribute((const void*)sp_cells_kernel<T, N>, hipFuncAttributeMaxDynamicSharedMemorySize, (int)lds_bytes)); \
         hipLaunchKernelGGL((sp_cells_kernel<T, N>), dim3((unsigned)blocks), dim3(256), lds_bytes, ctx->stream, \
-                           av, bv, d_cells, n_cells, d_out, d_events, events_stride, hist, hist_rows, slot_words); } while (0)
+                           av, bv, d_cells, n_cells, d_out, d_events, events_stride, hist, hist_rows, slot_words, d_n_live); } while (0)
     if (trace) { if (hasn) SP_LAUNCH(true, true); else SP_LAUNCH(true, false); }
     else       { if (hasn) SP_LAUNCH(false, true); else SP_LAUNCH(false, false); }
 #undef SP_LAUNCH
@@ -497,8 +499,8 @@
             whist = (uint16_t*)sp_pool(ctx, "wide_hist", wblocks * 4 * (size_t)hist_rows * SP_WIDE * sizeof(uint16_t));
             if (!whist) return sp_fail(ctx, SP_ERR_OUT_OF_MEMORY, "align: wide traceback scratch");
         }
-        if (trace) hipLaunchKernelGGL((sp_cells_wide_kernel<true>), dim3((unsigned)wblocks), dim3(256), 0, ctx->stream, av, bv, d_cells, n_cells, d_out, d_events, events_stride, whist, hist_rows, retry_wide);
-        else hipLaunchKernelGGL((sp_cells_wide_kernel<false>), dim3((unsigned)wblocks), dim3(256), 0, ctx->stream, av, bv, d_cells, n_cells, d_out, d_events, events_stride, whist, hist_rows, retry_wide);
+        if (trace) hipLaunchKernelGGL((sp_cells_wide_kernel<true>), dim3((unsigned)wblocks), dim3(256), 0, ctx->stream, av, bv, d_cells, n_cells, d_out, d_events, events_stride, whist, hist_rows, retry_wide, d_n_live);
+        else hipLaunchKernelGGL((sp_cells_wide_kernel<false>), dim3((unsigned)wblocks), dim3(256), 0, ctx->stream, av, bv, d_cells, n_cells, d_out, d_events, events_stride, whist, hist_rows, retry_wide, d_n_live);
         SP_HIP_CHECK(ctx, hipGetLastError());
     }
     return SP_OK;
diff --git a/pb-starphase_amd/csrc/sp_internal.h b/pb-starphase_amd/csrc/sp_internal.h
--- a/pb-starphase_amd/csrc/sp_internal.h
+++ b/pb-starphase_amd/csrc/sp_internal.h
@@ -91,6 +91,7 @@
     int k8_persist_backoff = 0;
     int k8_persist_failures = 0;
     sp_seqset* uploading = nullptr;
+    int k3_device = 1;
     int k5_block_pairs = 4096;
     int cyp_cohort_min_group = 12;
     int cyp_cohort_streams = 8;
@@ -139,12 +140,12 @@
                      int32_t* d_diag, int32_t* d_votes, int topk = 1, const char* prof_name = "anchor", uint32_t a_period = 1);
 int sp_launch_cells(sp_ctx* ctx, const sp_seqset* A, const sp_seqset* B,
                     const CellDesc* d_cells, uint64_t n_cells,
-                    sp_aln* d_out, uint32_t* d_events, uint32_t events_stride, const char* prof_name, int retry_wide = 0);
+                    sp_aln* d_out, uint32_t* d_events, uint32_t events_stride, const char* prof_name, int retry_wide = 0, const uint32_t* d_n_live = nullptr);
 
 int sp_launch_affine(sp_ctx* ctx, const sp_seqset* A, const sp_seqset* B, const void* d_pairs , uint64_t n_pairs, const sp_affine_opts& o, int band,
                      sp_affine_aln* d_out, const char* prof_name, const uint32_t* d_n_live = nullptr, const void* d_wins = nullptr, const void* d_mids = nullptr);
 int sp_rescore_mappings(sp_ctx* ctx, const sp_seqset* Aw, const sp_seqset* Bw, const CellDesc* d_cells, const sp_aln* d_ref, uint64_t n, bool target_is_a,
-                        const sp_affine_opts& o, int band, sp_affine_aln* d_out, const char* prefix, uint32_t stride, int trace_retry_wide = 0, const sp_aln* d_tr_in = nullptr, const uint32_t* d_ev_in = nullptr, int ends_only = 0, int windows = -1, void* d_audit = nullptr);
+                        const sp_affine_opts& o, int band, sp_affine_aln* d_out, const char* prefix, uint32_t stride, int trace_retry_wide = 0, const sp_aln* d_tr_in = nullptr, const uint32_t* d_ev_in = nullptr, int ends_only = 0, int windows = -1, void* d_audit = nullptr, const uint32_t* d_n_live = nullptr);
 int sp_launch_affine_map(sp_ctx* ctx, const sp_seqset* A, const sp_seqset* B, const void* d_pairs , uint64_t n_pairs, const sp_affine_opts& o, sp_affine_aln* d_out,
                          uint32_t* d_n_cigar, uint64_t* d_op_off, uint32_t* d_ops, uint64_t ops_cap, unsigned long long* d_cursor, const char* prof_name);
 constexpr uint32_t SP_ANCHOR_SKIP = 0xFFFFFFFFu;
```

Result: no change. 359,700 reads/s, median of 2 (+0.7%).
